# ZooMEISTER/vickers-hardness-Unet

Measured on AMD Instinct MI355X. Metric: 512x512 images/sec (train fwd+bwd), higher is better.
Workload: dtype bf16

## Files before the change

### include/vk_unet.h

```cpp
#ifndef VK_UNET_H
#define VK_UNET_H

#include <stddef.h>
#include <stdint.h>

#ifdef __cplusplus
extern "C" {
#endif

#define VK_ABI_VERSION 1
#define VK_STATS_REPLICAS 32

typedef enum { VK_F32 = 0, VK_BF16 = 1, VK_F16 = 2 } vk_dtype;

enum { VK_OK = 0, VK_ERR_ARG = -1, VK_ERR_STATE = -2, VK_ERR_UNSUPPORTED = -3 };

int vk_version(void);
const char* vk_last_error_string(void);
int vk_has_gfx950_code(void);
int vk_probe_mfma_rate(int iters, int waves_per_simd, float* sink, double* flops_out, void* stream);
int vk_set_reserved_cus(int n);
int vk_debug_hold_cus(int workgroups, int threads, int lds_bytes, int microseconds, const void* traffic, size_t traffic_bytes,
                      float* sink, void* stream);

// ... 16 lines not shown
  int N, H, W;
  int Ho, Wo;
  int K;
  int R, S, stride, pad;
  int transposed;
  vk_src src0, src1;
} vk_conv_desc;

int vk_conv_fwd(const vk_conv_desc* d, const void* w, void* y, void* y1, int split_k1, int accumulate,
                double* stats, void* stream);

int vk_conv_dgrad_pool2(const vk_conv_desc* d, const void* w, void* y_half, void* y1, int split_k1, int accumulate,
                        void* stream);

int vk_halo_pack(vk_dtype dtype, int rows, int red, const void* src, void* dst, void* stream);
int vk_conv_uses_halo_pack(const vk_conv_desc* d);
int vk_conv_fwd_packed(const vk_conv_desc* d, const void* w_halo, void* y, void* y1, int split_k1, int accumulate, double* stats,
                       void* stream);

#define VK_SPLITK_WORKSPACE_BYTES (32u << 20)
int vk_conv_fwd_splitk(const vk_conv_desc* d, const void* w_halo, void* y, void* workspace, size_t workspace_bytes, void* stream);

typedef struct {
  const void* z;
  const float* scale;
  const float* shift;
  double* sums;
  const void* mask;
  int accumulate;
} vk_bnr;

int vk_conv_dgrad_fused(const vk_conv_desc* d, const void* w, void* y, void* y1, int split_k1, int pool2, const vk_bnr* bnr,
                        void* stream);

int vk_conv1x1_fwd(const vk_conv_desc* d, const void* w, void* y, int accumulate, double* stats, void* stream);
int vk_conv1x1_wgrad(const vk_conv_desc* d, const void* dz, float* dw, void* workspace, size_t workspace_bytes, void* stream);

int vk_stem_fwd(vk_dtype dtype, int N, int H, int W, const void* x4, const void* wp, void* y, double* stats,
                void* stream);

#define VK_WGRAD_WORKSPACE_BYTES (64u << 20)
int vk_conv_wgrad(const vk_conv_desc* d, const void* dz, float* dw, void* workspace, size_t workspace_bytes, void* stream);
#define VK_WGRAD_BATCH_TABLE_BYTES (128u << 10)
int vk_conv_wgrad_batch_supports(const vk_conv_desc* d);
int vk_conv_wgrad_batch(const vk_conv_desc* descs, const void* const* dz, float* const* dw, int n, int workgroups, void* tables,
                        size_t tables_bytes, void* workspace, size_t workspace_bytes, void* stream);
int vk_stem_wgrad(vk_dtype dtype, int N, int H, int W, const void* x4, const void* dz, float* dw_krsc3, void* workspace,
                  size_t workspace_bytes, void* stream);
int vk_stem_wgrad_bn(vk_dtype dtype, int N, int H, int W, const void* x4, const void* g, const void* z, const float* coef_abc,
                     float* dw_krsc3, void* workspace, size_t workspace_bytes, void* stream);
int vk_conv_bwd_onepass(const vk_conv_desc* d_fwd, const void* g, const void* z, const float* coef_abc, const void* w_dgrad, void* y,
                        const vk_bnr* bnr, float* dw, void* workspace, size_t workspace_bytes, void* stream);
int vk_stem_dgrad(vk_dtype dtype, int N, int H, int W, const void* g, const void* z, const float* coef_abc, const float* w_krsc3,
                  float* dx, void* stream);

typedef struct {
  int h, w;
  int src_stride;
  int size;
  int nh, nw;
  int top, left;
  int pad_value;
} vk_letterbox_desc;

int vk_letterbox_preprocess(const vk_letterbox_desc* d, const uint8_t* bgr, float* x_nchw, void* stream);
int vk_letterbox_postprocess_mask(const vk_letterbox_desc* d, const float* logits, float thresh, uint8_t* mask_hw, void* stream);
// ... 98 lines not shown

typedef struct {
  int item;
  int k;
  int oy, ox;
  float zoom;
  float cos_a, sin_a;
  int reserved;
} vk_patch_params;

#define VK_PATCH_FORCE_GENERAL 1

int vk_patch_index(int n_items, const vk_patch_item* items_host, void* items_dev, size_t images_bytes, const uint8_t* masks,
                   size_t masks_bytes, int32_t* rowcum, size_t rowcum_len, void* stream);
int vk_patch_batch(int n, int size, int n_items, const void* items_dev, const uint8_t* images, const uint8_t* masks, const int32_t* rowcum,
                   const vk_patch_params* params_host, void* params_dev, int flags, int32_t* origins, uint8_t* patches_rgb,
                   uint8_t* patches_mask, void* stream);

int vk_input_transform(vk_dtype dtype, int N, int H, int W, const float* x, void* x4, void* stream);

int vk_bn_finalize(int C, int train, const double* stats, double count, const float* gamma, const float* beta,
                   float* running_mean, float* running_var, float eps, float momentum, float* scale, float* shift,
                   float* save_mean, float* save_invstd, void* stream);

int vk_bn_relu_maxpool(vk_dtype dtype, int N, int H, int W, int C, const void* z, const float* scale,
                       const float* shift, void* pooled, uint8_t* argmax, void* stream);
int vk_maxpool_bwd(vk_dtype dtype, int N, int H, int W, int C, const void* dpool, const uint8_t* argmax, void* dy,
                   void* stream);
int vk_maxpool_bwd_bn_reduce(vk_dtype dtype, int N, int H, int W, int C, const void* dpool, const uint8_t* argmax, const void* z,
                             const float* scale, const float* shift, void* dy, double* sums, void* stream);

int vk_bn_add_relu(vk_dtype dtype, size_t pixels, int C, const void* z, const float* scale, const float* shift,
                   const void* res, const float* rscale, const float* rshift, void* out, void* stream);

int vk_bn_bwd_reduce(vk_dtype dtype, size_t pixels, int C, const void* dy, const void* z, int mask_mode,
                     const float* scale, const float* shift, const void* mask_src, double* sums, void* stream);
int vk_bn_bwd_coeffs(int C, const double* sums, double count, const float* gamma, const float* save_mean,
                     const float* save_invstd, float* dgamma, float* dbeta, float* coef_abc, void* stream);
int vk_bn_bwd_apply(vk_dtype dtype, size_t pixels, int C, const void* dy, const void* z, int mask_mode,
                    const float* scale, const float* shift, const void* mask_src, const float* coef_abc, void* dz,
                    void* g_out, int g_accumulate, void* stream);
int vk_bn_bwd_coeffs_frozen(int C, const double* sums, const float* gamma, const float* running_mean, const float* running_invstd,
                            float* dgamma, float* dbeta, float* coef_abc, void* stream);
int vk_bn_bwd_apply_fused(vk_dtype dtype, size_t pixels, int C, const void* dy, const void* z, int mask_mode,
                          const float* scale, const float* shift, const void* mask_src, const double* sums, double count,
                          const float* gamma, const float* save_mean, const float* save_invstd, float* dgamma, float* dbeta,
                          void* dz, void* g_out, int g_accumulate, void* stream);

int vk_upsample2x_bwd(vk_dtype dtype, int N, int H, int W, int C, const void* d_up, void* d_low, int accumulate,
                      void* stream);

int vk_head_fwd(vk_dtype dtype, int N, int H, int W, const vk_src* src, const float* w9x16, const float* bias,
                float* logits, void* stream);
int vk_dec4_tail_eval(vk_dtype dtype, int N, int H, int W, const vk_src* src, const void* w1_pack, const float* scale1, const float* shift1,
                      const void* w2_plain, const float* scale2, const float* shift2, const float* head_w9x16, const float* head_bias,
                      float* logits, void* stream);
#define VK_HEAD_WORKSPACE_BYTES (1024u * 148u * 4u)
int vk_head_bwd(vk_dtype dtype, int N, int H, int W, const vk_src* src, const float* w9x16, const float* dlogits,
                void* dy, float* dw9x16, float* dbias, void* workspace, size_t workspace_bytes, void* stream);
int vk_head_bwd_fused(vk_dtype dtype, int N, int H, int W, const vk_src* src, const float* w9x16, const float* dlogits,
                      void* dy, float* dw9x16, float* dbias, const vk_bnr* bnr, void* workspace, size_t workspace_bytes, void* stream);

int vk_bce_dice_loss(size_t count, const float* logits, const float* target, double* sums, float* loss_out,
                     float* dlogits, float grad_scale, float w_bce, float w_dice, void* stream);

int vk_head_fwd_multi(vk_dtype dtype, int N, int H, int W, int C, const vk_src* src, const float* w, const float* bias, float* logits,
// ... 219 lines not shown
```

### vickers-hardness-unet_amd/_lib.py

```python
from __future__ import annotations

import ctypes as C
import os
import subprocess
from pathlib import Path

PKG_DIR = Path(__file__).resolve().parent
LIB_PATH = Path(os.environ["VK_LIB"]) if os.environ.get("VK_LIB") else PKG_DIR / "libvkunet.so"
CSRC = PKG_DIR / "csrc"

VK_F32, VK_BF16, VK_F16 = 0, 1, 2
VK_LOSS_BINARY, VK_LOSS_MULTILABEL, VK_LOSS_MULTICLASS = 0, 1, 2
VK_ENC_RESNET18, VK_ENC_RESNET34, VK_ENC_RESNET50 = 18, 34, 50
VK_ADAMW_MAX_GROUPS = 8
VK_NORM_L2, VK_NORM_INF = 0, 1
VK_TILE_MAX_ORIGINS, VK_TILE_MAX_SIDE = 64, 4096
VK_BLEND_PROB, VK_BLEND_LOGIT = 0, 1
VK_PATCH_FORCE_GENERAL = 1


class VkError(RuntimeError):
    pass


class vk_src(C.Structure):
    _fields_ = [("ptr", C.c_void_p), ("C", C.c_int), ("up", C.c_int), ("scale", C.c_void_p),
                ("shift", C.c_void_p), ("relu", C.c_int)]


class vk_conv_desc(C.Structure):
    _fields_ = [("dtype", C.c_int), ("N", C.c_int), ("H", C.c_int), ("W", C.c_int), ("Ho", C.c_int),
                ("Wo", C.c_int), ("K", C.c_int), ("R", C.c_int), ("S", C.c_int), ("stride", C.c_int),
                ("pad", C.c_int), ("transposed", C.c_int), ("src0", vk_src), ("src1", vk_src)]


class vk_bnr(C.Structure):
    _fields_ = [("z", C.c_void_p), ("scale", C.c_void_p), ("shift", C.c_void_p), ("sums", C.c_void_p), ("mask", C.c_void_p),
                ("accumulate", C.c_int)]


class vk_letterbox_desc(C.Structure):
    _fields_ = [("h", C.c_int), ("w", C.c_int), ("src_stride", C.c_int), ("size", C.c_int), ("nh", C.c_int),
                ("nw", C.c_int), ("top", C.c_int), ("left", C.c_int), ("pad_value", C.c_int)]


class vk_tile_desc(C.Structure):
    _fields_ = [("h", C.c_int), ("w", C.c_int), ("src_stride", C.c_int), ("T", C.c_int), ("overlap", C.c_int), ("ny", C.c_int),
                ("nx", C.c_int), ("ys", C.c_int * VK_TILE_MAX_ORIGINS), ("xs", C.c_int * VK_TILE_MAX_ORIGINS), ("view_mask", C.c_int),
                ("pad_value", C.c_int), ("C", C.c_int)]


class vk_geom_desc(C.Structure):
    _fields_ = [("h", C.c_int), ("w", C.c_int), ("bin_thresh", C.c_float), ("morph_kernel", C.c_int), ("open_iter", C.c_int),
                ("close_iter", C.c_int), ("min_area", C.c_int), ("max_components", C.c_int)]


class vk_geom_det(C.Structure):
    _fields_ = [("label", C.c_int), ("area", C.c_int), ("box", C.c_int * 8), ("cx", C.c_float), ("cy", C.c_float),
                ("rw", C.c_float), ("rh", C.c_float), ("ux", C.c_float), ("uy", C.c_float), ("hull_n", C.c_int),
                ("reserved", C.c_int), ("d1", C.c_double), ("d2", C.c_double), ("d_mean", C.c_double)]


class vk_geom_quad(C.Structure):
    _fields_ = [("label", C.c_int), ("area", C.c_int), ("box", C.c_int * 8), ("cx", C.c_float), ("cy", C.c_float),
                ("valid", C.c_int), ("branch", C.c_int), ("n_candidates", C.c_int), ("contour_n", C.c_int), ("hull_n", C.c_int),
                ("flags", C.c_int), ("quality", C.c_double), ("d1", C.c_double), ("d2", C.c_double), ("d_mean", C.c_double)]


class vk_aug_params(C.Structure):
    _fields_ = [("d4", C.c_int), ("rotate", C.c_int), ("cos_a", C.c_float), ("sin_a", C.c_float), ("photo", C.c_int),
                ("alpha", C.c_float), ("beta", C.c_float), ("blur_ksize", C.c_int), ("noise_scale", C.c_float),
# ... 60 lines not shown
                ("iters", C.c_int * 4), ("v", C.c_double * 8), ("vs", C.c_double * 8), ("d1", C.c_double), ("d2", C.c_double),
                ("d_mean", C.c_double)]


class vk_adamw_group(C.Structure):
    _fields_ = [("lr", C.c_float), ("beta1", C.c_float), ("beta2", C.c_float), ("eps", C.c_float), ("weight_decay", C.c_float)]


class vk_unet_config(C.Structure):
    _fields_ = [("N", C.c_int), ("size", C.c_int), ("dtype", C.c_int), ("training", C.c_int), ("width", C.c_int)]


class vk_tensor_info(C.Structure):
    _fields_ = [("name", C.c_char * 96), ("kind", C.c_int), ("dims", C.c_int * 4), ("ndim", C.c_int),
                ("offset", C.c_int64), ("numel", C.c_int64)]


vp, ci, cf, cd, sz, i64 = C.c_void_p, C.c_int, C.c_float, C.c_double, C.c_size_t, C.c_int64
P = C.POINTER

SIGNATURES = {
    "vk_version": (ci, []),
    "vk_last_error_string": (C.c_char_p, []),
    "vk_has_gfx950_code": (ci, []),
    "vk_probe_mfma_rate": (ci, [ci, ci, vp, P(C.c_double), vp]),
    "vk_set_reserved_cus": (ci, [ci]),
    "vk_debug_hold_cus": (ci, [ci, ci, ci, ci, vp, sz, vp, vp]),
    "vk_debug_set_stamp_buffer": (ci, [vp]),
    "vk_prof_enable": (ci, [ci]),
    "vk_prof_collect": (ci, [C.c_char_p, sz]),
    "vk_conv_fwd": (ci, [P(vk_conv_desc), vp, vp, vp, ci, ci, vp, vp]),
    "vk_conv_dgrad_pool2": (ci, [P(vk_conv_desc), vp, vp, vp, ci, ci, vp]),
    "vk_conv_dgrad_fused": (ci, [P(vk_conv_desc), vp, vp, vp, ci, ci, P(vk_bnr), vp]),
    "vk_head_bwd_fused": (ci, [ci, ci, ci, ci, P(vk_src), vp, vp, vp, vp, vp, P(vk_bnr), vp, sz, vp]),
    "vk_halo_pack": (ci, [ci, ci, ci, vp, vp, vp]),
    "vk_conv_uses_halo_pack": (ci, [P(vk_conv_desc)]),
    "vk_conv_fwd_packed": (ci, [P(vk_conv_desc), vp, vp, vp, ci, ci, vp, vp]),
    "vk_conv_fwd_splitk": (ci, [P(vk_conv_desc), vp, vp, vp, sz, vp]),
    "vk_stem_fwd": (ci, [ci, ci, ci, ci, vp, vp, vp, vp, vp]),
    "vk_conv_wgrad": (ci, [P(vk_conv_desc), vp, vp, vp, sz, vp]),
    "vk_conv1x1_fwd": (ci, [P(vk_conv_desc), vp, vp, ci, vp, vp]),
    "vk_conv1x1_wgrad": (ci, [P(vk_conv_desc), vp, vp, vp, sz, vp]),
    "vk_conv_wgrad_batch_supports": (ci, [P(vk_conv_desc)]),
    "vk_conv_wgrad_batch": (ci, [P(vk_conv_desc), P(vp), P(vp), ci, ci, vp, sz, vp, sz, vp]),
    "vk_stem_wgrad": (ci, [ci, ci, ci, ci, vp, vp, vp, vp, sz, vp]),
    "vk_stem_wgrad_bn": (ci, [ci, ci, ci, ci, vp, vp, vp, vp, vp, vp, sz, vp]),
    "vk_conv_bwd_onepass": (ci, [P(vk_conv_desc), vp, vp, vp, vp, vp, P(vk_bnr), vp, vp, sz, vp]),
    "vk_stem_dgrad": (ci, [ci, ci, ci, ci, vp, vp, vp, vp, vp, vp]),
    "vk_letterbox_preprocess": (ci, [P(vk_letterbox_desc), vp, vp, vp]),
    "vk_letterbox_postprocess_mask": (ci, [P(vk_letterbox_desc), vp, cf, vp, vp]),
    "vk_letterbox_postprocess_prob": (ci, [P(vk_letterbox_desc), vp, vp, vp]),
    "vk_letterbox_postprocess_labels": (ci, [P(vk_letterbox_desc), ci, vp, vp, vp]),
    "vk_letterbox_postprocess_mask_multi": (ci, [P(vk_letterbox_desc), ci, vp, cf, vp, vp]),
    "vk_letterbox_postprocess_prob_multi": (ci, [P(vk_letterbox_desc), ci, ci, vp, vp, vp]),
    "vk_tile_preprocess": (ci, [P(vk_tile_desc), vp, vp, vp]),
    "vk_tile_blend": (ci, [P(vk_tile_desc), ci, vp, cf, vp, vp, vp]),
    "vk_geom_workspace_bytes": (i64, [P(vk_geom_desc), ci]),
    "vk_geom_minarearect": (ci, [P(vk_geom_desc), ci, vp, vp, vp, vp, vp, sz, vp]),
    "vk_geom_quadrilateral": (ci, [P(vk_geom_desc), ci, ci, vp, vp, vp, vp, vp, sz, vp]),
    "vk_geom_slot_map": (ci, [P(vk_geom_desc), ci, vp, sz, vp, vp]),
    "vk_letterbox_u8": (ci, [P(vk_letterbox_desc), vp, vp, vp]),
    "vk_letterbox_mask_u8": (ci, [P(vk_letterbox_desc), vp, vp, vp]),
    "vk_augment_workspace_bytes": (C.c_size_t, [ci, ci]),
    "vk_augment_batch": (ci, [ci, ci, ci, vp, vp, vp, P(vk_aug_params), vp, vp, vp, C.c_size_t, vp, vp, vp]),
    "vk_patch_index": (ci, [ci, P(vk_patch_item), vp, sz, vp, sz, vp, sz, vp]),
    "vk_patch_batch": (ci, [ci, ci, ci, vp, vp, vp, vp, P(vk_patch_params), vp, ci, vp, vp, vp, vp]),
    "vk_input_transform": (ci, [ci, ci, ci, ci, vp, vp, vp]),
    "vk_bn_finalize": (ci, [ci, ci, vp, cd, vp, vp, vp, vp, cf, cf, vp, vp, vp, vp, vp]),
    "vk_bn_relu_maxpool": (ci, [ci, ci, ci, ci, ci, vp, vp, vp, vp, vp, vp]),
    "vk_maxpool_bwd": (ci, [ci, ci, ci, ci, ci, vp, vp, vp, vp]),
    "vk_maxpool_bwd_bn_reduce": (ci, [ci, ci, ci, ci, ci, vp, vp, vp, vp, vp, vp, vp, vp]),
    "vk_bn_add_relu": (ci, [ci, sz, ci, vp, vp, vp, vp, vp, vp, vp, vp]),
    "vk_bn_bwd_reduce": (ci, [ci, sz, ci, vp, vp, ci, vp, vp, vp, vp, vp]),
    "vk_bn_bwd_coeffs": (ci, [ci, vp, cd, vp, vp, vp, vp, vp, vp, vp]),
    "vk_bn_bwd_coeffs_frozen": (ci, [ci, vp, vp, vp, vp, vp, vp, vp, vp]),
    "vk_bn_bwd_apply": (ci, [ci, sz, ci, vp, vp, ci, vp, vp, vp, vp, vp, vp, ci, vp]),
    "vk_bn_bwd_apply_fused": (ci, [ci, sz, ci, vp, vp, ci, vp, vp, vp, vp, cd, vp, vp, vp, vp, vp, vp, vp, ci, vp]),
    "vk_upsample2x_bwd": (ci, [ci, ci, ci, ci, ci, vp, vp, ci, vp]),
    "vk_head_fwd": (ci, [ci, ci, ci, ci, P(vk_src), vp, vp, vp, vp]),
    "vk_dec4_tail_eval": (ci, [ci, ci, ci, ci, P(vk_src), vp, vp, vp, vp, vp, vp, vp, vp, vp, vp]),
    "vk_head_bwd": (ci, [ci, ci, ci, ci, P(vk_src), vp, vp, vp, vp, vp, vp, sz, vp]),
    "vk_bce_dice_loss": (ci, [sz, vp, vp, vp, vp, vp, cf, cf, cf, vp]),
    "vk_head_fwd_multi": (ci, [ci, ci, ci, ci, ci, P(vk_src), vp, vp, vp, vp]),
    "vk_head_multi_workspace_bytes": (sz, [ci]),
    "vk_head_bwd_multi": (ci, [ci, ci, ci, ci, ci, P(vk_src), vp, vp, vp, vp, vp, P(vk_bnr), vp, sz, vp]),
    "vk_multi_loss_workspace_bytes": (sz, [ci, ci, ci]),
    "vk_multilabel_loss": (ci, [ci, ci, ci, vp, vp, vp, sz, vp, vp, cf, cf, cf, vp]),
    "vk_multiclass_loss": (ci, [ci, ci, ci, vp, vp, vp, sz, vp, vp, cf, cf, cf, vp]),
    "vk_seg_loss_cfg_size": (sz, []),
    "vk_seg_loss_workspace_bytes": (sz, [ci, ci, ci]),
    "vk_seg_loss": (ci, [P(vk_seg_loss_cfg), ci, ci, ci, vp, vp, vp, sz, vp, vp, cf, vp]),
    "vk_lovasz_cfg_size": (sz, []),
    "vk_lovasz_workspace_bytes": (sz, [P(vk_lovasz_cfg), ci, ci, ci]),
    "vk_lovasz_loss": (ci, [P(vk_lovasz_cfg), ci, ci, ci, vp, vp, vp, sz, vp, vp, cf, ci, vp]),
    "vk_lovasz_flat_workspace_bytes": (sz, [ci, i64]),
    "vk_lovasz_flat": (ci, [vp, vp, ci, i64, vp, sz, vp, vp, vp, vp]),
    "vk_seg_metrics_workspace_bytes": (C.c_size_t, [ci]),
    "vk_seg_metrics": (ci, [ci, sz, vp, vp, ci, cf, cf, vp, sz, vp, vp]),
    "vk_seg_metrics_multi_workspace_bytes": (sz, [ci, ci]),
    "vk_seg_metrics_multi": (ci, [ci, ci, ci, sz, vp, vp, ci, cf, cf, vp, sz, vp, vp, vp, vp]),
    "vk_sweep_hist": (ci, [ci, sz, sz, vp, vp, ci, ci, ci, ci, ci, vp, vp, ci, vp, vp, vp]),
    "vk_sweep_curves_layout": (ci, [ci, ci, ci, ci, P(vk_sweep_layout)]),
    "vk_sweep_curves_out_bytes": (sz, [ci, ci, ci, ci]),
    "vk_sweep_curves": (ci, [ci, ci, ci, vp, vp, ci, cf, vp, sz, vp, sz, vp]),
    "vk_inst_contingency": (ci, [ci, ci, ci, vp, vp, ci, ci, vp, vp]),
# ... 117 lines not shown
```

### vickers-hardness-unet_amd/csrc/conv_halo.hip

```cpp
#include <stdlib.h>
#include <string.h>

#include <string>
#include <type_traits>

#include "vk_common.h"

#ifdef VK_STAMP
#define VK_T(var) { __builtin_amdgcn_sched_barrier(0); const unsigned long long t_ = __builtin_amdgcn_s_memtime(); __builtin_amdgcn_s_waitcnt(0xC07F); __builtin_amdgcn_sched_barrier(0); var = t_; }
#else
#define VK_T(var)
#endif

namespace vk {

struct HaloSrc {
  const void* ptr;
  const float* scale;
  const float* shift;
  int C, up, relu;
  uint32_t bytes;
};

#ifndef VK_EPI_BATCH_READS
#define VK_EPI_BATCH_READS 1
#endif
#ifndef VK_COLP_DEFER_STATS
#define VK_COLP_DEFER_STATS 1
#endif
#ifndef VK_COLQ_ILV
#define VK_COLQ_ILV 1
#endif
#ifndef VK_COLQ_DIAG
#define VK_COLQ_DIAG 0
#endif
#ifndef VK_COLQ_PRE
#define VK_COLQ_PRE 1
#endif
struct HaloParams {
  HaloSrc s0, s1;
  const void* w;
  uint32_t w_bytes;
  void* y0;
  void* y1;
  int ld0, ld1, split;
  double* stats;
  int N, H, W, K, C, flip, accumulate, pool2;
  int Hi, Wi;
  int tiles_x, tiles_y, nchunks;
  unsigned long long* stamps;
  int kyn;
  int ksplit;
  size_t slab_bytes;
  float* slab;
  int dbg;
  const void* bnr_z;
  const float* bnr_scale;
  const float* bnr_shift;
  double* bnr_sums;
  const void* bnr_mask;
};

template <typename T, int TH, int BN, int WGM, int WGN>
struct HaloCfg {
  using Tr = ElemTraits<T>;
  static constexpr int EB = Tr::kBytes;
  static constexpr int VE = Tr::kVec;
  static constexpr int CK = 64 / EB;
  static constexpr int HW_ = 18, HH = TH + 2, HPIX = HH * HW_;
  static constexpr int APS = 96;
  static constexpr int A_BYTES = HPIX * APS;
  static constexpr int B_BYTES = 3 * BN * 64;
  static constexpr int NPV = (HPIX * 4 + 255) / 256;
  static constexpr int NBV = (3 * BN * 4 + 255) / 256;
  static constexpr int BM = TH * 16;
  static constexpr int WR = TH / WGM;
  static constexpr int WCH = BN / WGN;
  static constexpr int TP = WR, TC = WCH / 16;
  static constexpr int ESB = BN * EB + 16;
  static constexpr int EVPR = BN / VE;
  static constexpr int ERPP = 256 / EVPR;
  static constexpr int EPASS = BM / ERPP;
  static constexpr int RED_OFF = BM * ESB;
  static constexpr int MAIN = A_BYTES + 2 * B_BYTES;
  static constexpr int ESLOTS = (BN / VE > 16) ? 4 * 4 / (BN / VE / 16) : 4 * 4;
  static constexpr int EPI = RED_OFF + ESLOTS * BN * 2 * 4;
  static constexpr int SMEM = MAIN > EPI ? MAIN : EPI;
  static_assert(WGM * WGN == 4 && TH % WGM == 0 && BN % (16 * WGN) == 0, "wave layout");
  static_assert(EPASS >= 1, "epilogue mapping");
  static_assert(SMEM <= 160 * 1024, "main-loop / epilogue LDS image exceeds the 160 KiB of a CU");
};

__device__ __forceinline__ int swz(int row) { return ((row >> 2) & 1) << 1; }

__device__ __forceinline__ int halo_group(int tid) {
  const int g = tid >> 2;
  return (g & ~3) | ((g & 1) << 1) | ((g >> 1) & 1);
}


template <typename T, int TH, int BN, int TP, int TC, int NT = 256, bool PRE = false, int OS = 1>
__device__ __forceinline__ void halo_epilogue(char* smem, f32x4_t (&acc)[TC][TP], const HaloParams& p, int n, int y0, int x0, int n0,
                                              int wrow0, int wch0, int py = 0, int px = 0, double* defer = nullptr) {
  using Tr = ElemTraits<T>;
  constexpr int EB = Tr::kBytes, VE = Tr::kVec;
  constexpr int BM = TH * 16;
  constexpr int ESB = BN * EB + 16;
  constexpr int EVPR = BN / VE, ERPP = NT / EVPR, EPASS = BM / ERPP, NW = NT / 64;
  constexpr int RED_OFF = BM * ESB;
  static_assert(BM % ERPP == 0 && EVPR <= 64, "epilogue mapping");
  const int tid = threadIdx.x, lane = tid & 63, wave = tid >> 6;
  const int li = lane & 15, kg = lane >> 4;

  const int e_row = tid / EVPR;
  const int e_vec = (EVPR == 16 && EB == 2) ? (((tid & 15) + ((e_row & 1) ? 15 : 0)) & 15) : tid % EVPR;
  const int col0 = n0 + e_vec * VE;
  const bool col_ok = col0 < p.K;
  char* yb = (char*)p.y0;
  int ld = p.ld0, colx = col0;
  bool first_part = true;
  if (p.split > 0 && col0 >= p.split) { yb = (char*)p.y1; ld = p.ld1; colx = col0 - p.split; first_part = false; }
  float s1[VE], s2[VE];
#pragma unroll
  for (int j = 0; j < VE; ++j) { s1[j] = 0.f; s2[j] = 0.f; }
  const bool bnr = p.bnr_z != nullptr && first_part && col_ok;
  const bool ext_mask = p.bnr_mask != nullptr;
  float bsc[VE], bsh[VE];
  if (bnr && !ext_mask) {
#pragma unroll
    for (int j = 0; j < VE; ++j) { bsc[j] = p.bnr_scale[colx + j]; bsh[j] = p.bnr_shift[colx + j]; }
  }
  auto finish = [&](float (&f)[VE], size_t elem_off, const u32x4_t* pre_old, const u32x4_t* pre_z, const u32x4_t* pre_m = nullptr) {
    u32x4_t* gp = reinterpret_cast<u32x4_t*>(yb + elem_off * EB);
    if (p.accumulate) {
      float o[VE];
      Vec16<T>::unpack(pre_old ? *pre_old : *gp, o);
#pragma unroll
      for (int j = 0; j < VE; ++j) f[j] += o[j];
    }
    u32x4_t v = Vec16<T>::pack(f);
    Vec16<T>::unpack(v, f);
    if (bnr) {
      float zf[VE];
      Vec16<T>::unpack(pre_z ? *pre_z : *reinterpret_cast<const u32x4_t*>((const char*)p.bnr_z + elem_off * EB), zf);
      if (ext_mask) {
        float mf[VE];
        Vec16<T>::unpack(pre_m ? *pre_m : *reinterpret_cast<const u32x4_t*>((const char*)p.bnr_mask + elem_off * EB), mf);
#pragma unroll
        for (int j = 0; j < VE; ++j)
          if (!(mf[j] > 0.f)) f[j] = 0.f;
      } else {
#pragma unroll
        for (int j = 0; j < VE; ++j)
          if (!(fmaf(zf[j], bsc[j], bsh[j]) > 0.f)) f[j] = 0.f;
      }
#pragma unroll
      for (int j = 0; j < VE; ++j) {
        s1[j] += f[j];
        s2[j] += f[j] * zf[j];
      }
      v = Vec16<T>::pack(f);
    } else {
#pragma unroll
      for (int j = 0; j < VE; ++j) { s1[j] += f[j]; s2[j] += f[j] * f[j]; }
    }
    *gp = v;
  };
  constexpr bool PRE_M = PRE && NT == 512;
  u32x4_t oldv[PRE ? EPASS : 1], zv[PRE ? EPASS : 1], mv[PRE_M ? EPASS : 1];
  constexpr bool EARLY = PRE && NT == 512;
  auto request_pre = [&]() {
    if (!(PRE && (p.accumulate || bnr) && !(p.pool2 && first_part))) return;
#pragma unroll
    for (int ps = 0; ps < (PRE ? EPASS : 0); ++ps) {
      const int row = e_row + ps * ERPP;
      const int y = OS * (y0 + (row >> 4)) + py, x = OS * (x0 + (row & 15)) + px;
      oldv[ps] = u32x4_t{0, 0, 0, 0};
      zv[ps] = u32x4_t{0, 0, 0, 0};
      if (PRE_M) mv[ps] = u32x4_t{0, 0, 0, 0};
      if (y < p.H && x < p.W && col_ok) {
        const size_t eoff = (((size_t)n * p.H + y) * p.W + x) * ld + colx;
        if (p.accumulate) oldv[ps] = *reinterpret_cast<const u32x4_t*>(yb + eoff * EB);
        if (bnr) zv[ps] = *reinterpret_cast<const u32x4_t*>((const char*)p.bnr_z + eoff * EB);
        if (PRE_M && bnr && ext_mask) mv[ps] = *reinterpret_cast<const u32x4_t*>((const char*)p.bnr_mask + eoff * EB);
      }
    }
  };
  if (EARLY) request_pre();
#pragma unroll
  for (int a = 0; a < TC; ++a)
#pragma unroll
    for (int b = 0; b < TP; ++b) {
      const int ch = wch0 + a * 16 + kg * 4;
      const int px = (wrow0 + b) * 16 + li;
      char* dst = smem + px * ESB + ch * EB;
      if (EB == 4) {
        *reinterpret_cast<f32x4_t*>(dst) = acc[a][b];
      } else {
        float f[8] = {acc[a][b][0], acc[a][b][1], acc[a][b][2], acc[a][b][3], 0.f, 0.f, 0.f, 0.f};
        const u32x4_t pk = Vec16<T>::pack(f);
        *reinterpret_cast<u32x2_t*>(dst) = u32x2_t{pk[0], pk[1]};
      }
    }
  __syncthreads();
  if (!EARLY) request_pre();

  if (p.pool2 && first_part) {
    const int Hh = p.H >> 1, Wh = p.W >> 1;
    for (int pr = e_row; pr < (TH / 2) * 8; pr += ERPP) {
      const int py = pr >> 3, px = pr & 7;
      const int y = (y0 >> 1) + py, x = (x0 >> 1) + px;
      if (y < Hh && x < Wh && col_ok) {
        float f[VE];
#pragma unroll
        for (int j = 0; j < VE; ++j) f[j] = 0.f;
#pragma unroll
        for (int q = 0; q < 4; ++q) {
// ... 83 lines not shown
          atomicAdd(sp + n0 + tid, (double)a);
          atomicAdd(sp + kc + n0 + tid, (double)b);
        }
      } else {
        double* sp = p.stats + (size_t)(blockIdx.x % VK_STATS_REPLICAS) * 2 * p.K;
        atomicAdd(sp + n0 + tid, (double)a);
        atomicAdd(sp + p.K + n0 + tid, (double)b);
      }
    }
  }
}

template <int BN>
__device__ __forceinline__ void stats_flush(const HaloParams& p, int n0, double (&d)[2]) {
  const int tid = threadIdx.x;
  if (tid < BN && n0 + tid < p.K) {
    if (p.bnr_sums) {
      const int kc = p.ld0;
      if (n0 + tid < kc) {
        double* sp = p.bnr_sums + (size_t)(blockIdx.x % VK_STATS_REPLICAS) * 2 * kc;
        atomicAdd(sp + n0 + tid, d[0]);
        atomicAdd(sp + kc + n0 + tid, d[1]);
      }
    } else if (p.stats) {
      double* sp = p.stats + (size_t)(blockIdx.x % VK_STATS_REPLICAS) * 2 * p.K;
      atomicAdd(sp + n0 + tid, d[0]);
      atomicAdd(sp + p.K + n0 + tid, d[1]);
    }
  }
  d[0] = 0.0;
  d[1] = 0.0;
}

template <typename T, int TH, int BN, int WGM, int WGN>
__global__ __launch_bounds__(256, 2) void conv3x3_halo_kernel(const HaloParams p) {
  using Cfg = HaloCfg<T, TH, BN, WGM, WGN>;
  constexpr int EB = Cfg::EB, VE = Cfg::VE, CK = Cfg::CK, HPIX = Cfg::HPIX, NPV = Cfg::NPV, NBV = Cfg::NBV;
  constexpr int TP = Cfg::TP, TC = Cfg::TC, APS = Cfg::APS;

  extern __shared__ __attribute__((aligned(16))) char smem[];
  char* const Abuf = smem;
  char* const Bbuf = smem + Cfg::A_BYTES;
  const int tid = threadIdx.x, lane = tid & 63, wave = tid >> 6;

  int bt = blockIdx.x;
  if ((gridDim.x & 7) == 0) bt = (bt & 7) * (int)(gridDim.x >> 3) + (bt >> 3);
  const int tx = bt % p.tiles_x;
  bt /= p.tiles_x;
  const int ty = bt % p.tiles_y;
  const int n = bt / p.tiles_y;
  const int y0 = ty * TH, x0 = tx * 16;
  const int n0 = blockIdx.y * BN;

  const __amdgpu_buffer_rsrc_t rs0 = make_rsrc(p.s0.ptr, p.s0.bytes);
  const __amdgpu_buffer_rsrc_t rs1 = make_rsrc(p.s1.ptr ? p.s1.ptr : p.s0.ptr, p.s1.ptr ? p.s1.bytes : 0u);
  const __amdgpu_buffer_rsrc_t rsw = make_rsrc(p.w, p.w_bytes);

  const int hv = tid & 3;
  const int hgrp = halo_group(tid);
  int h_full[NPV], h_half[NPV];
  const int Hh = p.H >> 1, Wh = p.W >> 1;
#pragma unroll
  for (int i = 0; i < NPV; ++i) {
    const int hp = hgrp + i * 64;
    const int hy = hp / 18, hx = hp - hy * 18;
    const int y = y0 - 1 + hy, x = x0 - 1 + hx;
    const bool ok = hp < HPIX && (unsigned)y < (unsigned)p.H && (unsigned)x < (unsigned)p.W;
// ... 129 lines not shown
  auto stage = [&](int st, u32x4_t (&ld_regs)[NBV], const u32x4_t (&st_regs)[NBV]) {
    const int cc = st / 3, r = st - cc * 3;
    const bool next_chunk = cc + 1 < p.nchunks;
#ifdef VK_STAMP
    unsigned long long t0, t1, t2, t3, t4;
#endif
    VK_T(t0)
    if (st + 2 < nst) load_b(ld_regs, st + 2);
    if (r == 0 && next_chunk) load_halo(cc + 1);
    VK_T(t1)
    compute(st & 1, r);
    VK_T(t2)
    if (r == 2 && next_chunk) {
      __syncthreads();
      store_halo();
    }
    if (st + 1 < nst) store_b(st_regs, (st + 1) & 1);
    VK_T(t3)
    __syncthreads();
    VK_T(t4)
#ifdef VK_STAMP
    tk_load += t1 - t0; tk_comp += t2 - t1; tk_store += t3 - t2; tk_bar += t4 - t3;
#endif
  };
  for (int st = 0; st < nst; st += 2) {
    stage(st, breg0, breg1);
    if (st + 1 < nst) stage(st + 1, breg1, breg0);
  }

#ifdef VK_STAMP
  unsigned long long te0, te1;
  VK_T(te0)
#endif
  halo_epilogue<T, TH, BN, TP, TC>(smem, acc, p, n, y0, x0, n0, wrow0, wch0);
#ifdef VK_STAMP
  VK_T(te1)
  if (p.stamps && lane == 0) {
    unsigned long long* o = p.stamps + ((size_t)(blockIdx.y * gridDim.x + blockIdx.x) * 4 + wave) * 8;
    o[0] = tk_load; o[1] = tk_comp; o[2] = tk_store; o[3] = tk_bar; o[4] = te1 - te0; o[5] = te0 - t_begin; o[6] = te1 - t_begin; o[7] = nst;
  }
#endif
}

template <typename T, int TH, int BN, int WGM, int WGN, bool ADB, int STR = 1>
struct ColCfg {
  using Tr = ElemTraits<T>;
  static constexpr int EB = Tr::kBytes;
  static constexpr int VE = Tr::kVec;
  static constexpr int CK = 64 / EB;
  static constexpr int NW = WGM * WGN, NT = 64 * NW;
  static constexpr int HH = STR == 1 ? TH + 2 : 2 * TH + 1;
  static constexpr int HWI = STR == 1 ? 18 : 33;
  static constexpr int RS = STR == 1 ? 18 : 34;
  static constexpr int HPIX = HH * HWI;
  static constexpr int APS = 96;
  static constexpr int A_BYTES = HH * RS * APS;
  static constexpr int NA = ADB ? 2 : 1;
  static constexpr int B_BYTES = 3 * BN * 64;
  static constexpr int NPV = (HPIX * 4 + NT - 1) / NT;
  static constexpr int NPIECE = 3 * BN / 16;
  static constexpr int BM = TH * 16;
  static constexpr int TP = TH / WGM, TC = BN / WGN / 16;
  static constexpr int NX = STR * (TP - 1) + 3;
  static constexpr int ESB = BN * EB + 16;
  static constexpr int NB = (BN <= 64 && STR == 1) ? 3 : 2;
  static constexpr int MAIN = NA * A_BYTES + NB * B_BYTES;
  static constexpr int ESLOTS = (BN / VE > 16) ? NW * 4 / (BN / VE / 16) : NW * 4;
  static constexpr int EPI = BM * ESB + ESLOTS * BN * 2 * 4;
  static constexpr int SMEM = MAIN > EPI ? MAIN : EPI;
  static_assert(TH % WGM == 0 && BN % (16 * WGN) == 0 && (NW == 4 || NW == 8), "wave layout");
  static_assert(STR == 1 || STR == 2, "stride");
  static_assert(SMEM <= 160 * 1024, "main-loop / epilogue LDS image exceeds the 160 KiB of a CU");
  static_assert(EPI >= BM * ESB + ESLOTS * BN * 8, "epilogue partial-sum slots must fit behind the output tile");
};

template <typename T, int TH, int BN, int WGM, int WGN, bool ADB, int MINW, int STR = 1>
__global__ __launch_bounds__(64 * WGM * WGN, MINW) void conv3x3_col_kernel(const HaloParams p) {
  using Cfg = ColCfg<T, TH, BN, WGM, WGN, ADB, STR>;
  constexpr int EB = Cfg::EB, VE = Cfg::VE, CK = Cfg::CK, HPIX = Cfg::HPIX, NPV = Cfg::NPV, NT = Cfg::NT, NW = Cfg::NW;
  constexpr int TP = Cfg::TP, TC = Cfg::TC, APS = Cfg::APS, NPIECE = Cfg::NPIECE, RS = Cfg::RS, HWI = Cfg::HWI, NX = Cfg::NX;
  typedef __attribute__((address_space(3))) void lds_void;

  extern __shared__ __attribute__((aligned(16))) char smem[];
  char* const Abuf = smem;
  char* const Bbuf = smem + Cfg::NA * Cfg::A_BYTES;
  const int tid = threadIdx.x, lane = tid & 63;
  const int wave = __builtin_amdgcn_readfirstlane(tid >> 6);

  int bt = blockIdx.x;
  int ky = blockIdx.y;
  if (p.kyn > 0) {
    const int j = bt >> 3;
    ky = j % p.kyn;
    bt = (bt & 7) * (int)((gridDim.x / p.kyn) >> 3) + j / p.kyn;
  } else if (p.kyn < 0) {
    const int kn = -p.kyn, xcd = bt & 7;
    ky = xcd % kn;
    bt = (xcd / kn) * (int)(gridDim.x >> 3) + (bt >> 3);
  } else if ((gridDim.x & 7) == 0) {
    bt = (bt & 7) * (int)(gridDim.x >> 3) + (bt >> 3);
  }
  const int tx = bt % p.tiles_x;
  bt /= p.tiles_x;
  const int ty = bt % p.tiles_y;
  const int n = bt / p.tiles_y;
  const int y0 = ty * TH, x0 = tx * 16;
  const int n0 = ky * BN;

  const __amdgpu_buffer_rsrc_t rs0 = make_rsrc(p.s0.ptr, p.s0.bytes);
// ... 155 lines not shown
      compute(A + (STR == 1 ? s : (s & 1) * 17 + (s >> 1)) * APS, Bbuf + (st & 1) * Cfg::B_BYTES + b_lane);
      VK_T(t2)
      if (ADB) {
        if (s == 1 && next_chunk && !(p.dbg & 4)) store_halo(Anext);
      } else {
        if (s == 2 && next_chunk && !(p.dbg & 4)) {
          __syncthreads();
          store_halo(Anext);
        }
      }
      VK_T(t3)
      if (!(p.dbg & 8)) __syncthreads();
      VK_T(t4)
#ifdef VK_STAMP
      tk_load += t1 - t0; tk_comp += t2 - t1; tk_store += t3 - t2; tk_bar += t4 - t3;
#endif
    }
  }
#ifdef VK_STAMP
  unsigned long long te0, te1;
  VK_T(te0)
#endif
  if (p.ksplit > 1) {
    float* sl = p.slab + (size_t)blockIdx.z * ((size_t)p.N * p.H * p.W * p.K);
#pragma unroll
    for (int a = 0; a < TC; ++a)
#pragma unroll
      for (int b = 0; b < TP; ++b) {
        const int y = y0 + wrow0 + b, x = x0 + li, ch = n0 + wch0 + a * 16 + kg * 4;
        if (y < p.H && x < p.W && ch < p.K) *reinterpret_cast<f32x4_t*>(sl + (((size_t)n * p.H + y) * p.W + x) * p.K + ch) = acc[a][b];
      }
    return;
  }
  halo_epilogue<T, TH, BN, TP, TC, NT, (BN <= 64 && TH == 16)>(smem, acc, p, n, y0, x0, n0, wrow0, wch0);
#ifdef VK_STAMP
  VK_T(te1)
  if (p.stamps && lane == 0) {
    unsigned long long* o = p.stamps + ((size_t)(blockIdx.y * gridDim.x + blockIdx.x) * NW + wave) * 8;
    o[0] = tk_load; o[1] = tk_comp; o[2] = tk_store; o[3] = tk_bar; o[4] = te1 - te0; o[5] = t_pro - t_begin; o[6] = te1 - t_begin; o[7] = st;
  }
#endif
}

template <typename T, int TH, int BN, int WGM, int WGN>
struct S2dCfg {
  using Tr = ElemTraits<T>;
  static constexpr int EB = Tr::kBytes, VE = Tr::kVec, CK = 64 / EB;
  static constexpr int NW = WGM * WGN, NT = 64 * NW;
  static constexpr int HH = TH + 1, RS = 17, HPIX = HH * RS, APS = 96;
  static constexpr int A_BYTES = HPIX * APS;
  static constexpr int B_BYTES = 3 * BN * 64;
  static constexpr int NPV = (HPIX * 4 + NT - 1) / NT;
  static constexpr int NPIECE = 3 * BN / 16;
  static constexpr int BM = TH * 16;
  static constexpr int TP = TH / WGM, TC = BN / WGN / 16;
  static constexpr int ESB = BN * EB + 16;
  static constexpr int MAIN = 2 * A_BYTES + 2 * B_BYTES;
  static constexpr int ESLOTS = (BN / VE > 16) ? NW * 4 / (BN / VE / 16) : NW * 4;
  static constexpr int EPI = BM * ESB + ESLOTS * BN * 2 * 4;
  static constexpr int SMEM = MAIN > EPI ? MAIN : EPI;
  static_assert(TH % WGM == 0 && BN % (16 * WGN) == 0 && NW == 8, "wave layout");
  static_assert(4 * TP * TC <= 32, "accumulator budget (four parity classes)");
  static_assert(SMEM <= 160 * 1024, "LDS image exceeds the 160 KiB of a CU");
};

template <typename T, int TH, int BN, int WGM, int WGN>
__global__ __launch_bounds__(64 * WGM * WGN, 1) void conv3x3_s2dg_kernel(const HaloParams p) {
// ... 108 lines not shown
    dma_b(cc, 1, (st + 1) & 1);
    if (next_chunk) load_halo(cc + 1);
    compute(A, Bbuf + (st & 1) * Cfg::B_BYTES + b_lane, std::integral_constant<int, 0>{});
    __syncthreads();
    ++st;
    dma_b(cc, 2, (st + 1) & 1);
    compute(A, Bbuf + (st & 1) * Cfg::B_BYTES + b_lane, std::integral_constant<int, 1>{});
    if (next_chunk) store_halo(Anext);
    __syncthreads();
    ++st;
    if (next_chunk) dma_b(cc + 1, 0, (st + 1) & 1);
    compute(A, Bbuf + (st & 1) * Cfg::B_BYTES + b_lane, std::integral_constant<int, 2>{});
    __syncthreads();
    ++st;
  }
#pragma unroll
  for (int q = 0; q < 4; ++q) {
    if (q) __syncthreads();
    halo_epilogue<T, TH, BN, TP, TC, NT, false, 2>(smem, acc[q], p, n, y0, x0, n0, wrow0, wch0, q >> 1, q & 1);
  }
}

template <typename T, int TH, int BN, int WGM, int WGN>
struct ColqCfg : ColCfg<T, TH, BN, WGM, WGN, true> {
  using Base = ColCfg<T, TH, BN, WGM, WGN, true>;
  static constexpr int MAIN = 2 * Base::A_BYTES + 3 * Base::B_BYTES;
  static constexpr int SMEM = MAIN > Base::EPI ? MAIN : Base::EPI;
  static constexpr int DMAW = Base::NPIECE / Base::NW;
  static_assert(Base::NPIECE % Base::NW == 0, "every wave must issue the same number of weight DMAs per stage (partial vmcnt wait)");
  static_assert(DMAW >= 1 && DMAW <= 15, "vmcnt immediate");
  static_assert(SMEM <= 160 * 1024, "LDS image exceeds the 160 KiB of a CU");
};

template <typename T, int TH, int BN, int WGM, int WGN>
__global__ __launch_bounds__(64 * WGM * WGN, 1) void conv3x3_colq_kernel(const HaloParams p) {
  using Cfg = ColqCfg<T, TH, BN, WGM, WGN>;
  constexpr int EB = Cfg::EB, VE = Cfg::VE, CK = Cfg::CK, HPIX = Cfg::HPIX, NPV = Cfg::NPV, NT = Cfg::NT, NW = Cfg::NW;
  constexpr int TP = Cfg::TP, TC = Cfg::TC, APS = Cfg::APS, NPIECE = Cfg::NPIECE;
  typedef __attribute__((address_space(3))) void lds_void;

  extern __shared__ __attribute__((aligned(16))) char smem[];
  char* const Abuf = smem;
  char* const Bbuf = smem + 2 * Cfg::A_BYTES;
  const int tid = threadIdx.x, lane = tid & 63;
  const int wave = __builtin_amdgcn_readfirstlane(tid >> 6);

  int bt = blockIdx.x;
  int ky = blockIdx.y;
  if (p.kyn > 0) {
    const int j = bt >> 3;
    ky = j % p.kyn;
    bt = (bt & 7) * (int)((gridDim.x / p.kyn) >> 3) + j / p.kyn;
  } else if (p.kyn < 0) {
    const int kn = -p.kyn, xcd = bt & 7;
    ky = xcd % kn;
    bt = (xcd / kn) * (int)(gridDim.x >> 3) + (bt >> 3);
  } else if ((gridDim.x & 7) == 0) {
    bt = (bt & 7) * (int)(gridDim.x >> 3) + (bt >> 3);
  }
  const int tx = bt % p.tiles_x;
  bt /= p.tiles_x;
  const int ty = bt % p.tiles_y;
  const int n = bt / p.tiles_y;
  const int y0 = ty * TH, x0 = tx * 16;
  const int n0 = ky * BN;

  const __amdgpu_buffer_rsrc_t rs0 = make_rsrc(p.s0.ptr, p.s0.bytes);
// ... 176 lines not shown
      } else {
      if (next_chunk) {
        if (s == 0 && !(VK_COLQ_DIAG & 4)) load_halo(cc + 1);
        dma_b(cc + 1, s);
      }
      if (more) {
#pragma unroll
        for (int a = 0; a < TC; ++a) W0n[a] = rd(Bn + (a * 16) * 64);
      }
      mfma_row(W2, 2);
      }
      if (more) {
#pragma unroll
        for (int h = 0; h < TP; ++h) X[h] = Xn[h];
#pragma unroll
        for (int a = 0; a < TC; ++a) W0[a] = W0n[a];
      }
    }
  }
  if (VK_COLQ_ILV) __builtin_amdgcn_s_waitcnt(kWaitAll);
  __syncthreads();

  if (p.ksplit > 1) {
    float* sl = p.slab + (size_t)blockIdx.z * ((size_t)p.N * p.H * p.W * p.K);
#pragma unroll
    for (int a = 0; a < TC; ++a)
#pragma unroll
      for (int b = 0; b < TP; ++b) {
        const int y = y0 + wrow0 + b, x = x0 + li, ch = n0 + wch0 + a * 16 + kg * 4;
        if (y < p.H && x < p.W && ch < p.K) *reinterpret_cast<f32x4_t*>(sl + (((size_t)n * p.H + y) * p.W + x) * p.K + ch) = acc[a][b];
      }
    return;
  }
  halo_epilogue<T, TH, BN, TP, TC, NT, ((VK_COLQ_PRE && sizeof(T) == 2) || (BN <= 64 && TH == 16))>(smem, acc, p, n, y0, x0, n0, wrow0, wch0);
}

template <typename T, int TH, int BN, int WGM, int WGN>
struct ColsCfg : ColCfg<T, TH, BN, WGM, WGN, true> {
  using Base = ColCfg<T, TH, BN, WGM, WGN, true>;
  static constexpr int MAIN = 2 * Base::A_BYTES + 4 * Base::B_BYTES;
  static constexpr int SMEM = MAIN > Base::EPI ? MAIN : Base::EPI;
  static constexpr int DMAW = Base::NPIECE / Base::NW;
  static_assert(Base::NPIECE % Base::NW == 0, "every wave must issue the same number of weight DMAs per stage (partial vmcnt wait)");
  static_assert(DMAW >= 1 && DMAW <= 15, "vmcnt immediate");
  static_assert(SMEM <= 160 * 1024, "LDS image exceeds the 160 KiB of a CU");
};

template <typename T, int TH, int BN, int WGM, int WGN>
__global__ __launch_bounds__(64 * WGM * WGN, 1) void conv3x3_cols_kernel(const HaloParams p) {
  using Cfg = ColsCfg<T, TH, BN, WGM, WGN>;
  constexpr int EB = Cfg::EB, VE = Cfg::VE, CK = Cfg::CK, HPIX = Cfg::HPIX, NPV = Cfg::NPV, NT = Cfg::NT, NW = Cfg::NW;
  constexpr int TP = Cfg::TP, TC = Cfg::TC, APS = Cfg::APS, NPIECE = Cfg::NPIECE;
  typedef __attribute__((address_space(3))) void lds_void;

  extern __shared__ __attribute__((aligned(16))) char smem[];
  char* const Abuf = smem;
  char* const Bbuf = smem + 2 * Cfg::A_BYTES;
  const int tid = threadIdx.x, lane = tid & 63;
  const int wave = __builtin_amdgcn_readfirstlane(tid >> 6);

  int bt = blockIdx.x;
  int ky = blockIdx.y;
  if (p.kyn > 0) {
    const int j = bt >> 3;
    ky = j % p.kyn;
    bt = (bt & 7) * (int)((gridDim.x / p.kyn) >> 3) + j / p.kyn;
  } else if (p.kyn < 0) {
    const int kn = -p.kyn, xcd = bt & 7;
    ky = xcd % kn;
    bt = (xcd / kn) * (int)(gridDim.x >> 3) + (bt >> 3);
  } else if ((gridDim.x & 7) == 0) {
    bt = (bt & 7) * (int)(gridDim.x >> 3) + (bt >> 3);
  }
  const int tx = bt % p.tiles_x;
  bt /= p.tiles_x;
  const int ty = bt % p.tiles_y;
  const int n = bt / p.tiles_y;
  const int y0 = ty * TH, x0 = tx * 16;
  const int n0 = ky * BN;

  const __amdgpu_buffer_rsrc_t rs0 = make_rsrc(p.s0.ptr, p.s0.bytes);
// ... 176 lines not shown
      tkX += t1 - t0; tkW += t2 - t1; tkB1 += t3 - t2; tkY += t4 - t3; tkB2 += t5 - t4;
#endif
    }
  }
  if (!late) {
    asm volatile("" ::: "memory");
    __builtin_amdgcn_s_barrier();
    asm volatile("" ::: "memory");
  }
  __builtin_amdgcn_s_waitcnt(kWaitAll);
#ifdef VK_STAMP
  {
    unsigned long long t_end;
    VK_T(t_end)
    if (p.stamps && lane == 0) {
      unsigned long long* o = p.stamps + ((size_t)(blockIdx.y * gridDim.x + blockIdx.x) * NW + wave) * 8;
      o[0] = tkX; o[1] = tkW; o[2] = tkB1; o[3] = tkY; o[4] = tkB2; o[5] = t_pro - t_begin; o[6] = t_end - t_begin; o[7] = 3 * (c_end - c_begin);
    }
  }
#endif
  __syncthreads();

  if (p.ksplit > 1) {
    float* sl = p.slab + (size_t)blockIdx.z * ((size_t)p.N * p.H * p.W * p.K);
#pragma unroll
    for (int a = 0; a < TC; ++a)
#pragma unroll
      for (int b = 0; b < TP; ++b) {
        const int y = y0 + wrow0 + b, x = x0 + li, ch = n0 + wch0 + a * 16 + kg * 4;
        if (y < p.H && x < p.W && ch < p.K) *reinterpret_cast<f32x4_t*>(sl + (((size_t)n * p.H + y) * p.W + x) * p.K + ch) = acc[a][b];
      }
    return;
  }
  halo_epilogue<T, TH, BN, TP, TC, NT, (BN <= 64 && TH == 16)>(smem, acc, p, n, y0, x0, n0, wrow0, wch0);
}

template <typename T, int TH, int BN, int WGM, int WGN, int MINW>
__global__ __launch_bounds__(64 * WGM * WGN, MINW) void conv3x3_colp_kernel(const HaloParams p) {
  using Cfg = ColCfg<T, TH, BN, WGM, WGN, false>;
  constexpr int EB = Cfg::EB, VE = Cfg::VE, CK = Cfg::CK, HPIX = Cfg::HPIX, NPV = Cfg::NPV, NT = Cfg::NT, NW = Cfg::NW;
  constexpr int TP = Cfg::TP, TC = Cfg::TC, APS = Cfg::APS, NPIECE = Cfg::NPIECE;
  typedef __attribute__((address_space(3))) void lds_void;

  extern __shared__ __attribute__((aligned(16))) char smem[];
  char* const Abuf = smem;
  char* const Bbuf = smem + Cfg::A_BYTES;
  const int tid = threadIdx.x, lane = tid & 63;
  const int wave = __builtin_amdgcn_readfirstlane(tid >> 6);
  const int nsp = p.N * p.tiles_y * p.tiles_x;
  const int total = nsp * p.kyn;
  const bool xcd_runs = (nsp & 7) == 0 && (gridDim.x & 7) == 0 && p.kyn == 1;

  const __amdgpu_buffer_rsrc_t rs0 = make_rsrc(p.s0.ptr, p.s0.bytes);
  const __amdgpu_buffer_rsrc_t rs1 = make_rsrc(p.s1.ptr ? p.s1.ptr : p.s0.ptr, p.s1.ptr ? p.s1.bytes : 0u);
  const __amdgpu_buffer_rsrc_t rsw = make_rsrc(p.w, p.w_bytes);

  const int hv = tid & 3;
  const int hgrp = halo_group(tid);
  const int Hh = p.H >> 1, Wh = p.W >> 1;
  struct TileGeo { int n, y0, x0, n0; };
  auto decode = [&](int t) {
    TileGeo g;
    const int ky = t % p.kyn;
    int bt = t / p.kyn;
    if (xcd_runs) bt = (bt & 7) * (nsp >> 3) + (bt >> 3);
    const int tx = bt % p.tiles_x;
    bt /= p.tiles_x;
    const int ty = bt % p.tiles_y;
    g.n = bt / p.tiles_y;
    g.y0 = ty * TH; g.x0 = tx * 16; g.n0 = ky * BN;
// ... 119 lines not shown
    TileGeo gn = g;
    const char* const A = Abuf + a_lane;
    auto stage = [&](int cc, auto s_c, auto last_c) {
      constexpr int s = decltype(s_c)::value;
      constexpr bool LAST = decltype(last_c)::value;
      if (s < 2) dma_b(g.n0, cc, s + 1, (st + 1) & 1);
      else if (!LAST) dma_b(g.n0, cc + 1, 0, (st + 1) & 1);
      if (s == 0 && !LAST) load_halo(cc + 1, h_full, h_half);
      if (s == 2 && LAST && more_tiles) {
        gn = decode(tn);
        halo_index(gn, h_full_n, h_half_n);
        load_halo(0, h_full_n, h_half_n);
      }
      compute(A + s * APS, Bbuf + (st & 1) * Cfg::B_BYTES + b_lane);
      if (s == 2 && !LAST) {
        __syncthreads();
        store_halo(Abuf, h_full);
      }
      __syncthreads();
      ++st;
    };
    using I0 = std::integral_constant<int, 0>;
    using I1 = std::integral_constant<int, 1>;
    using I2 = std::integral_constant<int, 2>;
    for (int cc = 0; cc + 1 < p.nchunks; ++cc) {
      stage(cc, I0{}, std::false_type{});
      stage(cc, I1{}, std::false_type{});
      stage(cc, I2{}, std::false_type{});
    }
    stage(p.nchunks - 1, I0{}, std::true_type{});
    stage(p.nchunks - 1, I1{}, std::true_type{});
    stage(p.nchunks - 1, I2{}, std::true_type{});
    constexpr bool DEFER = VK_COLP_DEFER_STATS && (sizeof(T) == 2 || BN < 64);
    halo_epilogue<T, TH, BN, TP, TC, NT, (BN <= 64 && TH == 16)>(smem, acc, p, g.n, g.y0, g.x0, g.n0, wrow0, wch0, 0, 0, DEFER ? dsum : nullptr);
    if (DEFER && (!more_tiles || gn.n0 != g.n0)) stats_flush<BN>(p, g.n0, dsum);
    if (!more_tiles) break;
    __syncthreads();
    t = tn;
    g = gn;
#pragma unroll
    for (int i = 0; i < NPV; ++i) { h_full[i] = h_full_n[i]; h_half[i] = h_half_n[i]; }
  }
}

struct StemTile {
  static constexpr int ROWS = 37, VPR = 20, PITCH = VPR * 16;
  static constexpr int A_BYTES = ROWS * PITCH;
  static constexpr int W_OFF = (A_BYTES + 1023) / 1024 * 1024, W_BYTES = 28 * 1024;
};

template <typename T>
__global__ __launch_bounds__(256, 3) void stem7x7_kernel(const HaloParams p) {
  using Cfg = ColCfg<T, 16, 64, 4, 1, false>;
  static_assert(sizeof(T) == 2, "16-bit types: a pixel of the NHWC4 input is 8 bytes");
  constexpr int NV = (StemTile::ROWS * StemTile::VPR + 255) / 256;
  extern __shared__ __attribute__((aligned(16))) char smem[];
  const int tid = threadIdx.x, lane = tid & 63;
  const int wave = __builtin_amdgcn_readfirstlane(tid >> 6);
  int bt = blockIdx.x;
  if ((gridDim.x & 7) == 0) bt = (bt & 7) * (int)(gridDim.x >> 3) + (bt >> 3);
  const int tx = bt % p.tiles_x;
  bt /= p.tiles_x;
  const int ty = bt % p.tiles_y;
  const int n = bt / p.tiles_y;
  const int y0 = ty * 16, x0 = tx * 16;
  const __amdgpu_buffer_rsrc_t rs0 = make_rsrc(p.s0.ptr, p.s0.bytes);
  const __amdgpu_buffer_rsrc_t rsw = make_rsrc(p.w, p.w_bytes);
// ... 30 lines not shown
  const int wrow0 = wave * 4;
  f32x4_t acc[4][4];
#pragma unroll
  for (int a = 0; a < 4; ++a)
#pragma unroll
    for (int b = 0; b < 4; ++b) acc[a][b] = f32x4_t{0.f, 0.f, 0.f, 0.f};
  const char* const xl = smem + (2 * wrow0) * StemTile::PITCH + 16 * (li + kg);
  const char* const wl = Wl + lane * 16;
#pragma unroll
  for (int r = 0; r < 7; ++r) {
    u32x4_t X[4], Wc[4];
#pragma unroll
    for (int a = 0; a < 4; ++a) Wc[a] = *reinterpret_cast<const u32x4_t*>(wl + (4 * r + a) * 1024);
#pragma unroll
    for (int b = 0; b < 4; ++b) X[b] = *reinterpret_cast<const u32x4_t*>(xl + (2 * b + r) * StemTile::PITCH);
#pragma unroll
    for (int a = 0; a < 4; ++a)
#pragma unroll
      for (int b = 0; b < 4; ++b) acc[a][b] = Mma<T>::run(Wc[a], X[b], acc[a][b]);
  }
  __syncthreads();
  halo_epilogue<T, 16, 64, 4, 4, 256, false>(smem, acc, p, n, y0, x0, 0, wrow0, 0);
}

int stem_tile_launch(vk_dtype dt, int N, int H, int W, const void* x4, const void* wp, void* y, double* stats, hipStream_t st) {
  if (dt == VK_F32 || getenv("VK_NO_STEM_TILE")) return VK_ERR_UNSUPPORTED;
  if ((size_t)N * H * W * 8 >= (1ull << 31)) return VK_ERR_UNSUPPORTED;
  HaloParams p;
  memset((void*)&p, 0, sizeof(p));
  p.s0 = HaloSrc{x4, nullptr, nullptr, 4, 0, 0, (uint32_t)((size_t)N * H * W * 8)};
  p.w = wp;
  p.w_bytes = 64u * 7u * 32u * 2u;
  p.y0 = y;
  p.ld0 = 64;
  p.stats = stats;
  p.N = N; p.H = H / 2; p.W = W / 2; p.K = 64; p.C = 4;
  p.Hi = H; p.Wi = W;
  p.tiles_x = (p.W + 15) / 16;
  p.tiles_y = (p.H + 15) / 16;
  using Cfg = ColCfg<bf16_t, 16, 64, 4, 1, false>;
  constexpr int MAIN = StemTile::W_OFF + StemTile::W_BYTES;
  constexpr int SMEM = MAIN > Cfg::EPI ? MAIN : Cfg::EPI;
  const dim3 grid((unsigned)(N * p.tiles_y * p.tiles_x));
  vkh::ProfScope ps("stem_tile_16b", st, 2.0 * (double)N * p.H * p.W * 64.0 * 147.0, ((double)N * H * W * 4.0 + (double)N * p.H * p.W * 64.0) * 2.0);
  if (dt == VK_BF16) hipLaunchKernelGGL(stem7x7_kernel<bf16_t>, grid, dim3(256), SMEM, st, p);
  else hipLaunchKernelGGL(stem7x7_kernel<f16_t>, grid, dim3(256), SMEM, st, p);
  VK_CHECK_HIP(hipGetLastError());
  return VK_OK;
}

template <typename T, int BN>
struct C16Cfg {
  static constexpr int TH = 16, HPIX = 18 * 18;
  static constexpr int APS = 48;
  static constexpr int A_BYTES = HPIX * APS + 64;
  static constexpr int BS = 336;
  static constexpr int B_BYTES = BN * BS;
  static constexpr int TP = 4, TC = BN / 16;
  static constexpr int ESB = BN * 2 + 16;
  static constexpr int EPI = 256 * ESB + 4 * 4 * BN * 2 * 4;
  static constexpr int MAIN = A_BYTES + B_BYTES;
  static constexpr int SMEM = MAIN > EPI ? MAIN : EPI;
};

template <typename T, int BN>
__global__ __launch_bounds__(256) void conv3x3_c16_kernel(const HaloParams p) {
// ... 594 lines not shown

template <typename T>
__global__ void k_pack_halo(int rows, int red, const T* __restrict__ src, T* __restrict__ dst) {
  constexpr int CK = 64 / ElemTraits<T>::kBytes, VE = ElemTraits<T>::kVec;
  const size_t total = (size_t)rows * 9 * red / VE;
  for (size_t v = blockIdx.x * (size_t)blockDim.x + threadIdx.x; v < total; v += (size_t)gridDim.x * blockDim.x) {
    const int pos = (int)(v & 3);
    size_t t = v >> 2;
    const int k = (int)(t % rows);
    t /= rows;
    const int tap = (int)(t % 9);
    const int cc = (int)(t / 9);
    const int j = pos ^ (((k >> 2) & 1) << 1);
    const u32x4_t x = *reinterpret_cast<const u32x4_t*>(src + ((size_t)k * 9 + tap) * red + cc * CK + j * VE);
    *reinterpret_cast<u32x4_t*>(dst + v * VE) = x;
  }
}

int halo_pack_impl(vk_dtype dt, int rows, int red, const void* src, void* dst, hipStream_t st) {
  const int eb = dt == VK_F32 ? 4 : 2;
  VK_CHECK_ARG(src && dst && rows > 0 && red % (64 / eb) == 0, "vk_halo_pack: reduction channels %d must be a multiple of %d", red, 64 / eb);
  const size_t nvec = (size_t)rows * 9 * red * eb / 16;
  unsigned nb = (unsigned)((nvec + 255) / 256);
  if (nb > 4096) nb = 4096;
  switch (dt) {
    case VK_F32: hipLaunchKernelGGL(k_pack_halo<float>, dim3(nb), dim3(256), 0, st, rows, red, (const float*)src, (float*)dst); break;
    case VK_BF16: hipLaunchKernelGGL(k_pack_halo<bf16_t>, dim3(nb), dim3(256), 0, st, rows, red, (const bf16_t*)src, (bf16_t*)dst); break;
    case VK_F16: hipLaunchKernelGGL(k_pack_halo<f16_t>, dim3(nb), dim3(256), 0, st, rows, red, (const f16_t*)src, (f16_t*)dst); break;
  }
  VK_CHECK_HIP(hipGetLastError());
  return VK_OK;
}

template <typename T, int TH, int BN, int WGM, int WGN>
static int launch_halo(HaloParams p, hipStream_t st) {
  using Cfg = HaloCfg<T, TH, BN, WGM, WGN>;
  p.tiles_x = (p.W + 15) / 16;
  p.tiles_y = (p.H + TH - 1) / TH;
  dim3 grid((unsigned)(p.N * p.tiles_y * p.tiles_x), (unsigned)((p.K + BN - 1) / BN), 1);
  static bool attr_done = false;
  if (!attr_done && Cfg::SMEM > 64 * 1024) {
    VK_CHECK_HIP(hipFuncSetAttribute((const void*)conv3x3_halo_kernel<T, TH, BN, WGM, WGN>,
                                     hipFuncAttributeMaxDynamicSharedMemorySize, Cfg::SMEM));
    attr_done = true;
  }
  {
    static const std::string tag_f = std::string("halo_") + (sizeof(T) == 4 ? "f32" : "16b") + "_t" + std::to_string(TH) + "_bn" + std::to_string(BN);
    static const std::string tag_d = tag_f + "_dgrad";
    const double macs = (double)p.N * p.H * p.W * p.K * 9.0 * p.C;
    const double bytes = ((double)p.N * p.H * p.W * (p.C + p.K) + 9.0 * p.K * p.C) * sizeof(T);
    const std::string& btag = p.flip ? tag_d : tag_f;
    const std::string dtag = getenv("VK_PROF_DETAIL") ? btag + ":H" + std::to_string(p.H) + "_K" + std::to_string(p.K) + "_C" + std::to_string(p.C) : btag;
    vkh::ProfScope ps(dtag.c_str(), st, 2.0 * macs, bytes);
    hipLaunchKernelGGL((conv3x3_halo_kernel<T, TH, BN, WGM, WGN>), grid, dim3(256), Cfg::SMEM, st, p);
  }
  VK_CHECK_HIP(hipGetLastError());
  return VK_OK;
}

template <typename T>
__global__ __launch_bounds__(256) void k_splitk_reduce(size_t n4, int splits, const float* __restrict__ slab, T* __restrict__ y) {
  const size_t e = blockIdx.x * (size_t)blockDim.x + threadIdx.x;
  if (e >= n4) return;
  f32x4_t a = *reinterpret_cast<const f32x4_t*>(slab + e * 4);
  for (int s = 1; s < splits; ++s) a = a + *reinterpret_cast<const f32x4_t*>(slab + ((size_t)s * n4 + e) * 4);
  if constexpr (sizeof(T) == 4) {
    *reinterpret_cast<f32x4_t*>(y + e * 4) = a;
  } else {
    float f[8] = {a[0], a[1], a[2], a[3], 0.f, 0.f, 0.f, 0.f};
    const u32x4_t pk = Vec16<T>::pack(f);
    *reinterpret_cast<u32x2_t*>(y + e * 4) = u32x2_t{pk[0], pk[1]};
  }
}

template <int PIPE, typename T, int TH, int BN, int WGM, int WGN, bool ADB, int MINW, int STR>
struct ColLaunch {
  using Cfg = ColCfg<T, TH, BN, WGM, WGN, ADB, STR>;
  static const void* kernel() { return (const void*)conv3x3_col_kernel<T, TH, BN, WGM, WGN, ADB, MINW, STR>; }
};
template <typename T, int TH, int BN, int WGM, int WGN, bool ADB, int MINW>
struct ColLaunch<1, T, TH, BN, WGM, WGN, ADB, MINW, 1> {
  using Cfg = ColqCfg<T, TH, BN, WGM, WGN>;
  static const void* kernel() { return (const void*)conv3x3_colq_kernel<T, TH, BN, WGM, WGN>; }
};
template <typename T, int TH, int BN, int WGM, int WGN, bool ADB, int MINW>
struct ColLaunch<2, T, TH, BN, WGM, WGN, ADB, MINW, 1> {
  using Cfg = ColsCfg<T, TH, BN, WGM, WGN>;
  static const void* kernel() { return (const void*)conv3x3_cols_kernel<T, TH, BN, WGM, WGN>; }
};

template <typename T, int TH, int BN, int WGM, int WGN, bool ADB, int MINW, int PIPE = 0, int STR = 1>
static int launch_col(HaloParams p, hipStream_t st) {
  using Sel = ColLaunch<PIPE, T, TH, BN, WGM, WGN, ADB, MINW, STR>;
  using Cfg = typename Sel::Cfg;
  const void* const kernel = Sel::kernel();
  p.tiles_x = (p.W + 15) / 16;
  p.tiles_y = (p.H + TH - 1) / TH;
  dim3 grid((unsigned)(p.N * p.tiles_y * p.tiles_x), (unsigned)((p.K + BN - 1) / BN), 1);
  const size_t out_elems = (size_t)p.N * p.H * p.W * p.K;
  int ks = 1;
  if (p.slab && !p.stats && !p.bnr_z && !p.accumulate && !p.pool2 && p.split == 0 && !getenv("VK_NO_SPLITK")) {
    const long wgs = (long)grid.x * grid.y;
    const char* force = getenv("VK_SPLITK");
    ks = force ? atoi(force) : (wgs < 128 ? (int)(256 / wgs) : 1);
    if (ks > p.nchunks / 2) ks = p.nchunks / 2;
    if (ks > 32) ks = 32;
    while (ks > 1 && (size_t)ks * out_elems * sizeof(float) > p.slab_bytes) --ks;
    if (ks < 2) ks = 1;
  }
  p.ksplit = ks;
  grid.z = (unsigned)ks;
  p.kyn = 0;
  if (ks == 1 && grid.y > 1 && (grid.x & 7) == 0 && !getenv("VK_COL_NO_KYFAST")) {
    p.kyn = (int)grid.y;
    grid.x *= grid.y;
    grid.y = 1;
    const char* km = getenv("VK_COL_KYMODE");
    const bool wst = km ? km[0] == 'w' : (size_t)p.w_bytes >= (3u << 20);
    if (PIPE && wst && 8 % p.kyn == 0 && (grid.x / 8) * (8 / p.kyn) * p.kyn == grid.x) p.kyn = -p.kyn;
  }
  static bool attr_done = false;
  if (!attr_done && Cfg::SMEM > 64 * 1024) {
    VK_CHECK_HIP(hipFuncSetAttribute(kernel, hipFuncAttributeMaxDynamicSharedMemorySize, Cfg::SMEM));
    attr_done = true;
  }
  {
    static const std::string tag_f = std::string(PIPE == 2 ? "cols_" : PIPE == 1 ? "colq_" : "col_") + (sizeof(T) == 4 ? "f32" : "16b") + "_t" + std::to_string(TH) + "_bn" +
                                     std::to_string(BN) + "_w" + std::to_string(WGM * WGN) + (STR == 2 ? "_s2" : "");
    static const std::string tag_d = tag_f + "_dgrad";
    const double macs = (double)p.N * p.H * p.W * p.K * 9.0 * p.C;
    const double bytes = ((double)p.N * ((double)p.Hi * p.Wi * p.C + (double)p.H * p.W * p.K) + 9.0 * p.K * p.C) * sizeof(T);
    const std::string& btag = p.flip ? tag_d : tag_f;
    const std::string dtag = getenv("VK_PROF_DETAIL") ? btag + ":H" + std::to_string(p.H) + "_K" + std::to_string(p.K) + "_C" + std::to_string(p.C) : btag;
    vkh::ProfScope ps(dtag.c_str(), st, 2.0 * macs, bytes);
    void* args[] = {(void*)&p};
    VK_CHECK_HIP(hipLaunchKernel(kernel, grid, dim3(Cfg::NT), args, Cfg::SMEM, st));
  }
  if (ks > 1) {
    vkh::ProfScope ps("splitk_reduce", st, 0.0, (double)out_elems * (4.0 * ks + sizeof(T)));
    hipLaunchKernelGGL(k_splitk_reduce<T>, dim3((unsigned)((out_elems / 4 + 255) / 256)), dim3(256), 0, st, out_elems / 4, ks, p.slab, (T*)p.y0);
  }
  VK_CHECK_HIP(hipGetLastError());
  return VK_OK;
}

template <typename T, int TH, int BN, int WGM, int WGN, int MINW>
static int launch_colp(HaloParams p, hipStream_t st) {
  using Cfg = ColCfg<T, TH, BN, WGM, WGN, false>;
  p.tiles_x = (p.W + 15) / 16;
  p.tiles_y = (p.H + TH - 1) / TH;
  p.kyn = (p.K + BN - 1) / BN;
  p.ksplit = 1;
  const long total = (long)p.N * p.tiles_y * p.tiles_x * p.kyn;
  int per_cu = (160 * 1024) / Cfg::SMEM;
  if (per_cu > 4) per_cu = 4;
  if (per_cu < 1) per_cu = 1;
  long g = 256L * per_cu;
  if (const char* e = getenv("VK_COL_PERSIST_GRID")) g = atol(e) > 0 ? atol(e) : g;
  if (g > total) g = total;
  static bool attr_done = false;
  if (!attr_done && Cfg::SMEM > 64 * 1024) {
    VK_CHECK_HIP(hipFuncSetAttribute((const void*)conv3x3_colp_kernel<T, TH, BN, WGM, WGN, MINW>,
                                     hipFuncAttributeMaxDynamicSharedMemorySize, Cfg::SMEM));
    attr_done = true;
  }
  {
    static const std::string tag_f = std::string("col_") + (sizeof(T) == 4 ? "f32" : "16b") + "_t" + std::to_string(TH) + "_bn" + std::to_string(BN) +
                                     "_w" + std::to_string(WGM * WGN);
    static const std::string tag_d = tag_f + "_dgrad";
    const double macs = (double)p.N * p.H * p.W * p.K * 9.0 * p.C;
    const double bytes = ((double)p.N * p.H * p.W * (p.C + p.K) + 9.0 * p.K * p.C) * sizeof(T);
    const std::string& btag = p.flip ? tag_d : tag_f;
    const std::string dtag = getenv("VK_PROF_DETAIL") ? btag + ":H" + std::to_string(p.H) + "_K" + std::to_string(p.K) + "_C" + std::to_string(p.C) : btag;
    vkh::ProfScope ps(dtag.c_str(), st, 2.0 * macs, bytes);
    hipLaunchKernelGGL((conv3x3_colp_kernel<T, TH, BN, WGM, WGN, MINW>), dim3((unsigned)g), dim3(Cfg::NT), Cfg::SMEM, st, p);
  }
  VK_CHECK_HIP(hipGetLastError());
  return VK_OK;
}

template <typename T, int BN>
static int launch_small(const HaloParams& p, hipStream_t st) {
  const long total = (long)p.N * ((p.H + 15) / 16) * ((p.W + 15) / 16) * ((p.K + BN - 1) / BN);
  const char* pe = getenv("VK_COL_PERSIST");
  const long min_tiles = pe ? (atol(pe) == 0 ? -1 : atol(pe)) : (BN == 64 ? 1024 : -1);
  const bool splitk_wanted = p.slab && !p.stats && !p.bnr_z && !p.accumulate && !p.pool2 && p.split == 0 && total < 128;
  if (min_tiles > 0 && !splitk_wanted && total >= min_tiles) return launch_colp<T, 16, BN, 4, 1, 2>(p, st);
  return launch_col<T, 16, BN, 4, 1, false, 2>(p, st);
}

template <typename T>
static int col_select(const HaloParams& p, hipStream_t st) {
  const char* alt_s = getenv("VK_COL_ALT");
  const int alt = alt_s ? atoi(alt_s) : 0;
  const long tiles16 = (long)p.N * ((p.H + 15) / 16) * ((p.W + 15) / 16);
  if (p.K >= 128) {
    const long kt = (p.K + 127) / 128;
    if (alt == 1) return launch_col<T, 16, 128, 2, 2, true, 1>(p, st);
    if (alt == 8 || (alt == 0 && p.nchunks <= 2 && p.K % 128 != 0) || (alt == 0 && p.nchunks == 1)) return launch_small<T, 64>(p, st);
    if (alt == 3 || (alt != 2 && alt != 7 && p.nchunks <= 2)) return launch_col<T, 8, 128, 2, 2, false, 2>(p, st);
    const char* const pipe_s = getenv("VK_COL_PIPE");
    const int pipe = pipe_s ? atoi(pipe_s) : 1;
    if (alt == 7 || (alt != 2 && tiles16 * kt < 256))
      return pipe == 2 ? launch_col<T, 8, 128, 2, 4, true, 1, 2>(p, st)
             : pipe    ? launch_col<T, 8, 128, 2, 4, true, 1, 1>(p, st) : launch_col<T, 8, 128, 2, 4, true, 2>(p, st);
    if (alt == 9) return launch_col<T, 16, 128, 2, 4, true, 1, 1>(p, st);
    return pipe == 2 ? launch_col<T, 16, 128, 4, 2, true, 1, 2>(p, st)
           : pipe    ? launch_col<T, 16, 128, 4, 2, true, 1, 1>(p, st) : launch_col<T, 16, 128, 4, 2, true, 2>(p, st);
// ... 77 lines not shown
  if (RS < 8) RS = 8;
  q.tiles_y = RS;
  const long strips = (long)p.N * ((p.H + RS - 1) / RS) * ((p.W + 15) / 16);
  dim3 grid((unsigned)((strips + 3) / 4), 1, 1);
  static const std::string tag_f = std::string("stream_16b_c") + std::to_string(CIN) + (UP ? "up" : "") + "_k" + std::to_string(TC * 16);
  static const std::string tag_d = tag_f + "_dgrad";
  const std::string& tag = p.flip ? tag_d : tag_f;
  const double in_px = (double)p.N * (p.H >> (UP ? 1 : 0)) * (p.W >> (UP ? 1 : 0));
  const double out_px = (double)p.N * p.H * p.W * (p.pool2 ? 0.25 : 1.0);
  const double bytes = (in_px * CIN + out_px * p.K * (p.bnr_z ? 2.0 : 1.0) + 9.0 * p.K * CIN) * 2.0;
  vkh::ProfScope ps(tag.c_str(), st, 2.0 * (double)p.N * p.H * p.W * p.K * 9.0 * CIN, bytes);
  hipLaunchKernelGGL((conv3x3_stream_kernel<T, CIN, TC, UP, MODE>), grid, dim3(256), Cfg::SMEM, st, q);
  VK_CHECK_HIP(hipGetLastError());
  return VK_OK;
}

template <typename T>
static int stream_try(const HaloParams& p, hipStream_t st) {
  if (getenv("VK_NO_STREAM")) return VK_ERR_UNSUPPORTED;
  if (p.s1.ptr || p.accumulate || p.split || p.ld0 != p.K) return VK_ERR_UNSUPPORTED;
  const bool up = p.s0.up != 0, bnr = p.bnr_z != nullptr, pool = p.pool2 != 0;
  if ((pool || up) && ((p.H | p.W) & 1)) return VK_ERR_UNSUPPORTED;
  const bool fwd = !p.flip && !bnr && !pool;
  if (fwd && p.C == 32 && up && p.K == 16) return launch_stream<T, 32, 1, true, 0>(p, st);
  if (fwd && p.C == 16 && !up && p.K == 16) return launch_stream<T, 16, 1, false, 0>(p, st);
  if (fwd && p.C == 32 && !up && p.K == 32) return launch_stream<T, 32, 2, false, 0>(p, st);
  if (p.flip && !p.s0.scale && bnr && !pool && p.C == 16 && p.K == 16) return launch_stream<T, 16, 1, false, 2>(p, st);
  if (p.flip && !p.s0.scale && bnr && !pool && p.C == 32 && p.K == 32) return launch_stream<T, 32, 2, false, 2>(p, st);
  if (p.flip && !p.s0.scale && bnr && pool && p.C == 16 && p.K == 32) return launch_stream<T, 16, 2, false, 3>(p, st);
  return VK_ERR_UNSUPPORTED;
}

int conv3x3_halo_try(const vk_conv_desc* d, const void* w, int packed, void* y, void* y1, int split_k1, int accumulate, double* stats,
                     int pool2, const vk_bnr* bnr, hipStream_t st, void* workspace, size_t workspace_bytes) {
  const bool s2 = d->stride == 2 && !d->transposed && d->H == 2 * d->Ho && d->W == 2 * d->Wo && d->K >= 128 && !d->src0.up && !d->src1.ptr &&
                  !pool2 && !bnr && !accumulate && !split_k1 && !getenv("VK_NO_S2_TILE");
  const bool s2d = d->stride == 2 && d->transposed && d->Ho == 2 * d->H && d->Wo == 2 * d->W && d->K >= 64 && d->K % 64 == 0 && !d->src0.up &&
                   !d->src1.ptr && !d->src0.scale && !pool2 && !bnr && !split_k1 && !getenv("VK_NO_S2_TILE");
  if (d->R != 3 || d->S != 3 || d->pad != 1) return VK_ERR_UNSUPPORTED;
  if (!s2 && !s2d && (d->stride != 1 || d->H != d->Ho || d->W != d->Wo)) return VK_ERR_UNSUPPORTED;
  const int eb = d->dtype == VK_F32 ? 4 : 2;
  const int ck = 64 / eb;
  const int C = d->src0.C + (d->src1.ptr ? d->src1.C : 0);
  const bool c16 = (eb == 2) && C == 16 && !d->src1.ptr && !d->src0.up && !s2 && !s2d;
  if (c16 ? packed : !packed) return VK_ERR_UNSUPPORTED;
  if (!c16 && (d->src0.C % ck || (d->src1.ptr && d->src1.C % ck))) return VK_ERR_UNSUPPORTED;
  if (d->K % 16) return VK_ERR_UNSUPPORTED;
  if (pool2 && ((d->H | d->W) & 1)) return VK_ERR_UNSUPPORTED;
  if (d->src1.ptr && d->src1.up) return VK_ERR_UNSUPPORTED;
  if ((size_t)d->N * d->H * d->W * C * eb >= (1ull << 31) || (size_t)d->N * d->H * d->W >= (1ull << 31)) return VK_ERR_UNSUPPORTED;
  if (s2d && (size_t)d->N * d->Ho * d->Wo * d->K * eb >= (1ull << 32)) return VK_ERR_UNSUPPORTED;
  HaloParams p;
  auto mk = [&](const vk_src& s) {
    HaloSrc h;
    h.ptr = s.ptr; h.scale = s.scale; h.shift = s.shift; h.C = s.C; h.up = s.up; h.relu = s.relu;
    h.bytes = s.ptr ? (uint32_t)((size_t)d->N * (d->H >> s.up) * (d->W >> s.up) * s.C * eb) : 0u;
    return h;
  };
  p.s0 = mk(d->src0);
  if (d->src1.ptr) p.s1 = mk(d->src1);
  else p.s1 = HaloSrc{nullptr, nullptr, nullptr, 0, 0, 0, 0u};
  p.w = w;
  p.w_bytes = (uint32_t)((size_t)d->K * 9 * C * eb);
  p.y0 = y; p.y1 = y1; p.split = split_k1;
  p.ld0 = split_k1 ? split_k1 : d->K;
  p.ld1 = split_k1 ? d->K - split_k1 : 0;
  p.stats = stats;
  p.N = d->N; p.H = d->Ho; p.W = d->Wo; p.K = d->K; p.C = C;
  p.Hi = d->H; p.Wi = d->W;
  p.flip = d->transposed;
  p.accumulate = accumulate;
  p.pool2 = pool2;
  p.ksplit = 1;
  p.kyn = 0;
  p.slab = (reinterpret_cast<uintptr_t>(workspace) & 15) ? nullptr : (float*)workspace;
  p.slab_bytes = p.slab ? workspace_bytes : 0;
  p.stamps = nullptr;
  p.dbg = getenv("VK_COL_DBG") ? atoi(getenv("VK_COL_DBG")) : 0;
  if (p.dbg & 1) p.w_bytes = 0;
#ifdef VK_STAMP
  { extern unsigned long long* g_vk_stamp_buf; p.stamps = g_vk_stamp_buf; }
#endif
  p.bnr_z = bnr ? bnr->z : nullptr;
  p.bnr_scale = bnr ? bnr->scale : nullptr;
  p.bnr_shift = bnr ? bnr->shift : nullptr;
  p.bnr_sums = bnr ? bnr->sums : nullptr;
  p.bnr_mask = bnr ? bnr->mask : nullptr;
  p.nchunks = c16 ? 1 : C / ck;
  if (p.bnr_mask && (c16 || s2 || s2d || pool2)) return VK_ERR_UNSUPPORTED;
  if (eb == 2 && !s2 && !s2d && !p.bnr_mask && (c16 || C == 32)) {
    const int rc = d->dtype == VK_BF16 ? stream_try<bf16_t>(p, st) : stream_try<f16_t>(p, st);
    if (rc != VK_ERR_UNSUPPORTED) return rc;
  }
  if (c16) {
    if (d->dtype == VK_BF16) return d->K >= 32 ? launch_c16<bf16_t, 32>(p, st) : launch_c16<bf16_t, 16>(p, st);
    return d->K >= 32 ? launch_c16<f16_t, 32>(p, st) : launch_c16<f16_t, 16>(p, st);
  }
  p.tiles_x = p.tiles_y = 0;
  if (s2d) {
    p.flip = 0;
    const long tiles = (long)d->N * ((d->H + 7) / 8) * ((d->W + 15) / 16);
    const bool wide = d->K % 128 == 0 && tiles * (d->K / 128) >= 256;
    switch (d->dtype) {
      case VK_F32: return wide ? launch_s2dg<float, 128>(p, st) : launch_s2dg<float, 64>(p, st);
      case VK_BF16: return wide ? launch_s2dg<bf16_t, 128>(p, st) : launch_s2dg<bf16_t, 64>(p, st);
      case VK_F16: return wide ? launch_s2dg<f16_t, 128>(p, st) : launch_s2dg<f16_t, 64>(p, st);
    }
    return VK_ERR_ARG;
  }
  if (s2) {
    p.slab = nullptr;
    p.slab_bytes = 0;
    switch (d->dtype) {
      case VK_F32: return launch_col<float, 8, 128, 2, 4, false, 1, 0, 2>(p, st);
      case VK_BF16: return launch_col<bf16_t, 8, 128, 2, 4, false, 1, 0, 2>(p, st);
      case VK_F16: return launch_col<f16_t, 8, 128, 2, 4, false, 1, 0, 2>(p, st);
    }
    return VK_ERR_ARG;
  }
  switch (d->dtype) {
    case VK_F32: return halo_select<float>(p, st);
    case VK_BF16: return halo_select<bf16_t>(p, st);
    case VK_F16: return halo_select<f16_t>(p, st);
// ... 14 lines not shown
```

### vickers-hardness-unet_amd/csrc/conv_igemm.hip

```cpp
#include <stdlib.h>

#include <string>

#include "vk_common.h"

namespace vk {

struct SrcDev {
  const void* ptr;
  const float* scale;
  const float* shift;
  int C, up, relu;
  uint32_t bytes;
};

struct ConvParams {
  SrcDev s0, s1;
  const void* w;
  uint32_t w_bytes;
  void* y0;
  void* y1;
  int ld0, ld1, split;
  double* stats;
  int N, H, W, Ho, Wo, K, R, S, slog, pad, transposed, accumulate;
// ... 420 lines not shown
  VK_CHECK_HIP(hipGetLastError());
  return VK_OK;
}

template <typename T, int MODE>
static int launch_bn(const ConvParams& p, hipStream_t st) {
  if (p.K >= 128) return launch_cfg<T, 128, 128, MODE>(p, st);
  if (p.K >= 64) return launch_cfg<T, 128, 64, MODE>(p, st);
  if (p.K >= 32) return launch_cfg<T, 128, 32, MODE>(p, st);
  return launch_cfg<T, 128, 16, MODE>(p, st);
}

template <typename T>
static int launch_mode(const ConvParams& p, int mode, hipStream_t st) {
  if (mode == 0) return launch_bn<T, 0>(p, st);
  if (mode == 1) {
    if (p.K >= 32) return launch_cfg<T, 128, 32, 1>(p, st);
    return launch_cfg<T, 128, 16, 1>(p, st);
  }
  return launch_cfg<T, 128, 64, 2>(p, st);
}

static int dispatch(vk_dtype dt, const ConvParams& p, int mode, hipStream_t st) {
  switch (dt) {
    case VK_F32: return launch_mode<float>(p, mode, st);
    case VK_BF16: return launch_mode<bf16_t>(p, mode, st);
    case VK_F16: return launch_mode<f16_t>(p, mode, st);
  }
  vkh::set_error("bad dtype %d", (int)dt);
  return VK_ERR_ARG;
}

int conv3x3_halo_try(const vk_conv_desc* d, const void* w, int packed, void* y, void* y1, int split_k1, int accumulate, double* stats,
                     int pool2, const vk_bnr* bnr, hipStream_t st, void* workspace, size_t workspace_bytes);
int halo_pack_impl(vk_dtype dt, int rows, int red, const void* src, void* dst, hipStream_t st);

static bool is_c16(const vk_conv_desc* d) {
  return d->dtype != VK_F32 && d->src0.C == 16 && !d->src1.ptr && !d->src0.up;
}

static bool halo_enabled() {
  return getenv("VK_NO_HALO") == nullptr;
}

int conv_fwd_impl(const vk_conv_desc* d, const void* w, int packed, void* y, void* y1, int split_k1, int accumulate,
                  double* stats, int pool2, const vk_bnr* bnr, hipStream_t st, void* workspace = nullptr, size_t workspace_bytes = 0) {
  VK_CHECK_ARG(d && w && y, "vk_conv_fwd: null argument");
  const int eb = d->dtype == VK_F32 ? 4 : 2;
  const int ve = 16 / eb;
  const int C = d->src0.C + (d->src1.ptr ? d->src1.C : 0);
  VK_CHECK_ARG(d->src0.ptr, "vk_conv_fwd: src0.ptr is null");
  VK_CHECK_ARG(d->stride == 1 || d->stride == 2, "vk_conv_fwd: stride %d unsupported", d->stride);
  VK_CHECK_ARG(d->K % ve == 0 && d->K >= 16, "vk_conv_fwd: K=%d must be a multiple of %d and >= 16", d->K, ve);
  VK_CHECK_ARG(!split_k1 || (y1 && split_k1 % ve == 0 && split_k1 < d->K), "vk_conv_fwd: bad split %d", split_k1);
  int mode;
  if (C % kBK == 0 && d->src0.C % kBK == 0) {
    mode = 0;
  } else {
    VK_CHECK_ARG(C == 16 && !d->src1.ptr, "vk_conv_fwd: C=%d unsupported (need multiple of 32, or 16 without concat)", C);
    mode = 1;
  }
  VK_CHECK_ARG(!d->src0.up || (d->H % 2 == 0 && d->W % 2 == 0), "vk_conv_fwd: upsampled source needs even H, W");
  VK_CHECK_ARG(!(d->src1.ptr && d->src1.up), "vk_conv_fwd: only src0 may be upsampled");
  if (halo_enabled()) {
    const int rc = conv3x3_halo_try(d, w, packed, y, y1, split_k1, accumulate, stats, pool2, bnr, st, workspace, workspace_bytes);
    if (rc != VK_ERR_UNSUPPORTED) return rc;
  }
  if (packed) {
    vkh::set_error("vk_conv_fwd_packed: shape not covered by the 3x3 stride-1 tile kernels (use vk_conv_fwd with plain weights)");
    return VK_ERR_UNSUPPORTED;
  }
  if (pool2 || bnr) {
    vkh::set_error("vk_conv_dgrad_fused: pooled / BN-fused outputs are only available on the 3x3 stride-1 tile kernels");
    return VK_ERR_UNSUPPORTED;
  }
  ConvParams p;
  p.s0 = make_src(d->src0, d->N, d->H, d->W, eb);
  if (d->src1.ptr) {
    p.s1 = make_src(d->src1, d->N, d->H, d->W, eb);
  } else {
    p.s1 = SrcDev{nullptr, nullptr, nullptr, 0, 0, 0, 0u};
  }
  const size_t in_bytes = (size_t)d->N * d->H * d->W * C * eb, out_bytes = (size_t)d->N * d->Ho * d->Wo * d->K * eb;
  VK_CHECK_ARG(in_bytes < (1ull << 31) && out_bytes < (1ull << 32), "vk_conv_fwd: tensor too large for 32-bit offsets");
  p.w = w;
  p.RS = d->R * d->S;
  p.RSC = p.RS * C;
  p.w_bytes = (uint32_t)((size_t)d->K * p.RSC * eb);
  p.y0 = y;
  p.y1 = y1;
  p.split = split_k1;
  p.ld0 = split_k1 ? split_k1 : d->K;
  p.ld1 = split_k1 ? d->K - split_k1 : 0;
  p.stats = stats;
  p.N = d->N; p.H = d->H; p.W = d->W; p.Ho = d->Ho; p.Wo = d->Wo; p.K = d->K; p.R = d->R; p.S = d->S;
  p.slog = d->stride == 2 ? 1 : 0;
  p.pad = d->pad;
  p.transposed = d->transposed;
  p.accumulate = accumulate;
// ... 33 lines not shown
  p.s1 = SrcDev{nullptr, nullptr, nullptr, 0, 0, 0, 0u};
  p.w = wp;
  p.RS = 7;
  p.RSC = 7 * 32;
  p.w_bytes = (uint32_t)(64 * p.RSC * eb);
  p.y0 = y; p.y1 = nullptr; p.split = 0; p.ld0 = 64; p.ld1 = 0;
  p.stats = stats;
  p.N = N; p.H = H; p.W = W; p.Ho = H / 2; p.Wo = W / 2; p.K = 64; p.R = 7; p.S = 1;
  p.slog = 1; p.pad = 3; p.transposed = 0; p.accumulate = 0;
  p.C = 32;
  p.M = N * p.Ho * p.Wo;
  p.nchunks = 7;
  p.log2C = 0;
  p.div_hw = vkh::make_fastdiv((uint32_t)(p.Ho * p.Wo));
  p.div_w = vkh::make_fastdiv((uint32_t)p.Wo);
  p.div_s = vkh::make_fastdiv(1);
  p.parity = 0;
  p.div_q = p.div_w2 = vkh::make_fastdiv(1);
  return dispatch(dt, p, 2, st);
}

}

extern "C" int vk_conv_fwd(const vk_conv_desc* d, const void* w, void* y, void* y1, int split_k1, int accumulate,
                           double* stats, void* stream) {
  return vk::conv_fwd_impl(d, w, 0, y, y1, split_k1, accumulate, stats, 0, nullptr, (hipStream_t)stream);
}

extern "C" int vk_conv_dgrad_pool2(const vk_conv_desc* d, const void* w, void* y_half, void* y1, int split_k1, int accumulate,
                                   void* stream) {
  return vk::conv_fwd_impl(d, w, vk::is_c16(d) ? 0 : 1, y_half, y1, split_k1, accumulate, nullptr, 1, nullptr, (hipStream_t)stream);
}

extern "C" int vk_conv_dgrad_fused(const vk_conv_desc* d, const void* w, void* y, void* y1, int split_k1, int pool2, const vk_bnr* bnr,
                                   void* stream) {
  VK_CHECK_ARG(!bnr || (bnr->z && bnr->sums && (bnr->mask || (bnr->scale && bnr->shift))), "vk_conv_dgrad_fused: incomplete vk_bnr");
  VK_CHECK_ARG(!bnr || !(bnr->mask && pool2), "vk_conv_dgrad_fused: the external mask does not combine with pool2");
  return vk::conv_fwd_impl(d, w, vk::is_c16(d) ? 0 : 1, y, y1, split_k1, bnr ? bnr->accumulate : 0, nullptr, pool2, bnr, (hipStream_t)stream);
}

extern "C" int vk_conv_fwd_packed(const vk_conv_desc* d, const void* w_halo, void* y, void* y1, int split_k1, int accumulate, double* stats,
                                  void* stream) {
  return vk::conv_fwd_impl(d, w_halo, 1, y, y1, split_k1, accumulate, stats, 0, nullptr, (hipStream_t)stream);
}

extern "C" int vk_conv_fwd_splitk(const vk_conv_desc* d, const void* w_halo, void* y, void* workspace, size_t workspace_bytes, void* stream) {
  return vk::conv_fwd_impl(d, w_halo, 1, y, nullptr, 0, 0, nullptr, 0, nullptr, (hipStream_t)stream, workspace, workspace_bytes);
}

extern "C" int vk_halo_pack(vk_dtype dtype, int rows, int red, const void* src, void* dst, void* stream) {
  return vk::halo_pack_impl(dtype, rows, red, src, dst, (hipStream_t)stream);
}

extern "C" int vk_conv_uses_halo_pack(const vk_conv_desc* d) {
  if (!d || d->R != 3 || d->S != 3 || d->pad != 1) return 0;
  const bool s2 = d->stride == 2 && !d->transposed && d->H == 2 * d->Ho && d->W == 2 * d->Wo && d->K >= 128 && !d->src0.up && !d->src1.ptr &&
                  !getenv("VK_NO_S2_TILE");
  const bool s2d = d->stride == 2 && d->transposed && d->Ho == 2 * d->H && d->Wo == 2 * d->W && d->K >= 64 && d->K % 64 == 0 && !d->src0.up &&
                   !d->src1.ptr && !d->src0.scale && !getenv("VK_NO_S2_TILE");
  if (s2d && (size_t)d->N * d->Ho * d->Wo * d->K * (d->dtype == VK_F32 ? 4 : 2) >= (1ull << 32)) return 0;
  if (!s2 && !s2d && (d->stride != 1 || d->H != d->Ho || d->W != d->Wo)) return 0;
  if (vk::is_c16(d)) return 0;
  const int ck = d->dtype == VK_F32 ? 16 : 32;
  if (d->src0.C % ck || (d->src1.ptr && (d->src1.C % ck || d->src1.up)) || d->K % 16) return 0;
  const size_t C = (size_t)d->src0.C + (d->src1.ptr ? d->src1.C : 0), px = (size_t)d->N * d->H * d->W;
  if (px * C * (d->dtype == VK_F32 ? 4 : 2) >= (1ull << 31) || px >= (1ull << 31)) return 0;
  return getenv("VK_NO_HALO") ? 0 : 1;
}

extern "C" int vk_stem_fwd(vk_dtype dtype, int N, int H, int W, const void* x4, const void* wp, void* y,
                           double* stats, void* stream) {
// ... 3 lines not shown
```

### vickers-hardness-unet_amd/csrc/elementwise.hip

```cpp
#include <math.h>

#include "vk_common.h"

namespace vk {

static inline int grid_for(size_t work_items, int block = 256, int max_blocks = 256 * 16) {
  size_t b = (work_items + block - 1) / block;
  if (b > (size_t)max_blocks) b = max_blocks;
  if (b < 1) b = 1;
  return (int)b;
}

constexpr int kWideC = 2048;
static inline int channel_grid(int blocks, int cv) {
  int g = cv, r = 256;
  while (r) { const int t = g % r; g = r; r = t; }
  const int m = cv / g;
  return (blocks + m - 1) / m * m;
}

template <typename T>
__global__ void k_input_transform(int N, int H, int W, const float* __restrict__ x, T* __restrict__ x4) {
  const size_t HW = (size_t)H * W;
  const float* xn = x + (size_t)blockIdx.y * 3 * HW;
// ... 127 lines not shown
        if (pw >= Wp) continue;
        const int s = w - (2 * pw - 1);
        const int code = r * 3 + s;
        const size_t pi = (((size_t)n * Hp + ph) * Wp + pw) * C + cv * VE;
        const uint8_t* ap = argmax + pi;
        uint8_t am[VE];
        if (VE == 8) {
          const u32x2_t q = *reinterpret_cast<const u32x2_t*>(ap);
#pragma unroll
          for (int j = 0; j < VE; ++j) am[j] = (uint8_t)((q[j >> 2] >> (8 * (j & 3))) & 0xff);
        } else {
          const uint32_t q = *reinterpret_cast<const uint32_t*>(ap);
#pragma unroll
          for (int j = 0; j < VE; ++j) am[j] = (uint8_t)((q >> (8 * j)) & 0xff);
        }
        float g[VE];
        Vec16<T>::unpack(*reinterpret_cast<const u32x4_t*>(dpool + pi), g);
#pragma unroll
        for (int j = 0; j < VE; ++j)
          if (am[j] == code) { acc[j] += g[j]; any = true; }
      }
    }
    if (any) {
      u32x4_t* dp = reinterpret_cast<u32x4_t*>(dy + i * VE);
      float o[VE];
      Vec16<T>::unpack(*dp, o);
#pragma unroll
      for (int j = 0; j < VE; ++j) o[j] += acc[j];
      *dp = Vec16<T>::pack(o);
    }
  }
}

template <typename T, int MAXC>
__global__ __launch_bounds__(256) void k_bn_add_relu(size_t pixels, int C, const T* __restrict__ z, const float* __restrict__ scale,
                                                     const float* __restrict__ shift, const T* __restrict__ res, const float* __restrict__ rscale,
                                                     const float* __restrict__ rshift, T* __restrict__ out) {
  constexpr int VE = ElemTraits<T>::kVec;
  constexpr int U = 4;
  const int CV = C / VE;
  const size_t total = pixels * CV;
  const size_t stride = (size_t)gridDim.x * blockDim.x;
  const size_t t0 = blockIdx.x * (size_t)blockDim.x + threadIdx.x;
  const int c0 = (int)(t0 % CV) * VE;
  __shared__ float cf[4][MAXC];
  for (int c = threadIdx.x; c < C; c += blockDim.x) {
    cf[0][c] = scale[c];
    cf[1][c] = shift[c];
    cf[2][c] = rscale ? rscale[c] : 1.f;
    cf[3][c] = rscale ? rshift[c] : 0.f;
  }
  __syncthreads();
  float sc[VE], sh[VE], rsc[VE], rsh[VE];
#pragma unroll
  for (int j = 0; j < VE; ++j) {
    sc[j] = cf[0][c0 + j];
    sh[j] = cf[1][c0 + j];
    rsc[j] = cf[2][c0 + j];
    rsh[j] = cf[3][c0 + j];
  }
  for (size_t i = t0; i < total; i += U * stride) {
    u32x4_t zv[U], rv[U];
#pragma unroll
    for (int u = 0; u < U; ++u) {
      const size_t k = i + u * stride;
      if (k < total) {
        zv[u] = *reinterpret_cast<const u32x4_t*>(z + k * VE);
        rv[u] = *reinterpret_cast<const u32x4_t*>(res + k * VE);
      }
    }
#pragma unroll
    for (int u = 0; u < U; ++u) {
      const size_t k = i + u * stride;
      if (k >= total) continue;
      float f[VE], r[VE];
      Vec16<T>::unpack(zv[u], f);
      Vec16<T>::unpack(rv[u], r);
#pragma unroll
      for (int j = 0; j < VE; ++j) f[j] = fmaxf(fmaf(f[j], sc[j], sh[j]) + fmaf(r[j], rsc[j], rsh[j]), 0.f);
      *reinterpret_cast<u32x4_t*>(out + k * VE) = Vec16<T>::pack(f);
    }
  }
}

constexpr int PB_ROWS = 16;
template <typename T>
__global__ __launch_bounds__(256) void k_maxpool_bwd_bn_reduce(int N, int H, int W, int C, const T* __restrict__ dpool,
                                                               const uint8_t* __restrict__ argmax, const T* __restrict__ z,
                                                               const float* __restrict__ scale, const float* __restrict__ shift,
                                                               T* __restrict__ dy, double* sums) {
  constexpr int VE = ElemTraits<T>::kVec;
  const int Hp = H / 2, Wp = W / 2, CV = C / VE;
  const int tid = threadIdx.x;
  const unsigned t = blockIdx.x * blockDim.x + tid;
  const bool active = t < (unsigned)(W * CV);
  const int w = active ? (int)(t / (unsigned)CV) : 0, cv = active ? (int)(t - (unsigned)w * CV) : 0;
  const int n = blockIdx.z;
  float sc[VE], sh[VE], s1[VE], s2[VE];
#pragma unroll
  for (int j = 0; j < VE; ++j) {
    sc[j] = scale[cv * VE + j];
    sh[j] = shift[cv * VE + j];
    s1[j] = 0.f;
    s2[j] = 0.f;
  }
  const int pw0 = (w & 1) ? (w - 1) / 2 : w / 2, npw = (w & 1) ? 2 : 1;
  if (active) {
    for (int hr = 0; hr < PB_ROWS; ++hr) {
      const int h = blockIdx.y * PB_ROWS + hr;
      if (h >= H) break;
      const size_t i = (((size_t)n * H + h) * W + w) * CV + cv;
      float g[VE], zf[VE];
      Vec16<T>::unpack(*reinterpret_cast<const u32x4_t*>(dy + i * VE), g);
// ... 49 lines not shown
  }
  __syncthreads();
  const int rows = 256 / CV;
  for (int c = tid; c < C; c += 256) {
    const int ccv = c / VE, cj = c % VE;
    double a = 0.0, b = 0.0;
    for (int r = 0; r < rows; ++r) {
      const int tt = r * CV + ccv;
      a += red[(tt * VE + cj) * 2];
      b += red[(tt * VE + cj) * 2 + 1];
    }
    double* sp = sums + (size_t)((blockIdx.x + blockIdx.y * gridDim.x) % VK_STATS_REPLICAS) * 2 * C;
    atomicAdd(sp + c, a);
    atomicAdd(sp + C + c, b);
  }
}

template <typename T, int MASK>
__device__ __forceinline__ void masked_grad(const T* dy, const T* z, const T* mask_src, size_t off, const float* sc,
                                            const float* sh, float* g, float* zf) {
  constexpr int VE = ElemTraits<T>::kVec;
  Vec16<T>::unpack(*reinterpret_cast<const u32x4_t*>(dy + off), g);
  Vec16<T>::unpack(*reinterpret_cast<const u32x4_t*>(z + off), zf);
  if (MASK == 1) {
#pragma unroll
    for (int j = 0; j < VE; ++j)
      if (!(fmaf(zf[j], sc[j], sh[j]) > 0.f)) g[j] = 0.f;
  } else if (MASK == 2) {
    float m[VE];
    Vec16<T>::unpack(*reinterpret_cast<const u32x4_t*>(mask_src + off), m);
#pragma unroll
    for (int j = 0; j < VE; ++j)
      if (!(m[j] > 0.f)) g[j] = 0.f;
  }
}

template <typename T, int MASK>
__global__ __launch_bounds__(256) void k_bn_bwd_reduce(size_t pixels, int C, const T* __restrict__ dy, const T* __restrict__ z,
                                                       const float* __restrict__ scale, const float* __restrict__ shift,
                                                       const T* __restrict__ mask_src, double* sums) {
  constexpr int VE = ElemTraits<T>::kVec;
  const int CV = C / VE;
  const int rows = 256 / CV;
  const int tid = threadIdx.x;
  const int cv = tid % CV, row = tid / CV;
  const bool active = row < rows;
  float sc[VE], sh[VE], s1[VE], s2[VE];
#pragma unroll
  for (int j = 0; j < VE; ++j) {
    sc[j] = (MASK == 1) ? scale[cv * VE + j] : 1.f;
    sh[j] = (MASK == 1) ? shift[cv * VE + j] : 0.f;
    s1[j] = 0.f;
    s2[j] = 0.f;
  }
  if (active) {
    const size_t stride = (size_t)gridDim.x * rows;
    size_t p = (size_t)blockIdx.x * rows + row;
    for (; p + 3 * stride < pixels; p += 4 * stride) {
      float g[4][VE], zf[4][VE];
#pragma unroll
      for (int u = 0; u < 4; ++u) masked_grad<T, MASK>(dy, z, mask_src, (p + u * stride) * C + cv * VE, sc, sh, g[u], zf[u]);
#pragma unroll
      for (int u = 0; u < 4; ++u)
#pragma unroll
        for (int j = 0; j < VE; ++j) { s1[j] += g[u][j]; s2[j] += g[u][j] * zf[u][j]; }
    }
// ... 941 lines not shown
extern "C" int vk_maxpool_bwd_bn_reduce(vk_dtype dtype, int N, int H, int W, int C, const void* dpool, const uint8_t* argmax, const void* z,
                                        const float* scale, const float* shift, void* dy, double* sums, void* stream) {
  VK_CHECK_ARG(dpool && argmax && z && scale && shift && dy && sums, "vk_maxpool_bwd_bn_reduce: null argument");
  VK_CHECK_ARG(H % 2 == 0 && W % 2 == 0 && C % 8 == 0, "vk_maxpool_bwd_bn_reduce: H, W even and C %% 8 == 0 required");
  const int cv = C / (dtype == VK_F32 ? 4 : 8);
  VK_CHECK_ARG(cv <= 256 && 256 % cv == 0, "vk_maxpool_bwd_bn_reduce: C=%d unsupported", C);
  VK_CHECK_ARG(N <= 65535 && H <= 65535 * vk::PB_ROWS, "vk_maxpool_bwd_bn_reduce: N or H too large for the launch grid");
  hipStream_t st = (hipStream_t)stream;
  const double eb = dtype == VK_F32 ? 4.0 : 2.0;
  vkh::ProfScope ps_("maxpool_bwd_bn_reduce", st, 0.0, (double)N * H * W * C * eb * 3.25 + (double)N * H * W * C / 4.0);
  DISPATCH_T(dtype, hipLaunchKernelGGL(k_maxpool_bwd_bn_reduce<T>, dim3((unsigned)((W * cv + 255) / 256), (unsigned)((H + PB_ROWS - 1) / PB_ROWS), (unsigned)N),
                                       dim3(256), 0, st, N, H, W, C, (const T*)dpool, argmax, (const T*)z, scale, shift, (T*)dy, sums));
  VK_CHECK_HIP(hipGetLastError());
  return VK_OK;
}

extern "C" int vk_bn_add_relu(vk_dtype dtype, size_t pixels, int C, const void* z, const float* scale, const float* shift,
                              const void* res, const float* rscale, const float* rshift, void* out, void* stream) {
  VK_CHECK_ARG(z && scale && shift && res && out, "vk_bn_add_relu: null argument");
  if (const int rc = check_flat_channels("vk_bn_add_relu", C)) return rc;
  hipStream_t st = (hipStream_t)stream;
  vkh::ProfScope ps_("bn_add_relu", st, 0.0, (double)pixels * C * (dtype == VK_F32 ? 4.0 : 2.0) * 3.0);
  if (C <= 512) {
    DISPATCH_T(dtype, hipLaunchKernelGGL((k_bn_add_relu<T, 512>), dim3(channel_grid(grid_for((pixels * (C / ElemTraits<T>::kVec) + 3) / 4), C / ElemTraits<T>::kVec)),
                                         dim3(256), 0, st, pixels, C, (const T*)z, scale, shift, (const T*)res, rscale, rshift, (T*)out));
  } else {
    DISPATCH_T(dtype, hipLaunchKernelGGL((k_bn_add_relu<T, kWideC>), dim3(channel_grid(grid_for((pixels * (C / ElemTraits<T>::kVec) + 3) / 4), C / ElemTraits<T>::kVec)),
                                         dim3(256), 0, st, pixels, C, (const T*)z, scale, shift, (const T*)res, rscale, rshift, (T*)out));
  }
  VK_CHECK_HIP(hipGetLastError());
  return VK_OK;
}

template <typename T>
static int launch_bn_bwd_reduce(size_t pixels, int C, const void* dy, const void* z, int mask_mode, const float* scale,
                                const float* shift, const void* mask_src, double* sums, hipStream_t st) {
  const int CV = C / ElemTraits<T>::kVec;
  if (CV > 256) {
    size_t nb = (pixels + 63) / 64;
    if (nb > 512) nb = 512;
    if (nb < 1) nb = 1;
#define VK_RW(M) hipLaunchKernelGGL((k_bn_bwd_reduce_wide<T, M>), dim3((unsigned)nb), dim3(256), 0, st, pixels, C, (const T*)dy, (const T*)z, scale, shift, (const T*)mask_src, sums)
    if (mask_mode == 0) VK_RW(0);
    else if (mask_mode == 1) VK_RW(1);
    else VK_RW(2);
#undef VK_RW
    return VK_OK;
  }
  const int rows = 256 / CV;
  size_t nb = (pixels + (size_t)rows * 16 - 1) / ((size_t)rows * 16);
  if (nb > 2048) nb = 2048;
  if (nb < 1) nb = 1;
  dim3 grid((unsigned)nb), block(256);
  if (mask_mode == 0) hipLaunchKernelGGL((k_bn_bwd_reduce<T, 0>), grid, block, 0, st, pixels, C, (const T*)dy, (const T*)z, scale, shift, (const T*)mask_src, sums);
  else if (mask_mode == 1) hipLaunchKernelGGL((k_bn_bwd_reduce<T, 1>), grid, block, 0, st, pixels, C, (const T*)dy, (const T*)z, scale, shift, (const T*)mask_src, sums);
  else hipLaunchKernelGGL((k_bn_bwd_reduce<T, 2>), grid, block, 0, st, pixels, C, (const T*)dy, (const T*)z, scale, shift, (const T*)mask_src, sums);
  return VK_OK;
}

extern "C" int vk_bn_bwd_reduce(vk_dtype dtype, size_t pixels, int C, const void* dy, const void* z, int mask_mode,
                                const float* scale, const float* shift, const void* mask_src, double* sums, void* stream) {
  VK_CHECK_ARG(dy && z && sums, "vk_bn_bwd_reduce: null argument");
  VK_CHECK_ARG(mask_mode >= 0 && mask_mode <= 2, "vk_bn_bwd_reduce: mask_mode %d", mask_mode);
  VK_CHECK_ARG(mask_mode != 1 || (scale && shift), "vk_bn_bwd_reduce: mask_mode 1 needs scale/shift");
  VK_CHECK_ARG(mask_mode != 2 || mask_src, "vk_bn_bwd_reduce: mask_mode 2 needs mask_src");
  if (const int rc = check_flat_channels("vk_bn_bwd_reduce", C)) return rc;
  hipStream_t st = (hipStream_t)stream;
  vkh::ProfScope ps_("bn_bwd_reduce", st, 0.0, (double)pixels * C * (dtype == VK_F32 ? 4.0 : 2.0) * (mask_mode == 2 ? 3.0 : 2.0));
  DISPATCH_T(dtype, launch_bn_bwd_reduce<T>(pixels, C, dy, z, mask_mode, scale, shift, mask_src, sums, st));
  VK_CHECK_HIP(hipGetLastError());
  return VK_OK;
}

extern "C" int vk_bn_bwd_coeffs(int C, const double* sums, double count, const float* gamma, const float* save_mean,
                                const float* save_invstd, float* dgamma, float* dbeta, float* coef_abc, void* stream) {
  VK_CHECK_ARG(sums && gamma && save_mean && save_invstd && dgamma && dbeta && coef_abc, "vk_bn_bwd_coeffs: null argument");
  vkh::ProfScope ps_("bn_bwd_coeffs", (hipStream_t)stream, 0.0, (double)C * 48.0);
  hipLaunchKernelGGL(k_bn_bwd_coeffs, dim3((C + 7) / 8), dim3(256), 0, (hipStream_t)stream, C, sums, count, gamma, save_mean,
                     save_invstd, dgamma, dbeta, coef_abc);
  VK_CHECK_HIP(hipGetLastError());
  return VK_OK;
}

extern "C" int vk_bn_bwd_coeffs_frozen(int C, const double* sums, const float* gamma, const float* running_mean, const float* running_invstd,
                                       float* dgamma, float* dbeta, float* coef_abc, void* stream) {
  VK_CHECK_ARG(sums && gamma && running_mean && running_invstd && dgamma && dbeta && coef_abc, "vk_bn_bwd_coeffs_frozen: null argument");
  vkh::ProfScope ps_("bn_bwd_coeffs_frozen", (hipStream_t)stream, 0.0, (double)C * 48.0);
  hipLaunchKernelGGL(k_bn_bwd_coeffs_frozen, dim3((C + 7) / 8), dim3(256), 0, (hipStream_t)stream, C, sums, gamma, running_mean,
                     running_invstd, dgamma, dbeta, coef_abc);
  VK_CHECK_HIP(hipGetLastError());
  return VK_OK;
}

struct BnApplyArgs {
  size_t pixels; int C; const void* dy; const void* z; int mask_mode; const float* scale; const float* shift; const void* mask_src;
  const float* coef; const double* sums; double count; const float* gamma; const float* mean; const float* invstd; float* dgamma; float* dbeta;
  void* dz; void* g_out; int g_acc;
};

template <typename T>
static int launch_bn_bwd_apply(const BnApplyArgs& a, hipStream_t st) {
  const int CV = a.C / ElemTraits<T>::kVec;
  const bool wide = a.C > 512;
  dim3 grid(channel_grid(grid_for(a.pixels * CV / 2 + 1), CV)), block(256);
  if (wide) {
#define VK_APPLY_W(M) hipLaunchKernelGGL((k_bn_bwd_apply<T, M, kWideC>), grid, block, 0, st, a.pixels, a.C, (const T*)a.dy, (const T*)a.z, a.scale, \
    a.shift, (const T*)a.mask_src, a.coef, a.sums, a.count, a.gamma, a.mean, a.invstd, a.dgamma, a.dbeta, (T*)a.dz, (T*)a.g_out, a.g_acc)
    if (a.mask_mode == 0) VK_APPLY_W(0);
    else if (a.mask_mode == 1) VK_APPLY_W(1);
    else VK_APPLY_W(2);
#undef VK_APPLY_W
    return VK_OK;
  }
#define VK_APPLY(M) hipLaunchKernelGGL((k_bn_bwd_apply<T, M, 512>), grid, block, 0, st, a.pixels, a.C, (const T*)a.dy, (const T*)a.z, a.scale, a.shift, \
    (const T*)a.mask_src, a.coef, a.sums, a.count, a.gamma, a.mean, a.invstd, a.dgamma, a.dbeta, (T*)a.dz, (T*)a.g_out, a.g_acc)
  if (a.mask_mode == 0) VK_APPLY(0);
  else if (a.mask_mode == 1) VK_APPLY(1);
  else VK_APPLY(2);
#undef VK_APPLY
  return VK_OK;
}

static int bn_bwd_apply_common(vk_dtype dtype, const BnApplyArgs& a, void* stream) {
  VK_CHECK_ARG(a.dy && a.z && a.dz && (a.coef || (a.sums && a.gamma && a.mean && a.invstd && a.dgamma && a.dbeta)), "vk_bn_bwd_apply: null argument");
  VK_CHECK_ARG(a.mask_mode >= 0 && a.mask_mode <= 2, "vk_bn_bwd_apply: mask_mode %d", a.mask_mode);
  VK_CHECK_ARG(a.mask_mode != 1 || (a.scale && a.shift), "vk_bn_bwd_apply: mask_mode 1 needs scale/shift");
  VK_CHECK_ARG(a.mask_mode != 2 || a.mask_src, "vk_bn_bwd_apply: mask_mode 2 needs mask_src");
  if (const int rc = check_flat_channels("vk_bn_bwd_apply", a.C)) return rc;
  hipStream_t st = (hipStream_t)stream;
  vkh::ProfScope ps_("bn_bwd_apply", st, 0.0, (double)a.pixels * a.C * (dtype == VK_F32 ? 4.0 : 2.0) * ((a.mask_mode == 2 ? 4.0 : 3.0) + (a.g_out ? (a.g_acc ? 2.0 : 1.0) : 0.0)));
  DISPATCH_T(dtype, launch_bn_bwd_apply<T>(a, st));
  VK_CHECK_HIP(hipGetLastError());
  return VK_OK;
}

extern "C" int vk_bn_bwd_apply(vk_dtype dtype, size_t pixels, int C, const void* dy, const void* z, int mask_mode,
                               const float* scale, const float* shift, const void* mask_src, const float* coef_abc, void* dz,
                               void* g_out, int g_accumulate, void* stream) {
  VK_CHECK_ARG(coef_abc, "vk_bn_bwd_apply: null coefficients");
  BnApplyArgs a{pixels, C, dy, z, mask_mode, scale, shift, mask_src, coef_abc, nullptr, 1.0, nullptr, nullptr, nullptr, nullptr, nullptr, dz, g_out, g_accumulate};
  return bn_bwd_apply_common(dtype, a, stream);
}

extern "C" int vk_bn_bwd_apply_fused(vk_dtype dtype, size_t pixels, int C, const void* dy, const void* z, int mask_mode,
                                     const float* scale, const float* shift, const void* mask_src, const double* sums, double count,
                                     const float* gamma, const float* save_mean, const float* save_invstd, float* dgamma, float* dbeta,
                                     void* dz, void* g_out, int g_accumulate, void* stream) {
  BnApplyArgs a{pixels, C, dy, z, mask_mode, scale, shift, mask_src, nullptr, sums, count, gamma, save_mean, save_invstd, dgamma, dbeta, dz, g_out, g_accumulate};
  return bn_bwd_apply_common(dtype, a, stream);
}

extern "C" int vk_upsample2x_bwd(vk_dtype dtype, int N, int H, int W, int C, const void* d_up, void* d_low, int accumulate,
                                 void* stream) {
  VK_CHECK_ARG(d_up && d_low && H % 2 == 0 && W % 2 == 0 && C % 8 == 0, "vk_upsample2x_bwd: bad argument");
  hipStream_t st = (hipStream_t)stream;
  vkh::ProfScope ps_("upsample2x_bwd", st, 0.0, (double)N * H * W * C * (dtype == VK_F32 ? 4.0 : 2.0) * 1.25);
  DISPATCH_T(dtype, hipLaunchKernelGGL(k_upsample2x_bwd<T>, dim3(grid_for((size_t)N * (H / 2) * (W / 2) * (C / ElemTraits<T>::kVec))),
                                       dim3(256), 0, st, N, H, W, C, (const T*)d_up, (T*)d_low, accumulate));
  VK_CHECK_HIP(hipGetLastError());
  return VK_OK;
}

extern "C" int vk_head_fwd(vk_dtype dtype, int N, int H, int W, const vk_src* src, const float* w9x16, const float* bias,
// ... 191 lines not shown
```

### vickers-hardness-unet_amd/csrc/engine.hip

```cpp
#include <stdarg.h>
#include <stdio.h>
#include <stdlib.h>
#include <string.h>

#include <algorithm>
#include <atomic>
#include <map>
#include <mutex>
#include <string>
#include <vector>

#include "vk_common.h"

namespace vkh {
static thread_local char g_err[512] = "";
void set_error(const char* fmt, ...) {
  va_list ap;
  va_start(ap, fmt);
  vsnprintf(g_err, sizeof(g_err), fmt, ap);
  va_end(ap);
}

struct ProfRec {
  std::string tag;
// ... 290 lines not shown
  int Win, Wout;
  bool pw = false;
  int w_t = -1, b_t = -1;
  int rank = 0;
  char* z = nullptr;
  char* g = nullptr;
};

struct BnL {
  std::string name;
  int C;
  int64_t g_off, b_off, rm_off, rv_off;
  int idx;
  int g_t = -1, b_t = -1;
  int rank = 0;
  double count;
  double* stats = nullptr;
  double* bsums = nullptr;
  float* scale = nullptr;
  float* shift = nullptr;
  float* mean = nullptr;
  float* invstd = nullptr;
  float* coef = nullptr;
  int64_t arena_off = 0;
};

struct BlockL {
  int conv1, conv2, convd;
  int conv3 = -1;
  int Cin, C, stride, Hin, Hout, Win, Wout;
  bool in_has_grad_first;
  char* out = nullptr;
  char* gout = nullptr;
};

struct DecL {
  int conv1, conv2;
  int Cup, Cskip, Cout, H, W;
};

struct Act {
  const void* ptr;
  int C;
  const float* scale;
  const float* shift;
  int relu;
};

}

using namespace vk;

constexpr int kMaxStages = 16;
constexpr int kMaxBatch = 40;
constexpr size_t kEngineSlabBytes = 176u << 20;
constexpr size_t kGradScratchFloats = 2048;
constexpr int kMaxBnLayers = 64;

struct EncoderTopo {
  int code;
  int nblocks[4];
  bool bottleneck;
  int nstages;
  int stage_blocks[8][2];
};
static const EncoderTopo kEncoders[] = {
// ... 1 lines not shown
    {VK_ENC_RESNET34, {3, 4, 6, 3}, false, 7, {{15, 15}, {14, 14}, {13, 13}, {12, 10}, {9, 7}, {6, 3}, {2, 0}}},
    {VK_ENC_RESNET50, {3, 4, 6, 3}, true, 7, {{15, 15}, {14, 14}, {13, 13}, {12, 10}, {9, 7}, {6, 3}, {2, 0}}},
};
static const EncoderTopo* find_encoder(int code) {
  for (const EncoderTopo& e : kEncoders)
    if (e.code == code) return &e;
  return nullptr;
}

struct vk_unet {
  vk_unet_config cfg;
  int classes = 1;
  const EncoderTopo* enc = nullptr;
  int sink_c = 512;
  int eb;
  std::vector<vk_tensor_info> infos;
  int n_ptensors = 0;
  std::vector<uint8_t> trainable;
  int last_rank = 0;
  uint64_t bn_frozen = 0, bn_frozen_fwd = 0;
  float* dx_in = nullptr;
  int input_rank = 0;
  unsigned mask_version = 0;
  std::vector<ConvL> convs;
  std::vector<BnL> bns;
  std::vector<BlockL> blocks;
  std::vector<DecL> decs;
  int stem_conv = -1, head_conv = -1;
  int layer_last_block[4];
  int64_t n_params = 0, n_bufs = 0, n_dgrad = 0;
  int64_t head_w_off = 0, head_b_off = 0;
  std::vector<std::pair<int64_t, int64_t>> buckets;
  size_t ws_bytes = 0;
  size_t off_x4 = 0, off_pool = 0, off_argmax = 0, off_gpool = 0, off_dup = 0, off_dlogits = 0, off_loss_sums = 0;
  size_t off_stats = 0, off_bsums = 0, stats_bytes = 0, off_farena = 0, farena_floats = 0, off_wf = 0, off_wd = 0, off_wstem = 0;
  size_t off_tab_pack = 0, off_tab_bn = 0, off_wslab = 0, off_wh = 0, off_tab_halo = 0, off_splitk = 0, splitk_bytes = 0;
  std::vector<HaloPackEntry> halo_tab;
  std::vector<size_t> off_z, off_g, off_out, off_gout;
  std::vector<char> g_prereduced;
  std::vector<char> tail_prereduced;
  float* params = nullptr;
  float* grads = nullptr;
  float* bufs = nullptr;
  int64_t* nbt = nullptr;
  char* ws = nullptr;
  bool bound = false;
  hipStream_t side = nullptr;
  hipEvent_t ev_fork = nullptr, ev_join = nullptr;
  bool side_dirty = false;
  struct WItem {
    vk_conv_desc d;
    const void* dz;
    float* dw;
  };
  struct WPlan {
    bool built = false;
    int target = 0, n = 0;
    unsigned version = 0;
    vk::WgradBatchPlan plan;
  };
  std::vector<WItem> pending;
  WPlan wplans[kMaxStages][2];
  size_t off_tab_wbatch = 0;
  std::vector<PackEntry> pack_tab;
  std::vector<CastRange> cast_tab;
  size_t off_tab_cast = 0;
// ... 255 lines not shown
    h->off_dlogits = take((size_t)N * h->classes * S * SW * 4);
  }
  h->off_loss_sums = take(8 * sizeof(double));
  size_t st = 0, fl = 0;
  for (BnL& b : h->bns) {
    st += 2 * (size_t)b.C * sizeof(double) * VK_STATS_REPLICAS;
    b.arena_off = (int64_t)fl;
    fl += 7 * (size_t)b.C;
  }
  h->stats_bytes = st;
  h->off_stats = take(st);
  h->off_bsums = take(st);
  h->farena_floats = fl;
  h->off_farena = take(fl * sizeof(float));
  h->off_wf = (eb == 4) ? 0 : take((size_t)h->n_params * eb);
  h->off_wd = tr ? take((size_t)h->n_dgrad * eb) : 0;
  h->off_wh = take((size_t)h->n_params * eb);
  h->off_tab_halo = take(2 * h->convs.size() * sizeof(HaloPackEntry));
  h->off_wstem = take(64 * 7 * 32 * eb);
  h->off_wslab = tr ? take(kEngineSlabBytes) : 0;
  h->off_tab_wbatch = tr ? take((size_t)kMaxStages * 2 * VK_WGRAD_BATCH_TABLE_BYTES) : 0;
  h->splitk_bytes = (!tr && (size_t)N * S * SW <= 4u * 512 * 512) ? VK_SPLITK_WORKSPACE_BYTES : 0;
  h->off_splitk = h->splitk_bytes ? take(h->splitk_bytes) : 0;
  h->off_tab_pack = take(h->convs.size() * sizeof(PackEntry));
  h->off_tab_cast = take(h->convs.size() * sizeof(CastRange));
  h->off_tab_bn = take(h->bns.size() * sizeof(BnEvalEntry));
  h->off_gscratch = tr ? take(grad_scratch_floats(h) * sizeof(float)) : 0;
  if (h->classes > 1) {
    h->mloss_bytes = vk_multi_loss_workspace_bytes(N, h->classes, S * SW);
    h->off_mloss = take(h->mloss_bytes);
  }
  h->sloss_bytes = vk_seg_loss_workspace_bytes(N, h->classes, S * SW);
  h->off_sloss = take(h->sloss_bytes);
  h->ws_bytes = off;
}

void assign_pointers(vk_unet* h) {
  char* ws = h->ws;
  h->debug.clear();
  const int N = h->cfg.N;
  for (size_t i = 0; i < h->convs.size(); ++i) {
    ConvL& c = h->convs[i];
    if ((int)i == h->head_conv) continue;
    c.z = ws + h->off_z[i];
    c.g = h->cfg.training ? ws + h->off_g[i] : nullptr;
    h->debug["z:" + c.name] = {c.z, {N, c.Hout, c.Wout, c.K}};
    if (c.g) h->debug["g:" + c.name] = {c.g, {N, c.Hout, c.Wout, c.K}};
  }
  for (size_t b = 0; b < h->blocks.size(); ++b) {
    BlockL& k = h->blocks[b];
    k.out = ws + h->off_out[b];
    k.gout = h->cfg.training ? ws + h->off_gout[b] : nullptr;
    const std::string nm = h->convs[k.conv1].name.substr(0, h->convs[k.conv1].name.size() - 6);
    h->debug["out:" + nm] = {k.out, {N, k.Hout, k.Wout, k.C}};
    if (k.gout) h->debug["gout:" + nm] = {k.gout, {N, k.Hout, k.Wout, k.C}};
  }
  const int S = h->cfg.size, SW = h->cfg.width;
  h->debug["x4"] = {ws + h->off_x4, {N, S, SW, 4}};
  h->debug["pool"] = {ws + h->off_pool, {N, S / 4, SW / 4, 64}};
  if (h->cfg.training) {
    h->debug["gpool"] = {ws + h->off_gpool, {N, S / 4, SW / 4, 64}};
    if (h->classes == 1) h->debug["dlogits"] = {ws + h->off_dlogits, {N, S, SW, 1}};
    else h->debug["dlogits"] = {ws + h->off_dlogits, {N, h->classes, S, SW}};
  }
  double* sp = (double*)(ws + h->off_stats);
  double* bp = (double*)(ws + h->off_bsums);
  float* fa = (float*)(ws + h->off_farena);
  for (BnL& b : h->bns) {
    b.stats = sp;
    b.bsums = bp;
    sp += 2 * b.C * VK_STATS_REPLICAS;
    bp += 2 * b.C * VK_STATS_REPLICAS;
    float* f = fa + b.arena_off;
    b.scale = f;
    b.shift = f + b.C;
    b.mean = f + 2 * b.C;
    b.invstd = f + 3 * b.C;
    b.coef = f + 4 * b.C;
    h->debug["scale:" + b.name] = {b.scale, {b.C}};
    h->debug["shift:" + b.name] = {b.shift, {b.C}};
  }
}

const void* fwd_weights(const vk_unet* h, const ConvL& c) {
  if (c.halo_fwd) return h->ws + h->off_wh + (size_t)c.w_off * h->eb;
// ... 335 lines not shown
  const int N = h->cfg.N, S = h->cfg.size, SW = h->cfg.width;
  const vk_dtype dt = h->cfg.dtype;
  if (training) {
    h->bn_frozen_fwd = h->bn_frozen;
    VK_CHECK_HIP(hipMemsetAsync(h->ws + h->off_stats, 0, h->stats_bytes, st));
    if (h->bn_frozen_fwd) {
      hipLaunchKernelGGL(k_bn_frozen_affine, dim3((unsigned)h->bns.size()), dim3(128), 0, st, (const BnEvalEntry*)(h->ws + h->off_tab_bn),
                         h->bn_frozen_fwd, h->params, h->bufs, (float*)(h->ws + h->off_farena), 1e-5f);
      VK_CHECK_HIP(hipGetLastError());
    }
  } else {
    hipLaunchKernelGGL(k_bn_eval_all, dim3((unsigned)h->bns.size()), dim3(128), 0, st, (const BnEvalEntry*)(h->ws + h->off_tab_bn),
                       h->params, h->bufs, (float*)(h->ws + h->off_farena), 1e-5f);
    VK_CHECK_HIP(hipGetLastError());
  }
  void* x4 = h->ws + h->off_x4;
  RET_IF(vk_input_transform(dt, N, S, SW, x, x4, st));
  ConvL& stem = h->convs[h->stem_conv];
  BnL& sbn = h->bns[stem.bn];
  RET_IF(vk_stem_fwd(dt, N, S, SW, x4, h->ws + h->off_wstem, stem.z, training && !frozen(h, sbn) ? sbn.stats : nullptr, st));
  RET_IF(finalize_bn(h, sbn, training, st));
  void* pool = h->ws + h->off_pool;
  RET_IF(vk_bn_relu_maxpool(dt, N, S / 2, SW / 2, 64, stem.z, sbn.scale, sbn.shift, pool, (uint8_t*)(h->ws + h->off_argmax), st));
  Act cur{pool, 64, nullptr, nullptr, 0};
  for (BlockL& k : h->blocks) {
    ConvL& c1 = h->convs[k.conv1];
    ConvL& c2 = h->convs[k.conv2];
    RET_IF(run_conv(h, c1, to_src(cur), null_src(), training, st));
    RET_IF(run_conv(h, c2, to_src(bn_act(h, c1)), null_src(), training, st));
    ConvL& ct = k.conv3 >= 0 ? h->convs[k.conv3] : c2;
    if (k.conv3 >= 0) RET_IF(run_conv(h, ct, to_src(bn_act(h, c2)), null_src(), training, st));
    const BnL& b2 = h->bns[ct.bn];
    const size_t pixels = (size_t)N * k.Hout * k.Wout;
    if (k.convd >= 0) {
      ConvL& cd = h->convs[k.convd];
      RET_IF(run_conv(h, cd, to_src(cur), null_src(), training, st));
      const BnL& bd = h->bns[cd.bn];
      RET_IF(vk_bn_add_relu(dt, pixels, k.C, ct.z, b2.scale, b2.shift, cd.z, bd.scale, bd.shift, k.out, st));
    } else {
      RET_IF(vk_bn_add_relu(dt, pixels, k.C, ct.z, b2.scale, b2.shift, cur.ptr, nullptr, nullptr, k.out, st));
    }
    cur = Act{k.out, k.C, nullptr, nullptr, 0};
  }
  Act skips[5];
  for (int i = 0; i < 3; ++i) {
    const BlockL& fb = h->blocks[h->layer_last_block[2 - i]];
    skips[i] = Act{fb.out, fb.C, nullptr, nullptr, 0};
  }
  skips[3] = bn_act(h, stem);
  skips[4] = Act{nullptr, 0, nullptr, nullptr, 0};
  Act xd = cur;
  for (size_t i = 0; i < h->decs.size(); ++i) {
    DecL& d = h->decs[i];
    ConvL& c1 = h->convs[d.conv1];
    ConvL& c2 = h->convs[d.conv2];
    const bool small_plan = (size_t)N * S * SW <= 4u * 512 * 512;
    if (!training && h->classes == 1 && i + 1 == h->decs.size() && dt != VK_F32 && !d.Cskip && d.Cup == 32 && c1.K == 16 && c2.K == 16 && c1.halo_fwd &&
        !c2.halo_fwd && S % 16 == 0 && SW % 16 == 0 && !getenv("VK_NO_TAIL_FUSION") && (small_plan || getenv("VK_TAIL_FUSION"))) {
      const vk_src s0 = to_src(xd, 1);
      const BnL& b1 = h->bns[c1.bn];
      const BnL& b2 = h->bns[c2.bn];
      return vk_dec4_tail_eval(dt, N, S, SW, &s0, fwd_weights(h, c1), b1.scale, b1.shift, fwd_weights(h, c2), b2.scale, b2.shift,
                               h->params + h->head_w_off, h->params + h->head_b_off, logits, st);
    }
    RET_IF(run_conv(h, c1, to_src(xd, 1), d.Cskip ? to_src(skips[i]) : null_src(), training, st));
    RET_IF(run_conv(h, c2, to_src(bn_act(h, c1)), null_src(), training, st));
    xd = bn_act(h, c2);
  }
  vk_src hs = to_src(xd);
  if (h->classes == 1) RET_IF(vk_head_fwd(dt, N, S, SW, &hs, h->params + h->head_w_off, h->params + h->head_b_off, logits, st));
  else RET_IF(vk_head_fwd_multi(dt, N, S, SW, h->classes, &hs, h->params + h->head_w_off, h->params + h->head_b_off, logits, st));
  if (training) {
    if (h->bn_frozen_fwd) hipLaunchKernelGGL(k_inc_i64_masked, dim3(1), dim3(64), 0, st, (int)h->bns.size(), h->nbt, h->bn_frozen_fwd);
    else hipLaunchKernelGGL(k_inc_i64, dim3(1), dim3(64), 0, st, (int)h->bns.size(), h->nbt);
// ... 226 lines not shown
    if (trains(h, c2.w_t)) RET_IF(conv_wgrad(h, c2, to_src(bn_act(h, c1)), null_src(), st));
  }
  if (i > 0) h->g_prereduced[h->decs[i - 1].conv2] = 0;
  if (!into1) return VK_OK;
  int onepass1 = 0;
  if (fused1 && i > 0 && !d.Cskip && trains(h, c1.w_t) && need_from(h, c1.rank + 1) && h->cfg.dtype != VK_F32 && !h->side && !on_1x1(c1) &&
      !getenv("VK_NO_ONEPASS") && !getenv("VK_NO_ONEPASS_UP") && !getenv("VK_NO_BNR_FUSION"))
    RET_IF(conv_bwd_onepass(h, c1, h->convs[h->decs[i - 1].conv2], 1, &onepass1, st));
  if (onepass1 == 1) {
    h->g_prereduced[h->decs[i - 1].conv2] = 1;
    return VK_OK;
  }
  if (onepass1 == 0) RET_IF(bn_relu_bwd_inplace(h, c1, fused1, st));
  if (need_from(h, c1.rank + 1)) {
    vk_conv_desc dd = dgrad_desc(h, c1);
    vk_bnr r;
    const bool want_bnr = i > 0 && !getenv("VK_NO_BNR_FUSION");
    if (want_bnr) r = bnr_of(h, h->convs[h->decs[i - 1].conv2]);
    const int rc = vk_conv_dgrad_fused(&dd, dgrad_weights(h, c1), g_prev, d.Cskip ? g_skip : nullptr, d.Cskip ? d.Cup : 0, 1,
                                       want_bnr ? &r : nullptr, st);
    if (rc == VK_OK && want_bnr) h->g_prereduced[h->decs[i - 1].conv2] = 1;
    if (rc != VK_OK && rc != VK_ERR_UNSUPPORTED) return rc;
    if (rc == VK_ERR_UNSUPPORTED) {
      void* dup = h->ws + h->off_dup;
      if (d.Cskip) RET_IF(conv_dgrad(h, c1, dup, g_skip, d.Cup, 0, st));
      else RET_IF(conv_dgrad(h, c1, dup, nullptr, 0, 0, st));
      RET_IF(vk_upsample2x_bwd(h->cfg.dtype, N, d.H, d.W, d.Cup, dup, g_prev, 0, st));
    }
  }
  if (!trains(h, c1.w_t)) return VK_OK;
  return conv_wgrad(h, c1, to_src(xprev, 1), d.Cskip ? to_src(skip) : null_src(), st);
}

int backward_block(vk_unet* h, int bi, hipStream_t st) {
  BlockL& k = h->blocks[bi];
  ConvL& c1 = h->convs[k.conv1];
  ConvL& c2 = h->convs[k.conv2];
  BnL& b2 = h->bns[c2.bn];
  const vk_dtype dt = h->cfg.dtype;
  const size_t pixels = (size_t)h->cfg.N * k.Hout * k.Wout;
  if (!need_from(h, b2.rank)) {
    h->tail_prereduced[(size_t)bi] = 0;
    return VK_OK;
  }
  Act xin;
  void* gin;
  if (bi == 0) {
    xin = Act{h->ws + h->off_pool, 64, nullptr, nullptr, 0};
    gin = h->ws + h->off_gpool;
  } else {
    BlockL& pb = h->blocks[bi - 1];
    xin = Act{pb.out, pb.C, nullptr, nullptr, 0};
    gin = pb.gout;
  }
  const bool pre = h->tail_prereduced[(size_t)bi] != 0;
  h->tail_prereduced[(size_t)bi] = 0;
  if (bi > 0) h->tail_prereduced[(size_t)bi - 1] = 0;
  const int mm = pre ? 0 : 2;
  if (!pre && bn_sums_needed(h, b2)) RET_IF(vk_bn_bwd_reduce(dt, pixels, k.C, k.gout, c2.z, 2, nullptr, nullptr, k.out, b2.bsums, st));
  if (k.convd < 0) {
    RET_IF(bn_bwd_phase2(h, b2, k.C, pixels, k.gout, c2.z, mm, k.out, c2.g, gin, k.in_has_grad_first ? 1 : 0, st));
  } else {
    ConvL& cd = h->convs[k.convd];
    BnL& bd = h->bns[cd.bn];
    RET_IF(bn_bwd_phase2(h, b2, k.C, pixels, k.gout, c2.z, mm, k.out, c2.g, nullptr, 0, st));
    if (bn_sums_needed(h, bd)) RET_IF(vk_bn_bwd_reduce(dt, pixels, k.C, k.gout, cd.z, mm, nullptr, nullptr, k.out, bd.bsums, st));
    RET_IF(bn_bwd_phase2(h, bd, k.C, pixels, k.gout, cd.z, mm, k.out, cd.g, nullptr, 0, st));
  }
  const bool into1 = need_from(h, h->bns[c1.bn].rank);
  bool fused1 = false;
  if (into1) RET_IF(conv_dgrad_into(h, c2, c1, &fused1, st));
  if (trains(h, c2.w_t)) RET_IF(conv_wgrad(h, c2, to_src(bn_act(h, c1)), null_src(), st));
  if (!into1) return k.convd >= 0 && trains(h, h->convs[k.convd].w_t) ? conv_wgrad(h, h->convs[k.convd], to_src(xin), null_src(), st) : VK_OK;
  RET_IF(bn_relu_bwd_inplace(h, c1, fused1, st));
  const bool into_gin = need_from(h, c1.rank + 1);
  bool tail_fused = false;
  const int tail_maxc = getenv("VK_TAIL_BNR_MAXC") ? atoi(getenv("VK_TAIL_BNR_MAXC")) : 1 << 20;
  if (into_gin && k.convd < 0 && bi > 0 && c1.halo_dg && k.C <= tail_maxc && !getenv("VK_NO_TAIL_BNR_FUSION")) {
    BlockL& pb = h->blocks[bi - 1];
    ConvL& pc2 = h->convs[pb.conv2];
    vk_conv_desc dd = dgrad_desc(h, c1);
    vk_bnr r;
    r.z = pc2.z; r.scale = nullptr; r.shift = nullptr; r.sums = h->bns[pc2.bn].bsums; r.mask = pb.out; r.accumulate = 1;
    const int rc = vk_conv_dgrad_fused(&dd, dgrad_weights(h, c1), gin, nullptr, 0, 0, &r, st);
    if (rc == VK_OK) { tail_fused = true; h->tail_prereduced[(size_t)bi - 1] = 1; }
    else if (rc != VK_ERR_UNSUPPORTED) return rc;
  }
  if (into_gin && !tail_fused) RET_IF(conv_dgrad(h, c1, gin, nullptr, 0, 1, st));
  if (k.convd >= 0) {
    ConvL& cd = h->convs[k.convd];
    if (into_gin) RET_IF(conv_dgrad(h, cd, gin, nullptr, 0, 1, st));
    if (trains(h, c1.w_t)) RET_IF(conv_wgrad(h, c1, to_src(xin), null_src(), st));
    return trains(h, cd.w_t) ? conv_wgrad(h, cd, to_src(xin), null_src(), st) : VK_OK;
  }
  return trains(h, c1.w_t) ? conv_wgrad(h, c1, to_src(xin), null_src(), st) : VK_OK;
}

int backward_bottleneck(vk_unet* h, int bi, hipStream_t st) {
  BlockL& k = h->blocks[bi];
  ConvL& c1 = h->convs[k.conv1];
  ConvL& c2 = h->convs[k.conv2];
  ConvL& c3 = h->convs[k.conv3];
  BnL& b3 = h->bns[c3.bn];
  const vk_dtype dt = h->cfg.dtype;
  const size_t pixels = (size_t)h->cfg.N * k.Hout * k.Wout;
  h->tail_prereduced[(size_t)bi] = 0;
  if (!need_from(h, b3.rank)) return VK_OK;
  Act xin;
  void* gin;
  if (bi == 0) {
    xin = Act{h->ws + h->off_pool, 64, nullptr, nullptr, 0};
    gin = h->ws + h->off_gpool;
  } else {
    BlockL& pb = h->blocks[bi - 1];
    xin = Act{pb.out, pb.C, nullptr, nullptr, 0};
    gin = pb.gout;
  }
  bool gin_written = k.in_has_grad_first;
  if (bn_sums_needed(h, b3)) RET_IF(vk_bn_bwd_reduce(dt, pixels, k.C, k.gout, c3.z, 2, nullptr, nullptr, k.out, b3.bsums, st));
// ... 171 lines not shown
```

Before: 3109.

## Store ReLU masks as bitmaps and alias the residual gradient into the fused dgrad epilogue

In the ResNet encoder's basic-block tails, the forward bn_add_relu now also writes a 1-bit-per-element ReLU mask. Backward BN reduce, apply and the fused dgrad epilogue read that bitmap (mask_mode 3) instead of the full bf16 block output, which cuts mask traffic. When the tail is prereduced and fused, the identity-residual gradient is no longer written into gin by BN apply. The dgrad epilogue instead reads it directly from gout through a new acc_src pointer, saving a read-modify-write pass. The cost is an extra template instantiation per conv kernel, extra workspace for the bitmaps, and a hard error if the tile kernel declines a case that tail_fusable accepted.

Measured after the change: 3127 (median of 6 runs). Within noise of the previous version (+0.6%).

```diff
diff --git a/include/vk_unet.h b/include/vk_unet.h
--- a/include/vk_unet.h
+++ b/include/vk_unet.h
@@ -72,6 +72,13 @@
 
 int vk_conv_dgrad_fused(const vk_conv_desc* d, const void* w, void* y, void* y1, int split_k1, int pool2, const vk_bnr* bnr,
                         void* stream);
+
+typedef struct {
+  const void* acc_src;
+  const void* mask_bits;
+} vk_dgrad_ext;
+int vk_conv_dgrad_fused_ex(const vk_conv_desc* d, const void* w, void* y, void* y1, int split_k1, int pool2, const vk_bnr* bnr,
+                           const vk_dgrad_ext* ext, void* stream);
 
 int vk_conv1x1_fwd(const vk_conv_desc* d, const void* w, void* y, int accumulate, double* stats, void* stream);
 int vk_conv1x1_wgrad(const vk_conv_desc* d, const void* dz, float* dw, void* workspace, size_t workspace_bytes, void* stream);
@@ -236,6 +243,8 @@
 
 int vk_bn_add_relu(vk_dtype dtype, size_t pixels, int C, const void* z, const float* scale, const float* shift,
                    const void* res, const float* rscale, const float* rshift, void* out, void* stream);
+int vk_bn_add_relu_bits(vk_dtype dtype, size_t pixels, int C, const void* z, const float* scale, const float* shift,
+                        const void* res, const float* rscale, const float* rshift, void* out, uint8_t* bits, void* stream);
 
 int vk_bn_bwd_reduce(vk_dtype dtype, size_t pixels, int C, const void* dy, const void* z, int mask_mode,
                      const float* scale, const float* shift, const void* mask_src, double* sums, void* stream);
diff --git a/vickers-hardness-unet_amd/_lib.py b/vickers-hardness-unet_amd/_lib.py
--- a/vickers-hardness-unet_amd/_lib.py
+++ b/vickers-hardness-unet_amd/_lib.py
@@ -37,6 +37,10 @@
 class vk_bnr(C.Structure):
     _fields_ = [("z", C.c_void_p), ("scale", C.c_void_p), ("shift", C.c_void_p), ("sums", C.c_void_p), ("mask", C.c_void_p),
                 ("accumulate", C.c_int)]
+
+
+class vk_dgrad_ext(C.Structure):
+    _fields_ = [("acc_src", C.c_void_p), ("mask_bits", C.c_void_p)]
 
 
 class vk_letterbox_desc(C.Structure):
@@ -163,6 +167,7 @@
     "vk_conv_fwd": (ci, [P(vk_conv_desc), vp, vp, vp, ci, ci, vp, vp]),
     "vk_conv_dgrad_pool2": (ci, [P(vk_conv_desc), vp, vp, vp, ci, ci, vp]),
     "vk_conv_dgrad_fused": (ci, [P(vk_conv_desc), vp, vp, vp, ci, ci, P(vk_bnr), vp]),
+    "vk_conv_dgrad_fused_ex": (ci, [P(vk_conv_desc), vp, vp, vp, ci, ci, P(vk_bnr), P(vk_dgrad_ext), vp]),
     "vk_head_bwd_fused": (ci, [ci, ci, ci, ci, P(vk_src), vp, vp, vp, vp, vp, P(vk_bnr), vp, sz, vp]),
     "vk_halo_pack": (ci, [ci, ci, ci, vp, vp, vp]),
     "vk_conv_uses_halo_pack": (ci, [P(vk_conv_desc)]),
@@ -202,6 +207,7 @@
     "vk_maxpool_bwd": (ci, [ci, ci, ci, ci, ci, vp, vp, vp, vp]),
     "vk_maxpool_bwd_bn_reduce": (ci, [ci, ci, ci, ci, ci, vp, vp, vp, vp, vp, vp, vp, vp]),
     "vk_bn_add_relu": (ci, [ci, sz, ci, vp, vp, vp, vp, vp, vp, vp, vp]),
+    "vk_bn_add_relu_bits": (ci, [ci, sz, ci, vp, vp, vp, vp, vp, vp, vp, vp, vp]),
     "vk_bn_bwd_reduce": (ci, [ci, sz, ci, vp, vp, ci, vp, vp, vp, vp, vp]),
     "vk_bn_bwd_coeffs": (ci, [ci, vp, cd, vp, vp, vp, vp, vp, vp, vp]),
     "vk_bn_bwd_coeffs_frozen": (ci, [ci, vp, vp, vp, vp, vp, vp, vp, vp]),
diff --git a/vickers-hardness-unet_amd/csrc/conv_halo.hip b/vickers-hardness-unet_amd/csrc/conv_halo.hip
--- a/vickers-hardness-unet_amd/csrc/conv_halo.hip
+++ b/vickers-hardness-unet_amd/csrc/conv_halo.hip
@@ -43,6 +43,7 @@
   uint32_t w_bytes;
   void* y0;
   void* y1;
+  const void* acc0;
   int ld0, ld1, split;
   double* stats;
   int N, H, W, K, C, flip, accumulate, pool2;
@@ -59,6 +60,7 @@
   const float* bnr_shift;
   double* bnr_sums;
   const void* bnr_mask;
+  const uint8_t* bnr_bits;
 };
 
 template <typename T, int TH, int BN, int WGM, int WGN>
@@ -99,7 +101,7 @@
 }
 
 
-template <typename T, int TH, int BN, int TP, int TC, int NT = 256, bool PRE = false, int OS = 1>
+template <typename T, int TH, int BN, int TP, int TC, int NT = 256, bool PRE = false, int OS = 1, bool EXT = false>
 __device__ __forceinline__ void halo_epilogue(char* smem, f32x4_t (&acc)[TC][TP], const HaloParams& p, int n, int y0, int x0, int n0,
                                               int wrow0, int wch0, int py = 0, int px = 0, double* defer = nullptr) {
   using Tr = ElemTraits<T>;
@@ -117,14 +119,16 @@
   const int col0 = n0 + e_vec * VE;
   const bool col_ok = col0 < p.K;
   char* yb = (char*)p.y0;
+  const char* ab = EXT ? (const char*)p.acc0 : yb;
   int ld = p.ld0, colx = col0;
   bool first_part = true;
-  if (p.split > 0 && col0 >= p.split) { yb = (char*)p.y1; ld = p.ld1; colx = col0 - p.split; first_part = false; }
+  if (p.split > 0 && col0 >= p.split) { yb = (char*)p.y1; ab = yb; ld = p.ld1; colx = col0 - p.split; first_part = false; }
   float s1[VE], s2[VE];
 #pragma unroll
   for (int j = 0; j < VE; ++j) { s1[j] = 0.f; s2[j] = 0.f; }
   const bool bnr = p.bnr_z != nullptr && first_part && col_ok;
-  const bool ext_mask = p.bnr_mask != nullptr;
+  const bool bit_mask = EXT && EB == 2 && p.bnr_bits != nullptr;
+  const bool ext_mask = p.bnr_mask != nullptr || bit_mask;
   float bsc[VE], bsh[VE];
   if (bnr && !ext_mask) {
 #pragma unroll
@@ -134,7 +138,7 @@
     u32x4_t* gp = reinterpret_cast<u32x4_t*>(yb + elem_off * EB);
     if (p.accumulate) {
       float o[VE];
-      Vec16<T>::unpack(pre_old ? *pre_old : *gp, o);
+      Vec16<T>::unpack(pre_old ? *pre_old : *reinterpret_cast<const u32x4_t*>(ab + elem_off * EB), o);
 #pragma unroll
       for (int j = 0; j < VE; ++j) f[j] += o[j];
     }
@@ -143,7 +147,12 @@
     if (bnr) {
       float zf[VE];
       Vec16<T>::unpack(pre_z ? *pre_z : *reinterpret_cast<const u32x4_t*>((const char*)p.bnr_z + elem_off * EB), zf);
-      if (ext_mask) {
+      if (bit_mask) {
+        const unsigned m = pre_m ? (*pre_m)[0] : (unsigned)p.bnr_bits[elem_off / VE];
+#pragma unroll
+        for (int j = 0; j < VE; ++j)
+          if (!((m >> j) & 1u)) f[j] = 0.f;
+      } else if (ext_mask) {
         float mf[VE];
         Vec16<T>::unpack(pre_m ? *pre_m : *reinterpret_cast<const u32x4_t*>((const char*)p.bnr_mask + elem_off * EB), mf);
 #pragma unroll
@@ -180,9 +189,10 @@
       if (PRE_M) mv[ps] = u32x4_t{0, 0, 0, 0};
       if (y < p.H && x < p.W && col_ok) {
         const size_t eoff = (((size_t)n * p.H + y) * p.W + x) * ld + colx;
-        if (p.accumulate) oldv[ps] = *reinterpret_cast<const u32x4_t*>(yb + eoff * EB);
+        if (p.accumulate) oldv[ps] = *reinterpret_cast<const u32x4_t*>(ab + eoff * EB);
         if (bnr) zv[ps] = *reinterpret_cast<const u32x4_t*>((const char*)p.bnr_z + eoff * EB);
-        if (PRE_M && bnr && ext_mask) mv[ps] = *reinterpret_cast<const u32x4_t*>((const char*)p.bnr_mask + eoff * EB);
+        if (PRE_M && bnr && bit_mask) mv[ps][0] = p.bnr_bits[eoff / VE];
+        else if (PRE_M && bnr && ext_mask) mv[ps] = *reinterpret_cast<const u32x4_t*>((const char*)p.bnr_mask + eoff * EB);
       }
     }
   };
@@ -332,7 +342,7 @@
   d[1] = 0.0;
 }
 
-template <typename T, int TH, int BN, int WGM, int WGN>
+template <typename T, int TH, int BN, int WGM, int WGN, bool EXT = false>
 __global__ __launch_bounds__(256, 2) void conv3x3_halo_kernel(const HaloParams p) {
   using Cfg = HaloCfg<T, TH, BN, WGM, WGN>;
   constexpr int EB = Cfg::EB, VE = Cfg::VE, CK = Cfg::CK, HPIX = Cfg::HPIX, NPV = Cfg::NPV, NBV = Cfg::NBV;
@@ -528,7 +538,7 @@
   unsigned long long te0, te1;
   VK_T(te0)
 #endif
-  halo_epilogue<T, TH, BN, TP, TC>(smem, acc, p, n, y0, x0, n0, wrow0, wch0);
+  halo_epilogue<T, TH, BN, TP, TC, 256, false, 1, EXT>(smem, acc, p, n, y0, x0, n0, wrow0, wch0);
 #ifdef VK_STAMP
   VK_T(te1)
   if (p.stamps && lane == 0) {
@@ -570,7 +580,7 @@
   static_assert(EPI >= BM * ESB + ESLOTS * BN * 8, "epilogue partial-sum slots must fit behind the output tile");
 };
 
-template <typename T, int TH, int BN, int WGM, int WGN, bool ADB, int MINW, int STR = 1>
+template <typename T, int TH, int BN, int WGM, int WGN, bool ADB, int MINW, int STR = 1, bool EXT = false>
 __global__ __launch_bounds__(64 * WGM * WGN, MINW) void conv3x3_col_kernel(const HaloParams p) {
   using Cfg = ColCfg<T, TH, BN, WGM, WGN, ADB, STR>;
   constexpr int EB = Cfg::EB, VE = Cfg::VE, CK = Cfg::CK, HPIX = Cfg::HPIX, NPV = Cfg::NPV, NT = Cfg::NT, NW = Cfg::NW;
@@ -792,7 +802,7 @@
       }
     return;
   }
-  halo_epilogue<T, TH, BN, TP, TC, NT, (BN <= 64 && TH == 16)>(smem, acc, p, n, y0, x0, n0, wrow0, wch0);
+  halo_epilogue<T, TH, BN, TP, TC, NT, (BN <= 64 && TH == 16), 1, EXT>(smem, acc, p, n, y0, x0, n0, wrow0, wch0);
 #ifdef VK_STAMP
   VK_T(te1)
   if (p.stamps && lane == 0) {
@@ -967,7 +977,7 @@
   static_assert(SMEM <= 160 * 1024, "LDS image exceeds the 160 KiB of a CU");
 };
 
-template <typename T, int TH, int BN, int WGM, int WGN>
+template <typename T, int TH, int BN, int WGM, int WGN, bool EXT = false>
 __global__ __launch_bounds__(64 * WGM * WGN, 1) void conv3x3_colq_kernel(const HaloParams p) {
   using Cfg = ColqCfg<T, TH, BN, WGM, WGN>;
   constexpr int EB = Cfg::EB, VE = Cfg::VE, CK = Cfg::CK, HPIX = Cfg::HPIX, NPV = Cfg::NPV, NT = Cfg::NT, NW = Cfg::NW;
@@ -1210,7 +1220,7 @@
       }
     return;
   }
-  halo_epilogue<T, TH, BN, TP, TC, NT, ((VK_COLQ_PRE && sizeof(T) == 2) || (BN <= 64 && TH == 16))>(smem, acc, p, n, y0, x0, n0, wrow0, wch0);
+  halo_epilogue<T, TH, BN, TP, TC, NT, ((VK_COLQ_PRE && sizeof(T) == 2) || (BN <= 64 && TH == 16)), 1, EXT>(smem, acc, p, n, y0, x0, n0, wrow0, wch0);
 }
 
 template <typename T, int TH, int BN, int WGM, int WGN>
@@ -1224,7 +1234,7 @@
   static_assert(SMEM <= 160 * 1024, "LDS image exceeds the 160 KiB of a CU");
 };
 
-template <typename T, int TH, int BN, int WGM, int WGN>
+template <typename T, int TH, int BN, int WGM, int WGN, bool EXT = false>
 __global__ __launch_bounds__(64 * WGM * WGN, 1) void conv3x3_cols_kernel(const HaloParams p) {
   using Cfg = ColsCfg<T, TH, BN, WGM, WGN>;
   constexpr int EB = Cfg::EB, VE = Cfg::VE, CK = Cfg::CK, HPIX = Cfg::HPIX, NPV = Cfg::NPV, NT = Cfg::NT, NW = Cfg::NW;
@@ -1467,10 +1477,10 @@
       }
     return;
   }
-  halo_epilogue<T, TH, BN, TP, TC, NT, (BN <= 64 && TH == 16)>(smem, acc, p, n, y0, x0, n0, wrow0, wch0);
-}
-
-template <typename T, int TH, int BN, int WGM, int WGN, int MINW>
+  halo_epilogue<T, TH, BN, TP, TC, NT, (BN <= 64 && TH == 16), 1, EXT>(smem, acc, p, n, y0, x0, n0, wrow0, wch0);
+}
+
+template <typename T, int TH, int BN, int WGM, int WGN, int MINW, bool EXT = false>
 __global__ __launch_bounds__(64 * WGM * WGN, MINW) void conv3x3_colp_kernel(const HaloParams p) {
   using Cfg = ColCfg<T, TH, BN, WGM, WGN, false>;
   constexpr int EB = Cfg::EB, VE = Cfg::VE, CK = Cfg::CK, HPIX = Cfg::HPIX, NPV = Cfg::NPV, NT = Cfg::NT, NW = Cfg::NW;
@@ -1656,7 +1666,7 @@
     stage(p.nchunks - 1, I1{}, std::true_type{});
     stage(p.nchunks - 1, I2{}, std::true_type{});
     constexpr bool DEFER = VK_COLP_DEFER_STATS && (sizeof(T) == 2 || BN < 64);
-    halo_epilogue<T, TH, BN, TP, TC, NT, (BN <= 64 && TH == 16)>(smem, acc, p, g.n, g.y0, g.x0, g.n0, wrow0, wch0, 0, 0, DEFER ? dsum : nullptr);
+    halo_epilogue<T, TH, BN, TP, TC, NT, (BN <= 64 && TH == 16), 1, EXT>(smem, acc, p, g.n, g.y0, g.x0, g.n0, wrow0, wch0, 0, 0, DEFER ? dsum : nullptr);
     if (DEFER && (!more_tiles || gn.n0 != g.n0)) stats_flush<BN>(p, g.n0, dsum);
     if (!more_tiles) break;
     __syncthreads();
@@ -1753,6 +1763,7 @@
   p.w = wp;
   p.w_bytes = 64u * 7u * 32u * 2u;
   p.y0 = y;
+  p.acc0 = y;
   p.ld0 = 64;
   p.stats = stats;
   p.N = N; p.H = H / 2; p.W = W / 2; p.K = 64; p.C = 4;
@@ -2413,17 +2424,23 @@
   return VK_OK;
 }
 
+static bool tail_ext(const HaloParams& p) { return p.acc0 != p.y0 || p.bnr_bits != nullptr; }
+static const char* tail_tag(const HaloParams& p) {
+  return p.acc0 != p.y0 ? (p.bnr_bits ? "+acc+bits" : "+acc") : (p.bnr_bits ? "+bits" : "");
+}
+
 template <typename T, int TH, int BN, int WGM, int WGN>
 static int launch_halo(HaloParams p, hipStream_t st) {
   using Cfg = HaloCfg<T, TH, BN, WGM, WGN>;
   p.tiles_x = (p.W + 15) / 16;
   p.tiles_y = (p.H + TH - 1) / TH;
   dim3 grid((unsigned)(p.N * p.tiles_y * p.tiles_x), (unsigned)((p.K + BN - 1) / BN), 1);
-  static bool attr_done = false;
-  if (!attr_done && Cfg::SMEM > 64 * 1024) {
-    VK_CHECK_HIP(hipFuncSetAttribute((const void*)conv3x3_halo_kernel<T, TH, BN, WGM, WGN>,
-                                     hipFuncAttributeMaxDynamicSharedMemorySize, Cfg::SMEM));
-    attr_done = true;
+  const bool ext = tail_ext(p);
+  const void* const kernel = ext ? (const void*)conv3x3_halo_kernel<T, TH, BN, WGM, WGN, true> : (const void*)conv3x3_halo_kernel<T, TH, BN, WGM, WGN>;
+  static bool attr_done[2] = {false, false};
+  if (!attr_done[ext] && Cfg::SMEM > 64 * 1024) {
+    VK_CHECK_HIP(hipFuncSetAttribute(kernel, hipFuncAttributeMaxDynamicSharedMemorySize, Cfg::SMEM));
+    attr_done[ext] = true;
   }
   {
     static const std::string tag_f = std::string("halo_") + (sizeof(T) == 4 ? "f32" : "16b") + "_t" + std::to_string(TH) + "_bn" + std::to_string(BN);
@@ -2431,9 +2448,10 @@
     const double macs = (double)p.N * p.H * p.W * p.K * 9.0 * p.C;
     const double bytes = ((double)p.N * p.H * p.W * (p.C + p.K) + 9.0 * p.K * p.C) * sizeof(T);
     const std::string& btag = p.flip ? tag_d : tag_f;
-    const std::string dtag = getenv("VK_PROF_DETAIL") ? btag + ":H" + std::to_string(p.H) + "_K" + std::to_string(p.K) + "_C" + std::to_string(p.C) : btag;
+    const std::string dtag = (getenv("VK_PROF_DETAIL") ? btag + ":H" + std::to_string(p.H) + "_K" + std::to_string(p.K) + "_C" + std::to_string(p.C) : btag) + tail_tag(p);
     vkh::ProfScope ps(dtag.c_str(), st, 2.0 * macs, bytes);
-    hipLaunchKernelGGL((conv3x3_halo_kernel<T, TH, BN, WGM, WGN>), grid, dim3(256), Cfg::SMEM, st, p);
+    void* args[] = {(void*)&p};
+    VK_CHECK_HIP(hipLaunchKernel(kernel, grid, dim3(256), args, Cfg::SMEM, st));
   }
   VK_CHECK_HIP(hipGetLastError());
   return VK_OK;
@@ -2457,24 +2475,33 @@
 template <int PIPE, typename T, int TH, int BN, int WGM, int WGN, bool ADB, int MINW, int STR>
 struct ColLaunch {
   using Cfg = ColCfg<T, TH, BN, WGM, WGN, ADB, STR>;
-  static const void* kernel() { return (const void*)conv3x3_col_kernel<T, TH, BN, WGM, WGN, ADB, MINW, STR>; }
+  static const void* kernel(bool ext) {
+    if constexpr (STR == 1)
+      if (ext) return (const void*)conv3x3_col_kernel<T, TH, BN, WGM, WGN, ADB, MINW, 1, true>;
+    return (const void*)conv3x3_col_kernel<T, TH, BN, WGM, WGN, ADB, MINW, STR>;
+  }
 };
 template <typename T, int TH, int BN, int WGM, int WGN, bool ADB, int MINW>
 struct ColLaunch<1, T, TH, BN, WGM, WGN, ADB, MINW, 1> {
   using Cfg = ColqCfg<T, TH, BN, WGM, WGN>;
-  static const void* kernel() { return (const void*)conv3x3_colq_kernel<T, TH, BN, WGM, WGN>; }
+  static const void* kernel(bool ext) {
+    return ext ? (const void*)conv3x3_colq_kernel<T, TH, BN, WGM, WGN, true> : (const void*)conv3x3_colq_kernel<T, TH, BN, WGM, WGN>;
+  }
 };
 template <typename T, int TH, int BN, int WGM, int WGN, bool ADB, int MINW>
 struct ColLaunch<2, T, TH, BN, WGM, WGN, ADB, MINW, 1> {
   using Cfg = ColsCfg<T, TH, BN, WGM, WGN>;
-  static const void* kernel() { return (const void*)conv3x3_cols_kernel<T, TH, BN, WGM, WGN>; }
+  static const void* kernel(bool ext) {
+    return ext ? (const void*)conv3x3_cols_kernel<T, TH, BN, WGM, WGN, true> : (const void*)conv3x3_cols_kernel<T, TH, BN, WGM, WGN>;
+  }
 };
 
 template <typename T, int TH, int BN, int WGM, int WGN, bool ADB, int MINW, int PIPE = 0, int STR = 1>
 static int launch_col(HaloParams p, hipStream_t st) {
   using Sel = ColLaunch<PIPE, T, TH, BN, WGM, WGN, ADB, MINW, STR>;
   using Cfg = typename Sel::Cfg;
-  const void* const kernel = Sel::kernel();
+  const bool ext = tail_ext(p);
+  const void* const kernel = Sel::kernel(ext);
   p.tiles_x = (p.W + 15) / 16;
   p.tiles_y = (p.H + TH - 1) / TH;
   dim3 grid((unsigned)(p.N * p.tiles_y * p.tiles_x), (unsigned)((p.K + BN - 1) / BN), 1);
@@ -2500,10 +2527,10 @@
     const bool wst = km ? km[0] == 'w' : (size_t)p.w_bytes >= (3u << 20);
     if (PIPE && wst && 8 % p.kyn == 0 && (grid.x / 8) * (8 / p.kyn) * p.kyn == grid.x) p.kyn = -p.kyn;
   }
-  static bool attr_done = false;
-  if (!attr_done && Cfg::SMEM > 64 * 1024) {
+  static bool attr_done[2] = {false, false};
+  if (!attr_done[ext] && Cfg::SMEM > 64 * 1024) {
     VK_CHECK_HIP(hipFuncSetAttribute(kernel, hipFuncAttributeMaxDynamicSharedMemorySize, Cfg::SMEM));
-    attr_done = true;
+    attr_done[ext] = true;
   }
   {
     static const std::string tag_f = std::string(PIPE == 2 ? "cols_" : PIPE == 1 ? "colq_" : "col_") + (sizeof(T) == 4 ? "f32" : "16b") + "_t" + std::to_string(TH) + "_bn" +
@@ -2512,7 +2539,7 @@
     const double macs = (double)p.N * p.H * p.W * p.K * 9.0 * p.C;
     const double bytes = ((double)p.N * ((double)p.Hi * p.Wi * p.C + (double)p.H * p.W * p.K) + 9.0 * p.K * p.C) * sizeof(T);
     const std::string& btag = p.flip ? tag_d : tag_f;
-    const std::string dtag = getenv("VK_PROF_DETAIL") ? btag + ":H" + std::to_string(p.H) + "_K" + std::to_string(p.K) + "_C" + std::to_string(p.C) : btag;
+    const std::string dtag = (getenv("VK_PROF_DETAIL") ? btag + ":H" + std::to_string(p.H) + "_K" + std::to_string(p.K) + "_C" + std::to_string(p.C) : btag) + tail_tag(p);
     vkh::ProfScope ps(dtag.c_str(), st, 2.0 * macs, bytes);
     void* args[] = {(void*)&p};
     VK_CHECK_HIP(hipLaunchKernel(kernel, grid, dim3(Cfg::NT), args, Cfg::SMEM, st));
@@ -2539,11 +2566,12 @@
   long g = 256L * per_cu;
   if (const char* e = getenv("VK_COL_PERSIST_GRID")) g = atol(e) > 0 ? atol(e) : g;
   if (g > total) g = total;
-  static bool attr_done = false;
-  if (!attr_done && Cfg::SMEM > 64 * 1024) {
-    VK_CHECK_HIP(hipFuncSetAttribute((const void*)conv3x3_colp_kernel<T, TH, BN, WGM, WGN, MINW>,
-                                     hipFuncAttributeMaxDynamicSharedMemorySize, Cfg::SMEM));
-    attr_done = true;
+  const bool ext = tail_ext(p);
+  const void* const kernel = ext ? (const void*)conv3x3_colp_kernel<T, TH, BN, WGM, WGN, MINW, true> : (const void*)conv3x3_colp_kernel<T, TH, BN, WGM, WGN, MINW>;
+  static bool attr_done[2] = {false, false};
+  if (!attr_done[ext] && Cfg::SMEM > 64 * 1024) {
+    VK_CHECK_HIP(hipFuncSetAttribute(kernel, hipFuncAttributeMaxDynamicSharedMemorySize, Cfg::SMEM));
+    attr_done[ext] = true;
   }
   {
     static const std::string tag_f = std::string("col_") + (sizeof(T) == 4 ? "f32" : "16b") + "_t" + std::to_string(TH) + "_bn" + std::to_string(BN) +
@@ -2552,9 +2580,10 @@
     const double macs = (double)p.N * p.H * p.W * p.K * 9.0 * p.C;
     const double bytes = ((double)p.N * p.H * p.W * (p.C + p.K) + 9.0 * p.K * p.C) * sizeof(T);
     const std::string& btag = p.flip ? tag_d : tag_f;
-    const std::string dtag = getenv("VK_PROF_DETAIL") ? btag + ":H" + std::to_string(p.H) + "_K" + std::to_string(p.K) + "_C" + std::to_string(p.C) : btag;
+    const std::string dtag = (getenv("VK_PROF_DETAIL") ? btag + ":H" + std::to_string(p.H) + "_K" + std::to_string(p.K) + "_C" + std::to_string(p.C) : btag) + tail_tag(p);
     vkh::ProfScope ps(dtag.c_str(), st, 2.0 * macs, bytes);
-    hipLaunchKernelGGL((conv3x3_colp_kernel<T, TH, BN, WGM, WGN, MINW>), dim3((unsigned)g), dim3(Cfg::NT), Cfg::SMEM, st, p);
+    void* args[] = {(void*)&p};
+    VK_CHECK_HIP(hipLaunchKernel(kernel, dim3((unsigned)g), dim3(Cfg::NT), args, Cfg::SMEM, st));
   }
   VK_CHECK_HIP(hipGetLastError());
   return VK_OK;
@@ -2698,7 +2727,7 @@
 }
 
 int conv3x3_halo_try(const vk_conv_desc* d, const void* w, int packed, void* y, void* y1, int split_k1, int accumulate, double* stats,
-                     int pool2, const vk_bnr* bnr, hipStream_t st, void* workspace, size_t workspace_bytes) {
+                     int pool2, const vk_bnr* bnr, hipStream_t st, void* workspace, size_t workspace_bytes, const void* acc_src, const void* mask_bits) {
   const bool s2 = d->stride == 2 && !d->transposed && d->H == 2 * d->Ho && d->W == 2 * d->Wo && d->K >= 128 && !d->src0.up && !d->src1.ptr &&
                   !pool2 && !bnr && !accumulate && !split_k1 && !getenv("VK_NO_S2_TILE");
   const bool s2d = d->stride == 2 && d->transposed && d->Ho == 2 * d->H && d->Wo == 2 * d->W && d->K >= 64 && d->K % 64 == 0 && !d->src0.up &&
@@ -2729,6 +2758,7 @@
   p.w = w;
   p.w_bytes = (uint32_t)((size_t)d->K * 9 * C * eb);
   p.y0 = y; p.y1 = y1; p.split = split_k1;
+  p.acc0 = acc_src ? acc_src : y;
   p.ld0 = split_k1 ? split_k1 : d->K;
   p.ld1 = split_k1 ? d->K - split_k1 : 0;
   p.stats = stats;
@@ -2752,9 +2782,11 @@
   p.bnr_shift = bnr ? bnr->shift : nullptr;
   p.bnr_sums = bnr ? bnr->sums : nullptr;
   p.bnr_mask = bnr ? bnr->mask : nullptr;
+  p.bnr_bits = bnr ? (const uint8_t*)mask_bits : nullptr;
+  if (p.bnr_bits && eb != 2) return VK_ERR_UNSUPPORTED;
   p.nchunks = c16 ? 1 : C / ck;
-  if (p.bnr_mask && (c16 || s2 || s2d || pool2)) return VK_ERR_UNSUPPORTED;
-  if (eb == 2 && !s2 && !s2d && !p.bnr_mask && (c16 || C == 32)) {
+  if ((p.bnr_mask || p.bnr_bits || acc_src) && (c16 || s2 || s2d || pool2)) return VK_ERR_UNSUPPORTED;
+  if (eb == 2 && !s2 && !s2d && !p.bnr_mask && !p.bnr_bits && !acc_src && (c16 || C == 32)) {
     const int rc = d->dtype == VK_BF16 ? stream_try<bf16_t>(p, st) : stream_try<f16_t>(p, st);
     if (rc != VK_ERR_UNSUPPORTED) return rc;
   }
diff --git a/vickers-hardness-unet_amd/csrc/conv_igemm.hip b/vickers-hardness-unet_amd/csrc/conv_igemm.hip
--- a/vickers-hardness-unet_amd/csrc/conv_igemm.hip
+++ b/vickers-hardness-unet_amd/csrc/conv_igemm.hip
@@ -476,7 +476,7 @@
 }
 
 int conv3x3_halo_try(const vk_conv_desc* d, const void* w, int packed, void* y, void* y1, int split_k1, int accumulate, double* stats,
-                     int pool2, const vk_bnr* bnr, hipStream_t st, void* workspace, size_t workspace_bytes);
+                     int pool2, const vk_bnr* bnr, hipStream_t st, void* workspace, size_t workspace_bytes, const void* acc_src, const void* mask_bits);
 int halo_pack_impl(vk_dtype dt, int rows, int red, const void* src, void* dst, hipStream_t st);
 
 static bool is_c16(const vk_conv_desc* d) {
@@ -488,7 +488,8 @@
 }
 
 int conv_fwd_impl(const vk_conv_desc* d, const void* w, int packed, void* y, void* y1, int split_k1, int accumulate,
-                  double* stats, int pool2, const vk_bnr* bnr, hipStream_t st, void* workspace = nullptr, size_t workspace_bytes = 0) {
+                  double* stats, int pool2, const vk_bnr* bnr, hipStream_t st, void* workspace = nullptr, size_t workspace_bytes = 0,
+                  const void* acc_src = nullptr, const void* mask_bits = nullptr) {
   VK_CHECK_ARG(d && w && y, "vk_conv_fwd: null argument");
   const int eb = d->dtype == VK_F32 ? 4 : 2;
   const int ve = 16 / eb;
@@ -507,8 +508,12 @@
   VK_CHECK_ARG(!d->src0.up || (d->H % 2 == 0 && d->W % 2 == 0), "vk_conv_fwd: upsampled source needs even H, W");
   VK_CHECK_ARG(!(d->src1.ptr && d->src1.up), "vk_conv_fwd: only src0 may be upsampled");
   if (halo_enabled()) {
-    const int rc = conv3x3_halo_try(d, w, packed, y, y1, split_k1, accumulate, stats, pool2, bnr, st, workspace, workspace_bytes);
+    const int rc = conv3x3_halo_try(d, w, packed, y, y1, split_k1, accumulate, stats, pool2, bnr, st, workspace, workspace_bytes, acc_src, mask_bits);
     if (rc != VK_ERR_UNSUPPORTED) return rc;
+  }
+  if (acc_src || mask_bits) {
+    vkh::set_error("vk_conv_dgrad_fused_ex: an accumulate source / a bit mask is only available on the 3x3 stride-1 tile kernels (16-bit types for the bits)");
+    return VK_ERR_UNSUPPORTED;
   }
   if (packed) {
     vkh::set_error("vk_conv_fwd_packed: shape not covered by the 3x3 stride-1 tile kernels (use vk_conv_fwd with plain weights)");
@@ -608,11 +613,23 @@
   return vk::conv_fwd_impl(d, w, vk::is_c16(d) ? 0 : 1, y_half, y1, split_k1, accumulate, nullptr, 1, nullptr, (hipStream_t)stream);
 }
 
+extern "C" int vk_conv_dgrad_fused_ex(const vk_conv_desc* d, const void* w, void* y, void* y1, int split_k1, int pool2, const vk_bnr* bnr,
+                                      const vk_dgrad_ext* ext, void* stream) {
+  const void* acc_src = ext ? ext->acc_src : nullptr;
+  const void* mask_bits = ext ? ext->mask_bits : nullptr;
+  VK_CHECK_ARG(!bnr || (bnr->z && bnr->sums && (bnr->mask || mask_bits || (bnr->scale && bnr->shift))), "vk_conv_dgrad_fused: incomplete vk_bnr");
+  VK_CHECK_ARG(!bnr || !((bnr->mask || mask_bits) && pool2), "vk_conv_dgrad_fused: the external mask does not combine with pool2");
+  VK_CHECK_ARG(!mask_bits || bnr, "vk_conv_dgrad_fused_ex: mask_bits needs a vk_bnr");
+  VK_CHECK_ARG(!mask_bits || (d && d->dtype != VK_F32), "vk_conv_dgrad_fused_ex: mask_bits is for the 16-bit types");
+  VK_CHECK_ARG(!acc_src || (bnr && bnr->accumulate), "vk_conv_dgrad_fused_ex: acc_src needs a vk_bnr with accumulate set");
+  VK_CHECK_ARG(!acc_src || !pool2, "vk_conv_dgrad_fused_ex: acc_src does not combine with pool2");
+  return vk::conv_fwd_impl(d, w, vk::is_c16(d) ? 0 : 1, y, y1, split_k1, bnr ? bnr->accumulate : 0, nullptr, pool2, bnr, (hipStream_t)stream,
+                           nullptr, 0, acc_src, mask_bits);
+}
+
 extern "C" int vk_conv_dgrad_fused(const vk_conv_desc* d, const void* w, void* y, void* y1, int split_k1, int pool2, const vk_bnr* bnr,
                                    void* stream) {
-  VK_CHECK_ARG(!bnr || (bnr->z && bnr->sums && (bnr->mask || (bnr->scale && bnr->shift))), "vk_conv_dgrad_fused: incomplete vk_bnr");
-  VK_CHECK_ARG(!bnr || !(bnr->mask && pool2), "vk_conv_dgrad_fused: the external mask does not combine with pool2");
-  return vk::conv_fwd_impl(d, w, vk::is_c16(d) ? 0 : 1, y, y1, split_k1, bnr ? bnr->accumulate : 0, nullptr, pool2, bnr, (hipStream_t)stream);
+  return vk_conv_dgrad_fused_ex(d, w, y, y1, split_k1, pool2, bnr, nullptr, stream);
 }
 
 extern "C" int vk_conv_fwd_packed(const vk_conv_desc* d, const void* w_halo, void* y, void* y1, int split_k1, int accumulate, double* stats,
diff --git a/vickers-hardness-unet_amd/csrc/elementwise.hip b/vickers-hardness-unet_amd/csrc/elementwise.hip
--- a/vickers-hardness-unet_amd/csrc/elementwise.hip
+++ b/vickers-hardness-unet_amd/csrc/elementwise.hip
@@ -183,10 +183,10 @@
   }
 }
 
-template <typename T, int MAXC>
+template <typename T, int MAXC, bool BITS = false>
 __global__ __launch_bounds__(256) void k_bn_add_relu(size_t pixels, int C, const T* __restrict__ z, const float* __restrict__ scale,
                                                      const float* __restrict__ shift, const T* __restrict__ res, const float* __restrict__ rscale,
-                                                     const float* __restrict__ rshift, T* __restrict__ out) {
+                                                     const float* __restrict__ rshift, T* __restrict__ out, uint8_t* __restrict__ bits = nullptr) {
   constexpr int VE = ElemTraits<T>::kVec;
   constexpr int U = 4;
   const int CV = C / VE;
@@ -229,7 +229,15 @@
       Vec16<T>::unpack(rv[u], r);
 #pragma unroll
       for (int j = 0; j < VE; ++j) f[j] = fmaxf(fmaf(f[j], sc[j], sh[j]) + fmaf(r[j], rsc[j], rsh[j]), 0.f);
-      *reinterpret_cast<u32x4_t*>(out + k * VE) = Vec16<T>::pack(f);
+      const u32x4_t ov = Vec16<T>::pack(f);
+      *reinterpret_cast<u32x4_t*>(out + k * VE) = ov;
+      if (BITS) {
+        Vec16<T>::unpack(ov, f);
+        unsigned m = 0;
+#pragma unroll
+        for (int j = 0; j < VE; ++j) m |= (f[j] > 0.f ? 1u : 0u) << j;
+        bits[k] = (uint8_t)m;
+      }
     }
   }
 }
@@ -345,6 +353,11 @@
 #pragma unroll
     for (int j = 0; j < VE; ++j)
       if (!(m[j] > 0.f)) g[j] = 0.f;
+  } else if (MASK == 3) {
+    const unsigned m = reinterpret_cast<const uint8_t*>(mask_src)[off / VE];
+#pragma unroll
+    for (int j = 0; j < VE; ++j)
+      if (!((m >> j) & 1u)) g[j] = 0.f;
   }
 }
 
@@ -1352,6 +1365,26 @@
   return VK_OK;
 }
 
+extern "C" int vk_bn_add_relu_bits(vk_dtype dtype, size_t pixels, int C, const void* z, const float* scale, const float* shift,
+                                   const void* res, const float* rscale, const float* rshift, void* out, uint8_t* bits, void* stream) {
+  VK_CHECK_ARG(z && scale && shift && res && out && bits, "vk_bn_add_relu_bits: null argument");
+  VK_CHECK_ARG(dtype == VK_BF16 || dtype == VK_F16, "vk_bn_add_relu_bits: the bit mask is for the 16-bit types");
+  if (const int rc = check_flat_channels("vk_bn_add_relu_bits", C)) return rc;
+  if (C > 512) {
+    vkh::set_error("vk_bn_add_relu_bits: C=%d unsupported (up to 512)", C);
+    return VK_ERR_UNSUPPORTED;
+  }
+  hipStream_t st = (hipStream_t)stream;
+  vkh::ProfScope ps_("bn_add_relu_bits", st, 0.0, (double)pixels * C * 2.0 * 3.0625);
+  const dim3 grid(channel_grid(grid_for((pixels * (C / 8) + 3) / 4), C / 8));
+  if (dtype == VK_BF16)
+    hipLaunchKernelGGL((k_bn_add_relu<bf16_t, 512, true>), grid, dim3(256), 0, st, pixels, C, (const bf16_t*)z, scale, shift, (const bf16_t*)res, rscale, rshift, (bf16_t*)out, bits);
+  else
+    hipLaunchKernelGGL((k_bn_add_relu<f16_t, 512, true>), grid, dim3(256), 0, st, pixels, C, (const f16_t*)z, scale, shift, (const f16_t*)res, rscale, rshift, (f16_t*)out, bits);
+  VK_CHECK_HIP(hipGetLastError());
+  return VK_OK;
+}
+
 template <typename T>
 static int launch_bn_bwd_reduce(size_t pixels, int C, const void* dy, const void* z, int mask_mode, const float* scale,
                                 const float* shift, const void* mask_src, double* sums, hipStream_t st) {
@@ -1374,19 +1407,21 @@
   dim3 grid((unsigned)nb), block(256);
   if (mask_mode == 0) hipLaunchKernelGGL((k_bn_bwd_reduce<T, 0>), grid, block, 0, st, pixels, C, (const T*)dy, (const T*)z, scale, shift, (const T*)mask_src, sums);
   else if (mask_mode == 1) hipLaunchKernelGGL((k_bn_bwd_reduce<T, 1>), grid, block, 0, st, pixels, C, (const T*)dy, (const T*)z, scale, shift, (const T*)mask_src, sums);
-  else hipLaunchKernelGGL((k_bn_bwd_reduce<T, 2>), grid, block, 0, st, pixels, C, (const T*)dy, (const T*)z, scale, shift, (const T*)mask_src, sums);
+  else if (mask_mode == 2) hipLaunchKernelGGL((k_bn_bwd_reduce<T, 2>), grid, block, 0, st, pixels, C, (const T*)dy, (const T*)z, scale, shift, (const T*)mask_src, sums);
+  else if constexpr (sizeof(T) == 2) hipLaunchKernelGGL((k_bn_bwd_reduce<T, 3>), grid, block, 0, st, pixels, C, (const T*)dy, (const T*)z, scale, shift, (const T*)mask_src, sums);
   return VK_OK;
 }
 
 extern "C" int vk_bn_bwd_reduce(vk_dtype dtype, size_t pixels, int C, const void* dy, const void* z, int mask_mode,
                                 const float* scale, const float* shift, const void* mask_src, double* sums, void* stream) {
   VK_CHECK_ARG(dy && z && sums, "vk_bn_bwd_reduce: null argument");
-  VK_CHECK_ARG(mask_mode >= 0 && mask_mode <= 2, "vk_bn_bwd_reduce: mask_mode %d", mask_mode);
+  VK_CHECK_ARG(mask_mode >= 0 && mask_mode <= 3, "vk_bn_bwd_reduce: mask_mode %d", mask_mode);
   VK_CHECK_ARG(mask_mode != 1 || (scale && shift), "vk_bn_bwd_reduce: mask_mode 1 needs scale/shift");
-  VK_CHECK_ARG(mask_mode != 2 || mask_src, "vk_bn_bwd_reduce: mask_mode 2 needs mask_src");
+  VK_CHECK_ARG(mask_mode < 2 || mask_src, "vk_bn_bwd_reduce: mask_mode 2 / 3 needs mask_src");
+  VK_CHECK_ARG(mask_mode != 3 || dtype != VK_F32, "vk_bn_bwd_reduce: mask_mode 3 (bit mask) is for the 16-bit types");
   if (const int rc = check_flat_channels("vk_bn_bwd_reduce", C)) return rc;
   hipStream_t st = (hipStream_t)stream;
-  vkh::ProfScope ps_("bn_bwd_reduce", st, 0.0, (double)pixels * C * (dtype == VK_F32 ? 4.0 : 2.0) * (mask_mode == 2 ? 3.0 : 2.0));
+  vkh::ProfScope ps_("bn_bwd_reduce", st, 0.0, (double)pixels * C * (dtype == VK_F32 ? 4.0 : 2.0) * (mask_mode == 2 ? 3.0 : mask_mode == 3 ? 2.0625 : 2.0));
   DISPATCH_T(dtype, launch_bn_bwd_reduce<T>(pixels, C, dy, z, mask_mode, scale, shift, mask_src, sums, st));
   VK_CHECK_HIP(hipGetLastError());
   return VK_OK;
@@ -1428,7 +1463,8 @@
     a.shift, (const T*)a.mask_src, a.coef, a.sums, a.count, a.gamma, a.mean, a.invstd, a.dgamma, a.dbeta, (T*)a.dz, (T*)a.g_out, a.g_acc)
     if (a.mask_mode == 0) VK_APPLY_W(0);
     else if (a.mask_mode == 1) VK_APPLY_W(1);
-    else VK_APPLY_W(2);
+    else if (a.mask_mode == 2) VK_APPLY_W(2);
+    else if constexpr (sizeof(T) == 2) VK_APPLY_W(3);
 #undef VK_APPLY_W
     return VK_OK;
   }
@@ -1436,19 +1472,21 @@
     (const T*)a.mask_src, a.coef, a.sums, a.count, a.gamma, a.mean, a.invstd, a.dgamma, a.dbeta, (T*)a.dz, (T*)a.g_out, a.g_acc)
   if (a.mask_mode == 0) VK_APPLY(0);
   else if (a.mask_mode == 1) VK_APPLY(1);
-  else VK_APPLY(2);
+  else if (a.mask_mode == 2) VK_APPLY(2);
+  else if constexpr (sizeof(T) == 2) VK_APPLY(3);
 #undef VK_APPLY
   return VK_OK;
 }
 
 static int bn_bwd_apply_common(vk_dtype dtype, const BnApplyArgs& a, void* stream) {
   VK_CHECK_ARG(a.dy && a.z && a.dz && (a.coef || (a.sums && a.gamma && a.mean && a.invstd && a.dgamma && a.dbeta)), "vk_bn_bwd_apply: null argument");
-  VK_CHECK_ARG(a.mask_mode >= 0 && a.mask_mode <= 2, "vk_bn_bwd_apply: mask_mode %d", a.mask_mode);
+  VK_CHECK_ARG(a.mask_mode >= 0 && a.mask_mode <= 3, "vk_bn_bwd_apply: mask_mode %d", a.mask_mode);
   VK_CHECK_ARG(a.mask_mode != 1 || (a.scale && a.shift), "vk_bn_bwd_apply: mask_mode 1 needs scale/shift");
-  VK_CHECK_ARG(a.mask_mode != 2 || a.mask_src, "vk_bn_bwd_apply: mask_mode 2 needs mask_src");
+  VK_CHECK_ARG(a.mask_mode < 2 || a.mask_src, "vk_bn_bwd_apply: mask_mode 2 / 3 needs mask_src");
+  VK_CHECK_ARG(a.mask_mode != 3 || dtype != VK_F32, "vk_bn_bwd_apply: mask_mode 3 (bit mask) is for the 16-bit types");
   if (const int rc = check_flat_channels("vk_bn_bwd_apply", a.C)) return rc;
   hipStream_t st = (hipStream_t)stream;
-  vkh::ProfScope ps_("bn_bwd_apply", st, 0.0, (double)a.pixels * a.C * (dtype == VK_F32 ? 4.0 : 2.0) * ((a.mask_mode == 2 ? 4.0 : 3.0) + (a.g_out ? (a.g_acc ? 2.0 : 1.0) : 0.0)));
+  vkh::ProfScope ps_("bn_bwd_apply", st, 0.0, (double)a.pixels * a.C * (dtype == VK_F32 ? 4.0 : 2.0) * ((a.mask_mode == 2 ? 4.0 : a.mask_mode == 3 ? 3.0625 : 3.0) + (a.g_out ? (a.g_acc ? 2.0 : 1.0) : 0.0)));
   DISPATCH_T(dtype, launch_bn_bwd_apply<T>(a, st));
   VK_CHECK_HIP(hipGetLastError());
   return VK_OK;
diff --git a/vickers-hardness-unet_amd/csrc/engine.hip b/vickers-hardness-unet_amd/csrc/engine.hip
--- a/vickers-hardness-unet_amd/csrc/engine.hip
+++ b/vickers-hardness-unet_amd/csrc/engine.hip
@@ -346,6 +346,7 @@
   bool in_has_grad_first;
   char* out = nullptr;
   char* gout = nullptr;
+  uint8_t* obits = nullptr;
 };
 
 struct DecL {
@@ -413,6 +414,7 @@
   int64_t head_w_off = 0, head_b_off = 0;
   std::vector<std::pair<int64_t, int64_t>> buckets;
   size_t ws_bytes = 0;
+  std::vector<size_t> off_obits;
   size_t off_x4 = 0, off_pool = 0, off_argmax = 0, off_gpool = 0, off_dup = 0, off_dlogits = 0, off_loss_sums = 0;
   size_t off_stats = 0, off_bsums = 0, stats_bytes = 0, off_farena = 0, farena_floats = 0, off_wf = 0, off_wd = 0, off_wstem = 0;
   size_t off_tab_pack = 0, off_tab_bn = 0, off_wslab = 0, off_wh = 0, off_tab_halo = 0, off_splitk = 0, splitk_bytes = 0;
@@ -734,6 +736,12 @@
   }
   h->sloss_bytes = vk_seg_loss_workspace_bytes(N, h->classes, S * SW);
   h->off_sloss = take(h->sloss_bytes);
+  h->off_obits.assign(h->blocks.size(), 0);
+  if (tr && eb == 2)
+    for (size_t b = 0; b < h->blocks.size(); ++b) {
+      const BlockL& k = h->blocks[b];
+      if (k.conv3 < 0 && k.C <= 512) h->off_obits[b] = take((size_t)N * k.Hout * k.Wout * k.C / 8);
+    }
   h->ws_bytes = off;
 }
 
@@ -753,6 +761,7 @@
     BlockL& k = h->blocks[b];
     k.out = ws + h->off_out[b];
     k.gout = h->cfg.training ? ws + h->off_gout[b] : nullptr;
+    k.obits = h->off_obits[b] ? (uint8_t*)(ws + h->off_obits[b]) : nullptr;
     const std::string nm = h->convs[k.conv1].name.substr(0, h->convs[k.conv1].name.size() - 6);
     h->debug["out:" + nm] = {k.out, {N, k.Hout, k.Wout, k.C}};
     if (k.gout) h->debug["gout:" + nm] = {k.gout, {N, k.Hout, k.Wout, k.C}};
@@ -1154,14 +1163,17 @@
     if (k.conv3 >= 0) RET_IF(run_conv(h, ct, to_src(bn_act(h, c2)), null_src(), training, st));
     const BnL& b2 = h->bns[ct.bn];
     const size_t pixels = (size_t)N * k.Hout * k.Wout;
+    uint8_t* const obits = training && !getenv("VK_NO_TAIL_BITS") ? k.obits : nullptr;
+    const void* res = cur.ptr;
+    const float *rscale = nullptr, *rshift = nullptr;
     if (k.convd >= 0) {
       ConvL& cd = h->convs[k.convd];
       RET_IF(run_conv(h, cd, to_src(cur), null_src(), training, st));
       const BnL& bd = h->bns[cd.bn];
-      RET_IF(vk_bn_add_relu(dt, pixels, k.C, ct.z, b2.scale, b2.shift, cd.z, bd.scale, bd.shift, k.out, st));
-    } else {
-      RET_IF(vk_bn_add_relu(dt, pixels, k.C, ct.z, b2.scale, b2.shift, cur.ptr, nullptr, nullptr, k.out, st));
-    }
+      res = cd.z; rscale = bd.scale; rshift = bd.shift;
+    }
+    if (obits) RET_IF(vk_bn_add_relu_bits(dt, pixels, k.C, ct.z, b2.scale, b2.shift, res, rscale, rshift, k.out, obits, st));
+    else RET_IF(vk_bn_add_relu(dt, pixels, k.C, ct.z, b2.scale, b2.shift, res, rscale, rshift, k.out, st));
     cur = Act{k.out, k.C, nullptr, nullptr, 0};
   }
   Act skips[5];
@@ -1454,6 +1466,11 @@
   return conv_wgrad(h, c1, to_src(xprev, 1), d.Cskip ? to_src(skip) : null_src(), st);
 }
 
+bool tail_fusable(vk_unet* h, ConvL& c) {
+  vk_conv_desc d = dgrad_desc(h, c);
+  return d.stride == 1 && vk_conv_uses_halo_pack(&d) != 0;
+}
+
 int backward_block(vk_unet* h, int bi, hipStream_t st) {
   BlockL& k = h->blocks[bi];
   ConvL& c1 = h->convs[k.conv1];
@@ -1476,18 +1493,25 @@
     gin = pb.gout;
   }
   const bool pre = h->tail_prereduced[(size_t)bi] != 0;
+  const int tail_maxc = getenv("VK_TAIL_BNR_MAXC") ? atoi(getenv("VK_TAIL_BNR_MAXC")) : 1 << 20;
   h->tail_prereduced[(size_t)bi] = 0;
   if (bi > 0) h->tail_prereduced[(size_t)bi - 1] = 0;
-  const int mm = pre ? 0 : 2;
-  if (!pre && bn_sums_needed(h, b2)) RET_IF(vk_bn_bwd_reduce(dt, pixels, k.C, k.gout, c2.z, 2, nullptr, nullptr, k.out, b2.bsums, st));
+  const bool use_bits = !getenv("VK_NO_TAIL_BITS");
+  const int mm = pre ? 0 : k.obits && use_bits ? 3 : 2;
+  const void* const msrc = mm == 3 ? (const void*)k.obits : (const void*)k.out;
+  if (!pre && bn_sums_needed(h, b2)) RET_IF(vk_bn_bwd_reduce(dt, pixels, k.C, k.gout, c2.z, mm, nullptr, nullptr, msrc, b2.bsums, st));
+  const bool into_gin = need_from(h, c1.rank + 1);
+  const bool tail_route = into_gin && k.convd < 0 && bi > 0 && c1.halo_dg && k.C <= tail_maxc && !getenv("VK_NO_TAIL_BNR_FUSION") &&
+                          tail_fusable(h, c1);
+  const bool alias = pre && k.convd < 0 && !k.in_has_grad_first && (tail_route || !into_gin) && !getenv("VK_NO_TAIL_ALIAS");
   if (k.convd < 0) {
-    RET_IF(bn_bwd_phase2(h, b2, k.C, pixels, k.gout, c2.z, mm, k.out, c2.g, gin, k.in_has_grad_first ? 1 : 0, st));
+    RET_IF(bn_bwd_phase2(h, b2, k.C, pixels, k.gout, c2.z, mm, msrc, c2.g, alias ? nullptr : gin, k.in_has_grad_first ? 1 : 0, st));
   } else {
     ConvL& cd = h->convs[k.convd];
     BnL& bd = h->bns[cd.bn];
-    RET_IF(bn_bwd_phase2(h, b2, k.C, pixels, k.gout, c2.z, mm, k.out, c2.g, nullptr, 0, st));
-    if (bn_sums_needed(h, bd)) RET_IF(vk_bn_bwd_reduce(dt, pixels, k.C, k.gout, cd.z, mm, nullptr, nullptr, k.out, bd.bsums, st));
-    RET_IF(bn_bwd_phase2(h, bd, k.C, pixels, k.gout, cd.z, mm, k.out, cd.g, nullptr, 0, st));
+    RET_IF(bn_bwd_phase2(h, b2, k.C, pixels, k.gout, c2.z, mm, msrc, c2.g, nullptr, 0, st));
+    if (bn_sums_needed(h, bd)) RET_IF(vk_bn_bwd_reduce(dt, pixels, k.C, k.gout, cd.z, mm, nullptr, nullptr, msrc, bd.bsums, st));
+    RET_IF(bn_bwd_phase2(h, bd, k.C, pixels, k.gout, cd.z, mm, msrc, cd.g, nullptr, 0, st));
   }
   const bool into1 = need_from(h, h->bns[c1.bn].rank);
   bool fused1 = false;
@@ -1495,18 +1519,23 @@
   if (trains(h, c2.w_t)) RET_IF(conv_wgrad(h, c2, to_src(bn_act(h, c1)), null_src(), st));
   if (!into1) return k.convd >= 0 && trains(h, h->convs[k.convd].w_t) ? conv_wgrad(h, h->convs[k.convd], to_src(xin), null_src(), st) : VK_OK;
   RET_IF(bn_relu_bwd_inplace(h, c1, fused1, st));
-  const bool into_gin = need_from(h, c1.rank + 1);
   bool tail_fused = false;
-  const int tail_maxc = getenv("VK_TAIL_BNR_MAXC") ? atoi(getenv("VK_TAIL_BNR_MAXC")) : 1 << 20;
-  if (into_gin && k.convd < 0 && bi > 0 && c1.halo_dg && k.C <= tail_maxc && !getenv("VK_NO_TAIL_BNR_FUSION")) {
+  if (tail_route) {
     BlockL& pb = h->blocks[bi - 1];
     ConvL& pc2 = h->convs[pb.conv2];
     vk_conv_desc dd = dgrad_desc(h, c1);
     vk_bnr r;
     r.z = pc2.z; r.scale = nullptr; r.shift = nullptr; r.sums = h->bns[pc2.bn].bsums; r.mask = pb.out; r.accumulate = 1;
-    const int rc = vk_conv_dgrad_fused(&dd, dgrad_weights(h, c1), gin, nullptr, 0, 0, &r, st);
+    vk_dgrad_ext ext;
+    ext.acc_src = alias ? k.gout : nullptr;
+    ext.mask_bits = use_bits ? pb.obits : nullptr;
+    const int rc = vk_conv_dgrad_fused_ex(&dd, dgrad_weights(h, c1), gin, nullptr, 0, 0, &r, &ext, st);
     if (rc == VK_OK) { tail_fused = true; h->tail_prereduced[(size_t)bi - 1] = 1; }
     else if (rc != VK_ERR_UNSUPPORTED) return rc;
+    else if (alias) {
+      vkh::set_error("backward_block: the tile kernels declined a data gradient that tail_fusable accepted (block %d)", bi);
+      return VK_ERR_STATE;
+    }
   }
   if (into_gin && !tail_fused) RET_IF(conv_dgrad(h, c1, gin, nullptr, 0, 1, st));
   if (k.convd >= 0) {
```
